# joejep/FOCNeRF

Hardware: AMD Instinct MI355X
Metric: train_samples_per_sec (higher is better)
Workload: dtype f16

## Files before the change

### focnerf_amd/_lib.py

```python
import ctypes
import os

import torch

_HERE = os.path.dirname(os.path.abspath(__file__))
LIB_PATH = os.environ.get("FOCNERF_LIB_PATH") or os.path.join(_HERE, "libfocnerf_hip.so")

c_u8p = ctypes.c_void_p
c_vp = ctypes.c_void_p
u32 = ctypes.c_uint32
u64 = ctypes.c_uint64
f32 = ctypes.c_float
i32 = ctypes.c_int

FOC_F32 = 0
FOC_F16 = 1



class FocOccTrainNode(ctypes.Structure):
    _fields_ = [
        ("struct_bytes", u32),
        ("n_rays", u32), ("max_steps", u32), ("cascade", u32), ("grid_size", u32), ("cap", u32), ("pad_align", u32),
        ("bound", f32), ("dt_gamma", f32), ("min_near", f32),
# ... 23 lines not shown
        ("mlp_workspace_bytes", u64),
    ]


SIGNATURES = {
    "foc_abi_version": (i32, []),
    "foc_last_error": (ctypes.c_char_p, []),
    "foc_arch": (ctypes.c_char_p, []),
    "foc_near_far_from_aabb": (i32, [c_vp, c_vp, c_vp, u32, f32, c_vp, c_vp, c_vp]),
    "foc_sph_from_ray": (i32, [c_vp, c_vp, f32, u32, c_vp, c_vp]),
    "foc_morton3D": (i32, [c_vp, u32, c_vp, c_vp]),
    "foc_morton3D_invert": (i32, [c_vp, u32, c_vp, c_vp]),
    "foc_packbits": (i32, [c_vp, u32, f32, c_vp, c_vp]),
    "foc_march_rays_train": (i32, [c_vp, c_vp, c_vp, f32, f32, u32, u32, u32, u32, u32, c_vp, c_vp,
                                   c_vp, c_vp, c_vp, c_vp, c_vp, c_vp, c_vp, c_vp]),
    "foc_march_rays_train_field": (i32, [c_vp, c_vp, c_vp, f32, f32, u32, u32, u32, u32, u32, c_vp, c_vp,
                                         c_vp, c_vp, c_vp, c_vp, c_vp, c_vp, c_vp, u32, c_vp, f32, c_vp]),
    "foc_set_option": (i32, [ctypes.c_char_p, i32]),
    "foc_get_option": (i32, [ctypes.c_char_p, c_vp]),
    "foc_guard_pick_device": (i32, [i32, i32, i32, i32]),
    "foc_grid_forward_index_path": (i32, [u32, u32, u32]),
    "foc_view_tile_order": (i32, [c_vp, u32, u32, u32, c_vp, c_vp, c_vp]),
    "foc_occ_train_forward": (i32, [ctypes.POINTER(FocOccTrainNode), c_vp]),
    "foc_occ_train_backward": (i32, [ctypes.POINTER(FocOccTrainNode), c_vp]),
    "foc_occ_train_forward_pad31": (i32, [ctypes.POINTER(FocOccTrainNode), f32, c_vp]),
    "foc_occ_train_backward_pad31": (i32, [ctypes.POINTER(FocOccTrainNode), f32, c_vp]),
    "foc_occ_tail_forward": (i32, [c_vp, c_vp, u32, c_vp, c_vp, u32, u32, f32, f32, c_vp, f32, c_vp, c_vp, c_vp, c_vp, c_vp, c_vp, c_vp]),
    "foc_occ_tail_backward": (i32, [c_vp, c_vp, c_vp, c_vp, u32, c_vp, c_vp, c_vp, c_vp, c_vp, u32, u32, f32, f32, c_vp, f32, c_vp, c_vp, c_vp]),
    "foc_march_rays_train_scratch_bytes": (u64, [u32, u32]),
    "foc_composite_rays_train_forward": (i32, [c_vp, c_vp, c_vp, c_vp, u32, u32, f32, c_vp, c_vp, c_vp, c_vp]),
    "foc_composite_rays_train_backward": (i32, [c_vp, c_vp, c_vp, c_vp, c_vp, c_vp, c_vp, c_vp, u32, u32, f32,
                                                c_vp, c_vp, c_vp]),
    "foc_march_rays": (i32, [u32, u32, c_vp, c_vp, c_vp, c_vp, f32, f32, u32, u32, u32, c_vp, c_vp, c_vp,
                             c_vp, c_vp, c_vp, c_vp, c_vp]),
    "foc_composite_rays": (i32, [u32, u32, f32, c_vp, c_vp, c_vp, c_vp, c_vp, c_vp, c_vp, c_vp, c_vp]),
    "foc_compact_alive": (i32, [c_vp, u32, c_vp, c_vp, c_vp, c_vp]),
    "foc_march_rays_two_phase": (i32, [u32, u32, c_vp, c_vp, c_vp, c_vp, f32, f32, u32, u32, u32, c_vp, c_vp, c_vp, c_vp, c_vp, c_vp, c_vp, c_vp, i32, c_vp]),
    "foc_composite_compact": (i32, [u32, u32, f32, c_vp, c_vp, c_vp, c_vp, c_vp, c_vp, c_vp, c_vp, c_vp, c_vp, c_vp, c_vp, u32, u32, i32, c_vp]),
    "foc_march_rays_two_phase_fills": (i32, [u32, i32]),
    "foc_march_rays_two_phase_sample_major": (i32, [u32, u32, i32]),
    "foc_occ_render_step_scratch_bytes": (u64, [u32]),
    "foc_occ_render_step": (i32, [u32, u32, c_vp, c_vp, c_vp, c_vp, c_vp, c_vp, f32, f32, u32, u32, u32, c_vp, c_vp, c_vp, c_vp, c_vp, c_vp, c_vp, c_vp,
                                  c_vp, c_vp, c_vp, u32, f32, u32, c_vp, u32, c_vp, u32, u32, c_vp, f32, c_vp, c_vp, c_vp, c_vp, u32, c_vp, u32, u32, c_vp]),
    "foc_occ_render_step_pad31": (i32, [u32, u32, c_vp, c_vp, c_vp, c_vp, c_vp, c_vp, f32, f32, u32, u32, u32, c_vp, c_vp, c_vp, c_vp, c_vp, c_vp, c_vp, c_vp,
                                        c_vp, c_vp, c_vp, u32, f32, u32, c_vp, u32, c_vp, u32, u32, c_vp, f32, c_vp, c_vp, c_vp, c_vp, u32, c_vp, u32, u32, f32,
                                        c_vp]),
    "foc_grid_encode_forward": (i32, [c_vp, c_vp, c_vp, c_vp, u32, u32, u32, u32, f32, u32, c_vp, u32, i32, u32,
                                      i32, c_vp, c_vp]),
    "foc_grid_encode_forward_bl": (i32, [c_vp, c_vp, c_vp, c_vp, u32, u32, u32, u32, f32, u32, c_vp, u32, i32, u32,
                                         i32, c_vp, c_vp]),
    "foc_grid_encode_backward": (i32, [c_vp, c_vp, c_vp, c_vp, c_vp, u32, u32, u32, u32, f32, u32, c_vp, c_vp,
                                       u32, i32, u32, i32, i32, c_vp, c_vp]),
    "foc_grid_encode_backward_workspace_bytes": (u64, [u32, u32, u32, u32, i32]),
    "foc_grid_planes_to_rows": (i32, [c_vp, c_vp, u32, u32, u32, c_vp]),
    "foc_grid_rows_to_planes": (i32, [c_vp, c_vp, u32, u32, u32, c_vp]),
    "foc_grid_encode_backward_binned": (i32, [c_vp, c_vp, c_vp, c_vp, c_vp, u32, u32, u32, u32, f32, u32, c_vp, c_vp,
                                              u32, i32, u32, i32, i32, c_vp, c_vp, u64, c_vp]),
    "foc_grid_encode_forward_counted": (i32, [c_vp, c_vp, c_vp, c_vp, u32, u32, u32, u32, f32, u32, u32, i32, u32, i32, c_vp, c_vp, u64, c_vp]),
    "foc_grid_encode_backward_count": (i32, [c_vp, c_vp, u32, u32, u32, u32, f32, u32, u32, i32, u32, i32, c_vp, c_vp, u64, c_vp]),
    "foc_grid_encode_backward_binned_counted": (i32, [c_vp, c_vp, c_vp, c_vp, c_vp, u32, u32, u32, u32, f32, u32, c_vp, c_vp,
                                                      u32, i32, u32, i32, i32, c_vp, c_vp, u64, c_vp]),
    "foc_grad_total_variation": (i32, [c_vp, c_vp, c_vp, c_vp, f32, u32, u32, u32, u32, f32, u32, u32, i32, i32, c_vp]),
    "foc_freq_encode_forward": (i32, [c_vp, u32, u32, u32, u32, c_vp, c_vp]),
    "foc_freq_encode_backward": (i32, [c_vp, c_vp, u32, u32, u32, u32, c_vp, c_vp]),
    "foc_ffmlp_forward": (i32, [c_vp, c_vp, u32, u32, u32, u32, u32, u32, u32, c_vp, c_vp, c_vp]),
    "foc_ffmlp_inference": (i32, [c_vp, c_vp, u32, u32, u32, u32, u32, u32, u32, c_vp, c_vp, c_vp]),
    "foc_ffmlp_backward": (i32, [c_vp, c_vp, c_vp, c_vp, u32, u32, u32, u32, u32, u32, u32, i32,
                                 c_vp, c_vp, c_vp, c_vp, u64, c_vp]),
    "foc_ffmlp_backward_workspace_bytes": (u64, [u32, u32, u32]),
    "foc_ffmlp_forward_planar": (i32, [c_vp, c_vp, u32, u32, u32, u32, u32, u32, u32, c_vp, c_vp]),
    "foc_ffmlp_backward_planar": (i32, [c_vp, c_vp, c_vp, u32, u32, u32, u32, u32, u32, u32, i32, c_vp, c_vp, c_vp, u64, c_vp]),
    "foc_allocate_splitk": (i32, [u64]),
    "foc_free_splitk": (i32, []),
    "foc_combine_select": (i32, [c_vp, c_vp, c_vp, c_vp, u64, c_vp]),
    "foc_combine_pack_keys": (i32, [c_vp, u32, c_vp, u64, c_vp]),
    "foc_combine_unpack": (i32, [c_vp, u32, c_vp, c_vp, c_vp, u64, c_vp]),
    "foc_combine_select_composite": (i32, [c_vp, u32, c_vp, c_vp, u32, u32, c_vp, u32, c_vp, c_vp, c_vp, c_vp]),
    "foc_combine_select4": (i32, [c_vp, c_vp, u64, c_vp]),
    "foc_mo_select": (i32, [c_vp, c_vp, c_vp, c_vp, u64, u32, u32, c_vp]),
    "foc_fixed_field_pack": (i32, [c_vp, c_vp, c_vp, c_vp, c_vp, c_vp, f32, u32, u32, f32, f32, c_vp, c_vp, c_vp, c_vp, u32, c_vp]),
    "foc_composite_fixed_steps": (i32, [c_vp, c_vp, c_vp, c_vp, u32, u32, f32, c_vp, c_vp, c_vp]),
    "foc_fixed_sample": (i32, [c_vp, c_vp, c_vp, c_vp, c_vp, c_vp, u32, u32, f32, c_vp, c_vp, c_vp, u32, c_vp]),
    "foc_fixed_tail_forward": (i32, [c_vp, c_vp, c_vp, c_vp, c_vp, c_vp, f32, u32, u32, f32, f32, c_vp, c_vp, c_vp, c_vp, c_vp, c_vp, u32, c_vp, c_vp]),
    "foc_fixed_tail_backward": (i32, [c_vp, c_vp, c_vp, c_vp, c_vp, c_vp, c_vp, c_vp, c_vp, c_vp, c_vp, f32, u32, u32, f32, f32, c_vp, c_vp, u32, c_vp, c_vp]),
    "foc_fixed_head_forward": (i32, [c_vp, c_vp, c_vp, c_vp, c_vp, u32, u32, f32, c_vp, c_vp, c_vp, c_vp, c_vp, c_vp, c_vp, u32, c_vp]),
    "foc_fixed_head_backward": (i32, [c_vp, c_vp, c_vp, c_vp, c_vp, c_vp, c_vp, c_vp, c_vp, c_vp, u32, u32, f32, c_vp, u32, c_vp]),
    "foc_color_head_forward": (i32, [c_vp, c_vp, u32, c_vp, u32, u32, u32, u32, c_vp, u32, c_vp, c_vp]),
    "foc_field_forward_train": (i32, [c_vp, c_vp, u32, c_vp, u32, c_vp, u32, u32, u32, u32, c_vp, c_vp, u32, c_vp, c_vp]),
    "foc_color_head_backward": (i32, [c_vp, c_vp, c_vp, u32, c_vp, c_vp, u32, u32, u32, u32, c_vp, c_vp, c_vp, u64, u32, c_vp, c_vp, c_vp]),
    "foc_color_head_forward_pad": (i32, [c_vp, c_vp, u32, c_vp, u32, u32, u32, u32, c_vp, u32, c_vp, f32, c_vp]),
    "foc_color_head_backward_pad": (i32, [c_vp, c_vp, c_vp, u32, c_vp, c_vp, u32, u32, u32, u32, c_vp, c_vp, c_vp, u64, u32, c_vp, c_vp, f32, c_vp]),
    "foc_field_forward_train_pad": (i32, [c_vp, c_vp, u32, c_vp, u32, c_vp, u32, u32, u32, u32, c_vp, c_vp, u32, c_vp, f32, c_vp]),
    "foc_color_head_forward_pad31": (i32, [c_vp, c_vp, u32, c_vp, u32, u32, u32, u32, c_vp, u32, c_vp, f32, c_vp]),
    "foc_color_head_backward_pad31": (i32, [c_vp, c_vp, c_vp, u32, c_vp, c_vp, u32, u32, u32, u32, c_vp, c_vp, c_vp, u64, u32, c_vp, c_vp, f32, c_vp]),
    "foc_field_forward_train_pad31": (i32, [c_vp, c_vp, u32, c_vp, u32, c_vp, u32, u32, u32, u32, c_vp, c_vp, u32, c_vp, f32, c_vp]),
    "foc_fixed_composite_forward": (i32, [c_vp, c_vp, c_vp, f32, u32, u32, f32, c_vp, c_vp]),
    "foc_fixed_composite_backward": (i32, [c_vp, c_vp, c_vp, c_vp, f32, u32, u32, f32, c_vp, c_vp, c_vp]),
    "foc_sample_head_forward": (i32, [c_vp, c_vp, u64, c_vp, c_vp, c_vp, u32, c_vp]),
    "foc_sample_head_backward": (i32, [c_vp, c_vp, c_vp, u64, c_vp, u32, c_vp]),
    "foc_sh_encode": (i32, [c_vp, u64, c_vp, c_vp]),
    "foc_rgb_head_forward": (i32, [c_vp, u64, c_vp, c_vp]),
    "foc_rgb_head_backward": (i32, [c_vp, c_vp, u64, c_vp, c_vp]),
    "foc_fixed_render_inference": (i32, [c_vp, c_vp, c_vp, c_vp, c_vp, c_vp, f32, u32, u32, f32, f32, c_vp, c_vp, c_vp, c_vp, u32, c_vp, c_vp]),
    "foc_nerf_field_inference": (i32, [c_vp, i32, c_vp, u32, u32, u32, c_vp, u32, c_vp, u32, u32, u32, u32, c_vp, c_vp, c_vp, c_vp]),
    "foc_nerf_field_inference_pad": (i32, [c_vp, i32, c_vp, u32, u32, u32, c_vp, u32, c_vp, u32, u32, u32, u32, c_vp, c_vp, c_vp, f32, c_vp]),
    "foc_nerf_field_inference_pad31": (i32, [c_vp, i32, c_vp, u32, u32, u32, c_vp, u32, c_vp, u32, u32, u32, u32, c_vp, c_vp, c_vp, f32, c_vp]),
    "foc_mark_untrained_grid": (i32, [c_vp, u32, f32, f32, f32, f32, f32, u32, u32, c_vp, c_vp, c_vp]),
    "foc_grid_cells_xyz": (i32, [u32, u32, f32, c_vp, c_vp, c_vp]),
    "foc_grid_update_sample_workspace_bytes": (u64, [u32, u32]),
    "foc_grid_update_sample": (i32, [c_vp, u32, u32, f32, u32, c_vp, c_vp, c_vp, c_vp, c_vp, c_vp, u64, c_vp]),
    "foc_grid_update_apply_workspace_bytes": (u64, [u32, u32]),
    "foc_grid_update_apply": (i32, [c_vp, u32, u32, c_vp, c_vp, u32, f32, f32, f32, c_vp, c_vp, c_vp, u64, c_vp]),
    "foc_background_forward": (i32, [c_vp, c_vp, c_vp, f32, u32, c_vp, c_vp, f32, u32, c_vp, c_vp, c_vp]),
    "foc_background_backward_workspace_bytes": (u64, [u32]),
    "foc_background_backward": (i32, [c_vp, c_vp, c_vp, c_vp, f32, u32, c_vp, c_vp, f32, u32, c_vp, c_vp, c_vp, c_vp, u64, c_vp]),
}


def _load():
    if not os.path.exists(LIB_PATH):
        raise ImportError(
            f"focnerf_amd: {LIB_PATH} is missing. Build it with `python -c 'import __graft_entry__ as g; g.build()'` "
            f"or `make -C focnerf_amd/csrc`. There is no CPU or PyTorch fallback for these ops.")
    try:
        lib = ctypes.CDLL(LIB_PATH)
    except OSError as e:
        raise ImportError(f"focnerf_amd: failed to load {LIB_PATH}: {e}") from e
    for name, (res, args) in SIGNATURES.items():
        fn = getattr(lib, name)
        fn.restype = res
        fn.argtypes = args
    return lib


class _Stream(ctypes.c_void_p):
    device_index = None


_multi_device = None


def _on_tensor_device(fn):
    def call(*args):
        global _multi_device
        if _multi_device is None:
            _multi_device = torch.cuda.device_count() > 1
        if _multi_device and args:
            idx = getattr(args[-1], "device_index", None)
            if idx is not None and idx != torch.cuda.current_device():
                with torch.cuda.device(idx):
                    return fn(*args)
        return fn(*args)
    call.__name__ = getattr(fn, "__name__", "foc_call")
    return call


class _Lib:

    def __init__(self, cdll):
        self._cdll = cdll
        for name, (_, args) in SIGNATURES.items():
            fn = getattr(cdll, name)
            setattr(self, name, _on_tensor_device(fn) if args and args[-1] is c_vp and not name.endswith("_bytes") else fn)


lib = _Lib(_load())


def check(rc, what=""):
    if rc != 0:
        msg = lib.foc_last_error().decode("utf-8", "replace")
        raise RuntimeError(f"focnerf_amd {what}: {msg} (code {rc})")


def ptr(t):
    if t is None:
        return None
    return ctypes.c_void_p(t.data_ptr())
# ... 57 lines not shown
```

### focnerf_amd/csrc/combine.hip

```cpp
#include "common.h"
#include <string.h>

static thread_local char g_err[512] = "";

void foc_set_error(const char *fmt, ...) {
    va_list ap;
    va_start(ap, fmt);
    vsnprintf(g_err, sizeof(g_err), fmt, ap);
    va_end(ap);
}

__global__ void __launch_bounds__(256) k_combine_select(const float *__restrict__ dens, const float *__restrict__ rgb,
                                                        float *__restrict__ max_dens, float *__restrict__ best_rgb, uint64_t n) {
    for (uint64_t i = (uint64_t)blockIdx.x * 256 + threadIdx.x; i < n; i += (uint64_t)gridDim.x * 256) {
        const float d = dens[i], m = max_dens[i];
        if (d > m) { best_rgb[i * 3] = rgb[i * 3]; best_rgb[i * 3 + 1] = rgb[i * 3 + 1]; best_rgb[i * 3 + 2] = rgb[i * 3 + 2]; }
        max_dens[i] = (d != d || m != m) ? __builtin_nanf("") : (d > m ? d : m);
    }
}

__global__ void __launch_bounds__(256) k_combine_pack(const float *__restrict__ dens, uint32_t rank, uint64_t *__restrict__ keys, uint64_t n) {
    for (uint64_t i = (uint64_t)blockIdx.x * 256 + threadIdx.x; i < n; i += (uint64_t)gridDim.x * 256) {
        float d = dens[i];
        d = d > 0.0f ? d : 0.0f;
// ... 85 lines not shown
        if (valid) {
            const uint64_t s = (uint64_t)n * T + i;
            float4 best = fields.p[0][s];
            for (uint32_t k = 1; k < K; k++) {
                const float4 f = fields.p[k][s];
                const float m = best.x;
                if (f.x > m) { best.y = f.y; best.z = f.z; best.w = f.w; }
                best.x = (f.x != f.x || m != m) ? __builtin_nanf("") : (f.x > m ? f.x : m);
            }
            if (merged4) merged4[s] = best;
            sigma = best.x; c0 = best.y; c1 = best.z; c2 = best.w;
            const float l0 = (i < T / 2) ? (step * (float)i) : fmaf(-step, (float)(T - 1 - i), 1.0f);
            const float z = near + span * l0;
            float delta = sample_dist;
            if (i + 1 < T) {
                const uint32_t i1 = i + 1;
                const float l1 = (i1 < T / 2) ? (step * (float)i1) : fmaf(-step, (float)(T - 1 - i1), 1.0f);
                delta = (near + span * l1) - z;
            }
            alpha = 1 - __expf(-delta * sigma);
            oz = (z - near) / span;
            oz = oz < 0 ? 0 : (oz > 1 ? 1 : oz);
        }
        const float om = valid ? (1 - alpha + 1e-15f) : 1.0f;
        const float P = wave_incl_prod(om, (int)lane);
        float Pex = __shfl_up(P, 1, 64);
        if (lane == 0) Pex = 1.0f;
        const float w = alpha * (Tc * Pex);
        r = fmaf(w, c0, r); g = fmaf(w, c1, g); b = fmaf(w, c2, b);
        a = fmaf(w, sigma, a); d = fmaf(w, oz, d); ws += w;
        Tc *= __shfl(P, 63, 64);
    }
    r = wave_sum(r); g = wave_sum(g); b = wave_sum(b); a = wave_sum(a); d = wave_sum(d); ws = wave_sum(ws);
    if (lane == 0) {
        for (uint32_t q = 0; q < n_bg; q++) {
            const float rest = (1 - ws) * (q == 0 ? bg0 : bg1);
            const float o[4] = {r + rest, g + rest, b + rest, a + rest};
#pragma unroll
            for (int k = 0; k < 4; k++) image4[((uint64_t)q * N + n) * 4 + k] = fminf(1.0f, fmaxf(0.0f, o[k]));
        }
        depth[n] = d;
    }
}

__global__ void __launch_bounds__(256) k_combine_select4(const float4 *__restrict__ f4, float4 *__restrict__ acc4, uint64_t n) {
    for (uint64_t i = (uint64_t)blockIdx.x * 256 + threadIdx.x; i < n; i += (uint64_t)gridDim.x * 256) {
        const float4 f = f4[i];
        float4 best = acc4[i];
        const float m = best.x;
        if (f.x > m) { best.y = f.y; best.z = f.z; best.w = f.w; }
        best.x = (f.x != f.x || m != m) ? __builtin_nanf("") : (f.x > m ? f.x : m);
        acc4[i] = best;
    }
}

template <typename T>
__global__ void __launch_bounds__(256) k_mo_select(const T *__restrict__ sig_new, const T *__restrict__ feat_new, T *__restrict__ sig_best,
                                                   T *__restrict__ feat_best, uint64_t n, uint32_t width) {
    const uint64_t s0 = ((uint64_t)blockIdx.x * 4u + (threadIdx.x >> 6)) * 64u;
    if (s0 >= n) return;
    const uint32_t lane = threadIdx.x & 63u;
    bool take = false;
    if (s0 + lane < n) {
        const T a_raw = sig_new[s0 + lane];
        const float a = (float)a_raw, b = (float)sig_best[s0 + lane];
        take = (a != a) || (b == b && a >= b);
        if (take) sig_best[s0 + lane] = a_raw;
    }
    const uint64_t rows = __ballot(take);
    const uint32_t live = (uint32_t)(n - s0 < 64u ? n - s0 : 64u);
    const uint64_t base = s0 * width;
    for (uint32_t e = lane; e < live * width; e += 64u)
        if ((rows >> (e / width)) & 1ull) feat_best[base + e] = feat_new[base + e];
}

#include <stdlib.h>
#include <string.h>
#include <atomic>
#include <mutex>
struct FocOptionRow { const char *name; std::atomic<int> value; };
static FocOptionRow foc_option_table[FOC_OPT_COUNT] = {
    {"FOC_MLP_BWD_FUSED", 1}, {"FOC_FIELD_FWD_FUSED", 1}, {"FOC_GB_MERGE_MAX_RES", 480}, {"FOC_GB_FACTORED", 1}, {"FOC_GB_TAIL_SPLIT", 16}, {"FOC_GRID_FUSE_SMALL", 1},
    {"FOC_GRID_PAIRS", 1}, {"FOC_GRID_FAST", 1}, {"FOC_MARCH_SERIAL", -1}, {"FOC_MARCH_RAYS_ROW_MAX", 131072}, {"FOC_OCC_MARCH_FORM", -1},
    {"FOC_OCC_SAMPLE_MAJOR", 1}, {"FOC_OCC_FIELD_PIECE", 1 << 23},
};
static int foc_option_parse(int which, const char *text) {
    if (which == FOC_OPT_OCC_MARCH_FORM) {
        if (text[0] == 't') return 0;
        if (text[0] == 'r') return 1;
        if (text[0] == 'l') return 2;
        if (text[0] == 's') return 3;
    }
    return atoi(text);
}
static void foc_options_init() {
    static std::once_flag once;
    std::call_once(once, [] {
        for (int i = 0; i < FOC_OPT_COUNT; i++) {
            const char *e = getenv(foc_option_table[i].name);
            if (e && e[0]) foc_option_table[i].value.store(foc_option_parse(i, e), std::memory_order_relaxed);
        }
    });
}
int foc_opt(FocOpt which) { foc_options_init(); return foc_option_table[which].value.load(std::memory_order_relaxed); }

extern "C" {

int foc_set_option(const char *name, int value) {
    foc_options_init();
    for (int i = 0; i < FOC_OPT_COUNT; i++)
        if (name && strcmp(name, foc_option_table[i].name) == 0) { foc_option_table[i].value.store(value, std::memory_order_relaxed); return FOC_OK; }
    foc_set_error("set_option: unknown option '%s'", name ? name : "(null)");
    return FOC_E_INVALID;
}

int foc_get_option(const char *name, int *value) {
    foc_options_init();
    for (int i = 0; i < FOC_OPT_COUNT; i++)
        if (name && value && strcmp(name, foc_option_table[i].name) == 0) { *value = foc_option_table[i].value.load(std::memory_order_relaxed); return FOC_OK; }
    foc_set_error("get_option: unknown option '%s'", name ? name : "(null)");
    return FOC_E_INVALID;
}

int foc_guard_pick_device(int stream_is_null, int stream_device, int pointer_device, int current_device) {
    return foc_guard_pick(stream_is_null != 0, stream_device, pointer_device, current_device);
}


int foc_combine_select_composite(const float *const *fields4, uint32_t K, const float *nears, const float *fars, uint32_t N, uint32_t T,
                                 const float *bgs, uint32_t n_bg, float *image4, float *depth, float *merged4, void *stream) {
    FocDeviceGuard foc_guard_(stream, nears);
    FOC_REQUIRE(K >= 1 && K <= FOC_COMBINE_MAX_OBJECTS, FOC_E_INVALID, "combine_select_composite: 1 <= K <= %d objects per call (got %u)",
                FOC_COMBINE_MAX_OBJECTS, K);
    FOC_REQUIRE(n_bg >= 1 && n_bg <= 2 && bgs, FOC_E_INVALID, "combine_select_composite: one or two backgrounds");
    FOC_REQUIRE(T >= 2, FOC_E_INVALID, "combine_select_composite: T must be >= 2");
    if (N == 0) return FOC_OK;
    FOC_REQUIRE(fields4 && nears && fars && image4 && depth, FOC_E_INVALID, "combine_select_composite: null pointer");
    CombineFields f;
    for (uint32_t k = 0; k < FOC_COMBINE_MAX_OBJECTS; k++) {
        f.p[k] = reinterpret_cast<const float4 *>(k < K ? fields4[k] : fields4[0]);
        FOC_REQUIRE(f.p[k] && ((uintptr_t)f.p[k] & 15) == 0, FOC_E_INVALID, "combine_select_composite: field %u is null or not 16-byte aligned", k);
    }
    FOC_REQUIRE(((uintptr_t)merged4 & 15) == 0, FOC_E_INVALID, "combine_select_composite: merged4 must be 16-byte aligned");
    hipLaunchKernelGGL(k_combine_select_composite, dim3(foc_div_up(N, 4)), dim3(256), 0, (hipStream_t)stream, f, K, nears, fars, N, T, bgs[0],
                       n_bg > 1 ? bgs[1] : 0.0f, n_bg, image4, depth, reinterpret_cast<float4 *>(merged4));
    FOC_CHECK_LAUNCH("combine_select_composite");
    return FOC_OK;
}

int foc_combine_select4(const float *field4, float *acc4, uint64_t n, void *stream) {
    FocDeviceGuard foc_guard_(stream, field4);
    FOC_REQUIRE(n == 0 || (field4 && acc4), FOC_E_INVALID, "combine_select4: null pointer");
    FOC_REQUIRE((((uintptr_t)field4 | (uintptr_t)acc4) & 15) == 0, FOC_E_INVALID, "combine_select4: fields must be 16-byte aligned");
    if (n == 0) return FOC_OK;
    hipLaunchKernelGGL(k_combine_select4, dim3(foc_grid_1d(n, 256)), dim3(256), 0, (hipStream_t)stream, reinterpret_cast<const float4 *>(field4),
                       reinterpret_cast<float4 *>(acc4), n);
    FOC_CHECK_LAUNCH("combine_select4");
    return FOC_OK;
}

int foc_mo_select(const void *sigma_new, const void *feat_new, void *sigma_best, void *feat_best, uint64_t n, uint32_t feat_width,
                  uint32_t elem_bytes, void *stream) {
    FocDeviceGuard foc_guard_(stream, sigma_new);
    FOC_REQUIRE(elem_bytes == 2 || elem_bytes == 4, FOC_E_INVALID, "mo_select: elem_bytes must be 2 (half) or 4 (float), got %u", elem_bytes);
    FOC_REQUIRE(feat_width >= 1 && feat_width <= 64, FOC_E_INVALID, "mo_select: feat_width %u outside 1..64", feat_width);
    FOC_REQUIRE(n == 0 || (sigma_new && feat_new && sigma_best && feat_best), FOC_E_INVALID, "mo_select: null pointer");
    FOC_REQUIRE(n < (1ull << 38), FOC_E_INVALID, "mo_select: n too large");
// ... 56 lines not shown
```

### focnerf_amd/csrc/common.h

```cpp
#pragma once
#include <hip/hip_runtime.h>
#include <hip/hip_fp16.h>
#include <stdint.h>
#include <stdio.h>
#include <stdarg.h>
#include "../../include/focnerf.h"

#define FOC_WAVE 64

void foc_set_error(const char *fmt, ...);

enum FocOpt {
    FOC_OPT_MLP_BWD_FUSED,
    FOC_OPT_FIELD_FWD_FUSED,
    FOC_OPT_GB_MERGE_MAX_RES,
    FOC_OPT_GB_FACTORED,
    FOC_OPT_GB_TAIL_SPLIT,
    FOC_OPT_GRID_FUSE_SMALL,
    FOC_OPT_GRID_PAIRS,
    FOC_OPT_GRID_FAST,
    FOC_OPT_MARCH_SERIAL,
    FOC_OPT_MARCH_RAYS_ROW_MAX,
    FOC_OPT_OCC_MARCH_FORM,
    FOC_OPT_OCC_SAMPLE_MAJOR,
    FOC_OPT_OCC_FIELD_PIECE,
    FOC_OPT_COUNT
};
int foc_opt(FocOpt which);

#define FOC_REQUIRE(cond, code, ...)                    \
    do {                                                \
        if (!(cond)) {                                  \
            foc_set_error(__VA_ARGS__);                 \
            return (code);                              \
        }                                               \
    } while (0)

#define FOC_CHECK_LAUNCH(name)                                                     \
    do {                                                                           \
        hipError_t e_ = hipGetLastError();                                         \
        if (e_ != hipSuccess) {                                                    \
            foc_set_error("%s: launch failed: %s", name, hipGetErrorString(e_));   \
            return FOC_E_LAUNCH;                                                   \
        }                                                                          \
    } while (0)

static inline int foc_guard_pick(bool stream_is_null, int stream_device, int pointer_device, int current_device) {
    if (!stream_is_null && stream_device >= 0) return stream_device;
    if (pointer_device >= 0) return pointer_device;
    return current_device;
}
struct FocDeviceGuard {
    int prev = -1;
    explicit FocDeviceGuard(void *stream, const void *first_pointer = nullptr) {
        static int n_devices = -1;
        if (n_devices < 0 && hipGetDeviceCount(&n_devices) != hipSuccess) { (void)hipGetLastError(); n_devices = 0; }
        if (n_devices == 1) return;
        int cur = 0;
        if (hipGetDevice(&cur) != hipSuccess) return;
        int sdev = -1, pdev = -1;
        if (stream != nullptr) {
            if (hipStreamGetDevice(static_cast<hipStream_t>(stream), &sdev) != hipSuccess) { (void)hipGetLastError(); sdev = -1; }
        } else if (first_pointer != nullptr) {
            hipPointerAttribute_t attr;
            if (hipPointerGetAttributes(&attr, first_pointer) == hipSuccess && attr.type == hipMemoryTypeDevice) pdev = attr.device;
            else (void)hipGetLastError();
        }
        const int want = foc_guard_pick(stream == nullptr, sdev, pdev, cur);
        if (want != cur && hipSetDevice(want) == hipSuccess) prev = cur;
    }
    ~FocDeviceGuard() { if (prev >= 0) (void)hipSetDevice(prev); }
    FocDeviceGuard(const FocDeviceGuard &) = delete;
    FocDeviceGuard &operator=(const FocDeviceGuard &) = delete;
};

static inline uint32_t foc_div_up(uint64_t a, uint64_t b) { return (uint32_t)((a + b - 1) / b); }

static inline uint32_t foc_grid_1d(uint64_t n, uint32_t block, uint32_t max_blocks = 256 * 8) {
    uint64_t g = (n + block - 1) / block;
    if (g < 1) g = 1;
    if (g > max_blocks) g = max_blocks;
    return (uint32_t)g;
}

__device__ __forceinline__ _Float16 foc_f2h(float v) { asm volatile("" : "+v"(v)); return (_Float16)v; }

__global__ static void __launch_bounds__(256) k_foc_zero(uint32_t *__restrict__ p, uint64_t n_words) {
    for (uint64_t i = (uint64_t)blockIdx.x * 256 + threadIdx.x; i < n_words; i += (uint64_t)gridDim.x * 256) p[i] = 0u;
}
static inline hipError_t foc_zero_async(void *p, size_t bytes, hipStream_t st) {
    const uint64_t n = bytes / 4;
    if (n == 0) return hipSuccess;
    uint64_t blocks = (n + 255) / 256;
    if (blocks > 4096) blocks = 4096;
    hipLaunchKernelGGL(k_foc_zero, dim3((uint32_t)blocks), dim3(256), 0, st, reinterpret_cast<uint32_t *>(p), n);
    return hipGetLastError();
}

__device__ __forceinline__ void foc_lds_barrier() { asm volatile("s_waitcnt lgkmcnt(0)\n\ts_barrier" ::: "memory"); }

__device__ __forceinline__ float wave_sum(float v) {
#pragma unroll
    for (int o = 32; o > 0; o >>= 1) v += __shfl_xor(v, o, 64);
    return v;
}
__device__ __forceinline__ int wave_sum_i(int v) {
#pragma unroll
    for (int o = 32; o > 0; o >>= 1) v += __shfl_xor(v, o, 64);
// ... 27 lines not shown
```

### focnerf_amd/csrc/field_fwd.hip

```cpp
#include "mlp_common.h"

typedef uint32_t ff_u2 __attribute__((ext_vector_type(2)));

__device__ __forceinline__ uint32_t ff_pack(float a, float b) {
    typedef _Float16 h2 __attribute__((ext_vector_type(2)));
    const h2 p = {(_Float16)a, (_Float16)b};
    return __builtin_bit_cast(uint32_t, p);
}

#ifndef FF_MIN_WAVES
#define FF_MIN_WAVES 2
#endif
template <int NLS, int NLC, bool RELU>
__global__ void __launch_bounds__(MLP_BLOCK, FF_MIN_WAVES) k_field_fwd_train(const _Float16 *__restrict__ planes, const _Float16 *__restrict__ w_sigma,
                                                               const _Float16 *__restrict__ w_color, _Float16 *__restrict__ h_out,
                                                               _Float16 *__restrict__ c_out, uint32_t B, MlpHead hd) {
    constexpr int HIDDEN = 64, MT = 2, KC = 4, KS0 = 2;
    constexpr int FS = MT * KS0 + (NLS - 1) * MT * KC + KC;
    constexpr int FC = MT * KS0 + (NLC - 1) * MT * KC + KC;
    extern __shared__ __attribute__((aligned(16))) _Float16 lds[];
    _Float16 *ldsS = lds, *ldsC = lds + FS * 512;
    const float *obj_bias = reinterpret_cast<const float *>(ldsC + FC * 512);
    stage_weights_fwd<HIDDEN>(w_sigma, ldsS, 32, NLS);
    stage_weights_fwd<HIDDEN>(w_color, ldsC, 32, NLC, true, head_ld0(hd));
    if (head_bias(hd)) stage_head_bias(w_color, hd, const_cast<float *>(obj_bias), HIDDEN);
    __syncthreads();

    const uint32_t lane = threadIdx.x & 63, wave = threadIdx.x >> 6;
    const int c = lane & 31, h = lane >> 5;
    const uint32_t n_tiles = (B + 31) / 32;
    const uint32_t tstride = gridDim.x * MLP_WAVES;
    uint32_t tile = blockIdx.x * MLP_WAVES + wave;
    h8 x_nxt[KS0], sh_nxt;
    auto fetch = [&](uint32_t t) {
#ifdef FF_TIMING_NO_LOAD
        const uint64_t r = (uint64_t)c + 0 * t;
#else
        const uint64_t r = min((uint64_t)min(t, n_tiles - 1u) * 32 + c, (uint64_t)B - 1);
#endif
#pragma unroll
        for (int kc = 0; kc < KS0; kc++) x_nxt[kc] = ld_planar8(planes, B, r, kc, h);
        sh_nxt = ld_head8(planes, hd, r, 0, h);
    };
    fetch(tile);
    for (; tile < n_tiles; tile += tstride) {
#ifndef FF_TIMING_HOIST
        asm volatile("" ::: "memory");
#endif
        const uint64_t row_raw = (uint64_t)tile * 32 + c;
        h8 x_cur[KS0];
#pragma unroll
        for (int kc = 0; kc < KS0; kc++) x_cur[kc] = x_nxt[kc];
        const h8 sh = sh_nxt;
        fetch(tile + tstride);
        f16v acc[MT];
#pragma unroll
        for (int mt = 0; mt < MT; mt++)
#pragma unroll
            for (int e = 0; e < 16; e++) acc[mt][e] = 0.0f;
#pragma unroll
        for (int kc = 0; kc < KS0; kc++)
#pragma unroll
            for (int mt = 0; mt < MT; mt++) acc[mt] = mfma16(ld_frag(ldsS, mt * KS0 + kc, lane), x_cur[kc], acc[mt]);
        f16v o;
        for (uint32_t l = 1; l <= (uint32_t)NLS; l++) {
            h8 bf[KC];
#pragma unroll
            for (int kc = 0; kc < KC; kc++) bf[kc] = acc_to_frag<RELU>(acc[kc >> 1], kc & 1);
            if (l < (uint32_t)NLS) {
                const uint32_t fbase = MT * KS0 + (l - 1) * MT * KC;
#pragma unroll
                for (int mt = 0; mt < MT; mt++)
#pragma unroll
                    for (int e = 0; e < 16; e++) acc[mt][e] = 0.0f;
#pragma unroll
                for (int kc = 0; kc < KC; kc++)
#pragma unroll
                    for (int mt = 0; mt < MT; mt++) acc[mt] = mfma16(ld_frag(ldsS, fbase + mt * KC + kc, lane), bf[kc], acc[mt]);
            } else {
#pragma unroll
                for (int e = 0; e < 16; e++) o[e] = 0.0f;
#pragma unroll
                for (int kc = 0; kc < KC; kc++) o = mfma16(ld_frag(ldsS, FS - KC + kc, lane), bf[kc], o);
            }
        }
        uint32_t P0 = ff_pack(o[0], o[1]), P1 = ff_pack(o[2], o[3]), P2 = ff_pack(o[4], o[5]), P3 = ff_pack(o[6], o[7]);
#ifdef FF_TIMING_NO_STORE
        if (row_raw == 0xFFFFFFFFFFull) {
#else
        if (row_raw < B) {
#endif
            *reinterpret_cast<ff_u2 *>(h_out + row_raw * 16 + 4 * h) = ff_u2{P0, P1};
            *reinterpret_cast<ff_u2 *>(h_out + row_raw * 16 + 8 + 4 * h) = ff_u2{P2, P3};
        }
        const uint32_t nxt = h == 0 ? P2 : 0u;
        const ff_u2 s02 = __builtin_amdgcn_permlane32_swap(P0, P2, false, false);
        const ff_u2 s13 = __builtin_amdgcn_permlane32_swap(P1, P3, false, false);
        const h8 hk = head_shift(u32x4{s02.x, s13.x, s02.y, s13.y}, nxt);
#pragma unroll
        for (int mt = 0; mt < MT; mt++) {
            if (head_bias(hd)) acc[mt] = ld_obj_bias(obj_bias, mt, h);
            else {
#pragma unroll
                for (int e = 0; e < 16; e++) acc[mt][e] = 0.0f;
            }
        }
#pragma unroll
        for (int kc = 0; kc < KS0; kc++)
#pragma unroll
            for (int mt = 0; mt < MT; mt++) acc[mt] = mfma16(ld_frag(ldsC, mt * KS0 + kc, lane), kc == 0 ? sh : hk, acc[mt]);
        for (uint32_t l = 1; l <= (uint32_t)NLC; l++) {
            h8 bf[KC];
#pragma unroll
            for (int kc = 0; kc < KC; kc++) bf[kc] = acc_to_frag<RELU>(acc[kc >> 1], kc & 1);
            if (l < (uint32_t)NLC) {
                const uint32_t fbase = MT * KS0 + (l - 1) * MT * KC;
#pragma unroll
                for (int mt = 0; mt < MT; mt++)
#pragma unroll
                    for (int e = 0; e < 16; e++) acc[mt][e] = 0.0f;
#pragma unroll
                for (int kc = 0; kc < KC; kc++)
#pragma unroll
                    for (int mt = 0; mt < MT; mt++) acc[mt] = mfma16(ld_frag(ldsC, fbase + mt * KC + kc, lane), bf[kc], acc[mt]);
            } else {
#pragma unroll
                for (int e = 0; e < 16; e++) o[e] = 0.0f;
#pragma unroll
                for (int kc = 0; kc < KC; kc++) o = mfma16(ld_frag(ldsC, FC - KC + kc, lane), bf[kc], o);
                if (hd.out_width == 4u) {
#ifdef FF_TIMING_NO_STORE
                    if (h == 0 && row_raw == 0xFFFFFFFFFFull) *reinterpret_cast<ff_u2 *>(c_out + row_raw * 4) = ff_u2{ff_pack(o[0], o[1]), ff_pack(o[2], o[3])};
#else
                    if (h == 0 && row_raw < B) *reinterpret_cast<ff_u2 *>(c_out + row_raw * 4) = ff_u2{ff_pack(o[0], o[1]), ff_pack(o[2], o[3])};
#endif
                } else store_tile<false>(c_out, 16, row_raw, B, 0, 16, o, h);
            }
        }
    }
}

static uint32_t ff_num_cus() {
    int dev = 0, n = 0;
    if (hipGetDevice(&dev) != hipSuccess || hipDeviceGetAttribute(&n, hipDeviceAttributeMultiprocessorCount, dev) != hipSuccess || n <= 0) n = 256;
    return (uint32_t)n;
}

template <int NLS, int NLC, bool RELU>
static int ff_launch(const void *planes, const void *w_sigma, const void *w_color, void *h, void *c, uint32_t B, const MlpHead &hd, hipStream_t st) {
    auto kern = k_field_fwd_train<NLS, NLC, RELU>;
    const size_t lds = (size_t)((4 + (NLS - 1) * 8 + 4) + (4 + (NLC - 1) * 8 + 4)) * 1024 + 256;
    if (lds > 64 * 1024) (void)hipFuncSetAttribute(reinterpret_cast<const void *>(kern), hipFuncAttributeMaxDynamicSharedMemorySize, (int)lds);
    static int resident = 0;
    if (!resident) {
        int n = 0;
        if (hipOccupancyMaxActiveBlocksPerMultiprocessor(&n, kern, MLP_BLOCK, lds) != hipSuccess || n < 1) n = 2;
        resident = n > 8 ? 8 : n;
    }
    uint32_t grid = foc_div_up(foc_div_up(B, 32), MLP_WAVES);
    const uint32_t cap = ff_num_cus() * (uint32_t)resident;
    if (grid > cap) grid = cap;
    hipLaunchKernelGGL(kern, dim3(grid), dim3(MLP_BLOCK), lds, st, (const _Float16 *)planes, (const _Float16 *)w_sigma, (const _Float16 *)w_color,
                       (_Float16 *)h, (_Float16 *)c, B, hd);
    FOC_CHECK_LAUNCH("field_forward_train");
    return FOC_OK;
}

template <int NLS, int NLC>
static int ff_launch_act(const void *planes, const void *w_sigma, const void *w_color, void *h, void *c, uint32_t B, int relu, const MlpHead &hd, hipStream_t st) {
    return relu ? ff_launch<NLS, NLC, true>(planes, w_sigma, w_color, h, c, B, hd, st) : ff_launch<NLS, NLC, false>(planes, w_sigma, w_color, h, c, B, hd, st);
}

static int field_forward_train(const void *planes, const void *sigma_weights, uint32_t sigma_layers, const void *ray_sh, uint32_t samples_per_ray,
                               const void *color_weights, uint32_t color_layers, uint32_t hidden_dim, uint32_t activation, uint32_t B, void *h, void *c,
                               uint32_t out_width, const void *obj_feat, float input_pad, bool pad31, void *stream) {
    FocDeviceGuard foc_guard_(stream, planes);
    if (B == 0) return FOC_OK;
    FOC_REQUIRE(planes && sigma_weights && ray_sh && color_weights && h && c, FOC_E_INVALID, "field_forward_train: null pointer");
    FOC_REQUIRE(hidden_dim == 64 && samples_per_ray >= 1, FOC_E_INVALID, "field_forward_train: hidden_dim must be 64 (got %u), samples_per_ray >= 1", hidden_dim);
    FOC_REQUIRE(activation == FOC_ACT_RELU || activation == FOC_ACT_NONE, FOC_E_INVALID, "field_forward_train: hidden activation must be relu(0) or none(6)");
    FOC_REQUIRE(out_width == 16 || out_width == 4, FOC_E_INVALID, "field_forward_train: out_width must be 16 or 4 (got %u)", out_width);
    const int prc = head_pad_check("field_forward_train", pad31, obj_feat, input_pad);
    if (prc) return prc;
    const MlpHead hd{(const _Float16 *)ray_sh, nullptr, samples_per_ray, out_width, (const _Float16 *)obj_feat, input_pad};
    const int relu = activation == FOC_ACT_RELU;
    hipStream_t st = (hipStream_t)stream;
    switch (sigma_layers * 10 + color_layers) {
        case 12: return ff_launch_act<1, 2>(planes, sigma_weights, color_weights, h, c, B, relu, hd, st);
        case 13: return ff_launch_act<1, 3>(planes, sigma_weights, color_weights, h, c, B, relu, hd, st);
        case 22: return ff_launch_act<2, 2>(planes, sigma_weights, color_weights, h, c, B, relu, hd, st);
        case 23: return ff_launch_act<2, 3>(planes, sigma_weights, color_weights, h, c, B, relu, hd, st);
        case 33: return ff_launch_act<3, 3>(planes, sigma_weights, color_weights, h, c, B, relu, hd, st);
        default: foc_set_error("field_forward_train: layer counts (%u, %u) are not built (1/2, 1/3, 2/2, 2/3, 3/3)", sigma_layers, color_layers); return FOC_E_INVALID;
    }
}

extern "C" {

int foc_field_forward_train(const void *planes, const void *sigma_weights, uint32_t sigma_layers, const void *ray_sh, uint32_t samples_per_ray,
                            const void *color_weights, uint32_t color_layers, uint32_t hidden_dim, uint32_t activation, uint32_t B, void *h, void *c,
                            uint32_t out_width, const void *obj_feat, void *stream) {
    return field_forward_train(planes, sigma_weights, sigma_layers, ray_sh, samples_per_ray, color_weights, color_layers, hidden_dim, activation, B, h, c,
                               out_width, obj_feat, 0.0f, false, stream);
}

int foc_field_forward_train_pad(const void *planes, const void *sigma_weights, uint32_t sigma_layers, const void *ray_sh, uint32_t samples_per_ray,
                                const void *color_weights, uint32_t color_layers, uint32_t hidden_dim, uint32_t activation, uint32_t B, void *h, void *c,
                                uint32_t out_width, const void *obj_feat, float input_pad, void *stream) {
    return field_forward_train(planes, sigma_weights, sigma_layers, ray_sh, samples_per_ray, color_weights, color_layers, hidden_dim, activation, B, h, c,
                               out_width, obj_feat, input_pad, false, stream);
}

int foc_field_forward_train_pad31(const void *planes, const void *sigma_weights, uint32_t sigma_layers, const void *ray_sh, uint32_t samples_per_ray,
                                  const void *color_weights, uint32_t color_layers, uint32_t hidden_dim, uint32_t activation, uint32_t B, void *h, void *c,
                                  uint32_t out_width, const void *obj_feat, float input_pad, void *stream) {
    return field_forward_train(planes, sigma_weights, sigma_layers, ray_sh, samples_per_ray, color_weights, color_layers, hidden_dim, activation, B, h, c,
                               out_width, obj_feat, input_pad, true, stream);
}

}
```

### focnerf_amd/csrc/fixedstep.hip

```cpp
#include "common.h"
#include <float.h>

typedef _Float16 h8 __attribute__((ext_vector_type(8)));

struct FsGeom { float near, far, span, sample_dist, step; };

#define FS_RAY_BLOCK 64u
__host__ __device__ __forceinline__ uint64_t fs_block_row(uint32_t n, uint32_t i, uint32_t T) {
    return (uint64_t)(n / FS_RAY_BLOCK) * FS_RAY_BLOCK * T + (uint64_t)i * FS_RAY_BLOCK + n % FS_RAY_BLOCK;
}

__device__ __forceinline__ FsGeom fs_geom(const float *__restrict__ nears, const float *__restrict__ fars, uint32_t n, uint32_t T) {
    FsGeom g;
    g.near = nears[n]; g.far = fars[n];
    g.span = g.far - g.near;
    g.sample_dist = g.span / (float)T;
    g.step = 1.0f / (float)(T - 1);
    return g;
}
__device__ __forceinline__ float fs_z(const FsGeom &g, uint32_t i, uint32_t T, const float *__restrict__ noise, uint64_t s) {
    const float lin = (i < T / 2) ? (g.step * (float)i) : fmaf(-g.step, (float)(T - 1 - i), 1.0f);
    float z = g.near + g.span * lin;
    if (noise) z = z + (noise[s] - 0.5f) * g.sample_dist;
    return z;
}

template <bool NOISE>
__device__ __forceinline__ float fs_zu(const FsGeom &g, uint32_t i, uint32_t T, float u) {
    const float lin = (i < T / 2) ? (g.step * (float)i) : fmaf(-g.step, (float)(T - 1 - i), 1.0f);
    float z = g.near + g.span * lin;
    if (NOISE) z = z + (u - 0.5f) * g.sample_dist;
    return z;
}

__device__ __forceinline__ void fs_sh16(float x, float y, float z, float (&o)[16]) {
    const float xy = x * y, xz = x * z, yz = y * z, x2 = x * x, y2 = y * y, z2 = z * z;
    o[0] = 0.28209479177387814f;
    o[1] = -0.48860251190291987f * y;
    o[2] = 0.48860251190291987f * z;
    o[3] = -0.48860251190291987f * x;
    o[4] = 1.0925484305920792f * xy;
    o[5] = -1.0925484305920792f * yz;
    o[6] = 0.94617469575755997f * z2 - 0.31539156525251999f;
    o[7] = -1.0925484305920792f * xz;
    o[8] = 0.54627421529603959f * x2 - 0.54627421529603959f * y2;
    o[9] = 0.59004358992664352f * y * (-3.0f * x2 + y2);
    o[10] = 2.8906114426405538f * xy * z;
    o[11] = 0.45704579946446572f * y * (1.0f - 5.0f * z2);
    o[12] = 0.3731763325901154f * z * (5.0f * z2 - 3.0f);
    o[13] = 0.45704579946446572f * x * (1.0f - 5.0f * z2);
    o[14] = 1.4453057213202769f * z * (x2 - y2);
    o[15] = 0.59004358992664352f * x * (-x2 + 3.0f * y2);
}

__global__ void __launch_bounds__(256) k_fs_sample(const float *__restrict__ rays_o, const float *__restrict__ rays_d, const float *__restrict__ nears,
                                                   const float *__restrict__ fars, const float *__restrict__ aabb, const float *__restrict__ noise,
                                                   uint32_t N, uint32_t T, float bound, float *__restrict__ xyzs, float *__restrict__ enc_in,
                                                   _Float16 *__restrict__ ray_sh, uint32_t ray_block) {
    const uint64_t total = ray_block ? (uint64_t)((N + FS_RAY_BLOCK - 1) / FS_RAY_BLOCK) * FS_RAY_BLOCK * T : (uint64_t)N * T;
    const float a0 = aabb[0], a1 = aabb[1], a2 = aabb[2], a3 = aabb[3], a4 = aabb[4], a5 = aabb[5];
    const float two_b = 2 * bound;
    for (uint64_t s = (uint64_t)blockIdx.x * 256 + threadIdx.x; s < total; s += (uint64_t)gridDim.x * 256) {
        uint32_t n, i;
        bool own = true;
        if (ray_block) {
            const uint32_t blk = (uint32_t)(s / ((uint64_t)FS_RAY_BLOCK * T)), in = (uint32_t)(s - (uint64_t)blk * FS_RAY_BLOCK * T);
            i = in / FS_RAY_BLOCK;
            n = blk * FS_RAY_BLOCK + in % FS_RAY_BLOCK;
            own = n < N;
            n = own ? n : N - 1;
        } else {
            n = (uint32_t)(s / T); i = (uint32_t)(s - (uint64_t)n * T);
        }
        const FsGeom g = fs_geom(nears, fars, n, T);
        const float z = fs_z(g, i, T, noise, (uint64_t)n * T + i);
        float x = rays_o[n * 3] + rays_d[n * 3] * z, y = rays_o[n * 3 + 1] + rays_d[n * 3 + 1] * z, w = rays_o[n * 3 + 2] + rays_d[n * 3 + 2] * z;
        x = fminf(fmaxf(x, a0), a3); y = fminf(fmaxf(y, a1), a4); w = fminf(fmaxf(w, a2), a5);
        if (xyzs) { xyzs[s * 3] = x; xyzs[s * 3 + 1] = y; xyzs[s * 3 + 2] = w; }
        if (enc_in) { enc_in[s * 3] = (x + bound) / two_b; enc_in[s * 3 + 1] = (y + bound) / two_b; enc_in[s * 3 + 2] = (w + bound) / two_b; }
        if (ray_sh && i == 0 && own) {
            float sh[16];
            fs_sh16(rays_d[n * 3], rays_d[n * 3 + 1], rays_d[n * 3 + 2], sh);
            h8 lo, hi;
#pragma unroll
            for (int k = 0; k < 8; k++) { lo[k] = foc_f2h(sh[k]); hi[k] = foc_f2h(sh[8 + k]); }
            h8 *dst = reinterpret_cast<h8 *>(ray_sh + (uint64_t)n * 16);
            dst[0] = lo; dst[1] = hi;
        }
    }
}

__global__ void __launch_bounds__(256) k_fs_head_fwd(const _Float16 *__restrict__ h, const float *__restrict__ rays_d, const float *__restrict__ nears,
                                                     const float *__restrict__ fars, const float *__restrict__ noise, uint32_t N, uint32_t T,
                                                     float density_scale, float *__restrict__ sigma_out, float *__restrict__ trans_out,
                                                     float *__restrict__ weights_out, float *__restrict__ weights_sum, float *__restrict__ depth,
                                                     _Float16 *__restrict__ cin, const _Float16 *__restrict__ obj, uint32_t cin_ld) {
    const uint32_t lane = threadIdx.x & 63;
    const uint32_t n = blockIdx.x * 4 + (threadIdx.x >> 6);
    if (n >= N) return;
    const FsGeom g = fs_geom(nears, fars, n, T);
    h8 shlo, shhi;
    h8 ob1 = {0, 0, 0, 0, 0, 0, 0, 0}, ob2 = {0, 0, 0, 0, 0, 0, 0, 0};
    _Float16 ob0 = (_Float16)0;
    if (cin) {
        float sh[16];
        fs_sh16(rays_d[n * 3], rays_d[n * 3 + 1], rays_d[n * 3 + 2], sh);
#pragma unroll
        for (int k = 0; k < 8; k++) { shlo[k] = foc_f2h(sh[k]); shhi[k] = foc_f2h(sh[8 + k]); }
        if (obj) {
            ob0 = obj[0];
#pragma unroll
            for (int k = 0; k < 8; k++) ob1[k] = obj[1 + k];
#pragma unroll
            for (int k = 0; k < 7; k++) ob2[k] = obj[9 + k];
        }
    }
    float Tc = 1.0f, ws = 0, dp = 0;
    for (uint32_t base = 0; base < T; base += 64) {
        const uint32_t i = base + lane;
        const bool valid = i < T;
        const uint64_t s = (uint64_t)n * T + (valid ? i : T - 1);
        h8 r0, r1;
        if (cin) { r0 = *reinterpret_cast<const h8 *>(h + s * 16); r1 = *reinterpret_cast<const h8 *>(h + s * 16 + 8); }
        else r0[0] = h[s * 16];
        const float sigma = expf((float)r0[0]);
        const float z = fs_z(g, valid ? i : T - 1, T, noise, s);
        float delta = g.sample_dist;
        if (i + 1 < T) delta = fs_z(g, i + 1, T, noise, s + 1) - z;
        const float alpha = valid ? 1 - expf((-delta * density_scale) * sigma) : 0.0f;
        const float om = valid ? (1 - alpha + 1e-15f) : 1.0f;
        const float P = wave_incl_prod(om, (int)lane);
        float Pex = __shfl_up(P, 1, 64);
        if (lane == 0) Pex = 1.0f;
        const float Tb = Tc * Pex;
        const float w = alpha * Tb;
        if (valid) {
            sigma_out[s] = sigma; trans_out[s] = Tb; weights_out[s] = w;
            float oz = (z - g.near) / g.span;
            oz = oz < 0.0f ? 0.0f : (oz > 1.0f ? 1.0f : oz);
            ws += w; dp += w * oz;
            if (cin) {
                h8 c2, c3;
#pragma unroll
                for (int k = 0; k < 7; k++) { c2[k] = r0[k + 1]; c3[k] = r1[k + 1]; }
                c2[7] = r1[0]; c3[7] = ob0;
                h8 *dst = reinterpret_cast<h8 *>(cin + s * cin_ld);
                dst[0] = shlo; dst[1] = shhi; dst[2] = c2; dst[3] = c3;
                if (cin_ld == 48) { dst[4] = ob1; dst[5] = ob2; }
            }
        }
        Tc *= __shfl(P, 63, 64);
    }
    ws = wave_sum(ws); dp = wave_sum(dp);
    if (lane == 0) { weights_sum[n] = ws; depth[n] = dp; }
}

__device__ __forceinline__ float wave_suffix_incl_sum(float v, int lane) {
#pragma unroll
    for (int o = 1; o < 64; o <<= 1) {
        const float u = __shfl_down(v, o, 64);
        if (lane + o < 64) v += u;
    }
    return v;
}

__global__ void __launch_bounds__(256) k_fs_head_bwd(const _Float16 *__restrict__ h, const float *__restrict__ sigma_in, const float *__restrict__ trans_in,
                                                     const float *__restrict__ nears, const float *__restrict__ fars, const float *__restrict__ noise,
                                                     const float *__restrict__ grad_w, const float *__restrict__ grad_ws, const float *__restrict__ grad_depth,
                                                     const _Float16 *__restrict__ grad_cin, uint32_t N, uint32_t T, float density_scale,
                                                     _Float16 *__restrict__ grad_h, uint32_t cin_ld) {
    const uint32_t lane = threadIdx.x & 63;
    const uint32_t n = blockIdx.x * 4 + (threadIdx.x >> 6);
// ... 22 lines not shown
        const float S_i = S_carry + (incl - gw_i);
        const float dalpha = gi * Tb - S_i / om;
        const float dsigma = dalpha * (delta * density_scale) * ex;
        const _Float16 h0 = h[s * 16];
        const float dh0 = dsigma * expf(fminf(fmaxf((float)h0, -15.0f), 15.0f));
        if (valid) {
            h8 o0, o1;
            if (grad_cin) {
                const h8 c2 = *reinterpret_cast<const h8 *>(grad_cin + s * cin_ld + 16), c3 = *reinterpret_cast<const h8 *>(grad_cin + s * cin_ld + 24);
#pragma unroll
                for (int k = 0; k < 7; k++) { o0[k + 1] = c2[k]; o1[k + 1] = c3[k]; }
                o1[0] = c2[7];
            } else {
#pragma unroll
                for (int k = 0; k < 8; k++) { o0[k] = (_Float16)0; o1[k] = (_Float16)0; }
            }
            o0[0] = foc_f2h(dh0);
            h8 *dst = reinterpret_cast<h8 *>(grad_h + s * 16);
            dst[0] = o0; dst[1] = o1;
        }
        S_carry += __shfl(incl, 0, 64);
    }
}

__device__ __forceinline__ float fs_sigmoid_h(float x) {
    return (float)(_Float16)(1.0f / (1.0f + expf(-x)));
}

__global__ void __launch_bounds__(256) k_fs_composite_fwd(const _Float16 *__restrict__ c, const float *__restrict__ weights, const float *__restrict__ bg_ray,
                                                          float bg_scalar, uint32_t N, uint32_t T, float thresh, float *__restrict__ image) {
    const uint32_t lane = threadIdx.x & 63;
    const uint32_t n = blockIdx.x * 4 + (threadIdx.x >> 6);
    if (n >= N) return;
    float r = 0, g = 0, b = 0, ws = 0;
    for (uint32_t i = lane; i < T; i += 64) {
        const uint64_t s = (uint64_t)n * T + i;
        const float w = weights[s];
        ws += w;
        if (w > thresh) {
            const uint2 raw = *reinterpret_cast<const uint2 *>(c + s * 16);
            const _Float16 *cc = reinterpret_cast<const _Float16 *>(&raw);
            r += w * fs_sigmoid_h((float)cc[0]); g += w * fs_sigmoid_h((float)cc[1]); b += w * fs_sigmoid_h((float)cc[2]);
        }
    }
    r = wave_sum(r); g = wave_sum(g); b = wave_sum(b); ws = wave_sum(ws);
    if (lane == 0) {
        const float b0 = bg_ray ? bg_ray[n * 3] : bg_scalar, b1 = bg_ray ? bg_ray[n * 3 + 1] : bg_scalar, b2 = bg_ray ? bg_ray[n * 3 + 2] : bg_scalar;
        image[n * 3] = r + (1 - ws) * b0; image[n * 3 + 1] = g + (1 - ws) * b1; image[n * 3 + 2] = b + (1 - ws) * b2;
    }
}

__global__ void __launch_bounds__(256) k_fs_composite_bwd(const float *__restrict__ grad_image, const _Float16 *__restrict__ c, const float *__restrict__ weights,
                                                          const float *__restrict__ bg_ray, float bg_scalar, uint32_t N, uint32_t T, float thresh,
                                                          _Float16 *__restrict__ grad_c, float *__restrict__ grad_w) {
    const uint64_t total = (uint64_t)N * T;
    for (uint64_t s = (uint64_t)blockIdx.x * 256 + threadIdx.x; s < total; s += (uint64_t)gridDim.x * 256) {
        const uint32_t n = (uint32_t)(s / T);
        const float g0 = grad_image[n * 3], g1 = grad_image[n * 3 + 1], g2 = grad_image[n * 3 + 2];
        const float b0 = bg_ray ? bg_ray[n * 3] : bg_scalar, b1 = bg_ray ? bg_ray[n * 3 + 1] : bg_scalar, b2 = bg_ray ? bg_ray[n * 3 + 2] : bg_scalar;
        const float w = weights[s];
        float gw = -(g0 * b0 + g1 * b1 + g2 * b2);
        h8 o0, o1;
#pragma unroll
        for (int k = 0; k < 8; k++) { o0[k] = (_Float16)0; o1[k] = (_Float16)0; }
        if (w > thresh) {
            const uint2 raw = *reinterpret_cast<const uint2 *>(c + s * 16);
            const _Float16 *cc = reinterpret_cast<const _Float16 *>(&raw);
            const float y0 = fs_sigmoid_h((float)cc[0]), y1 = fs_sigmoid_h((float)cc[1]), y2 = fs_sigmoid_h((float)cc[2]);
            gw += g0 * y0 + g1 * y1 + g2 * y2;
            o0[0] = foc_f2h(g0 * w * y0 * (1 - y0)); o0[1] = foc_f2h(g1 * w * y1 * (1 - y1)); o0[2] = foc_f2h(g2 * w * y2 * (1 - y2));
        }
        grad_w[s] = gw;
        h8 *dst = reinterpret_cast<h8 *>(grad_c + s * 16);
        dst[0] = o0; dst[1] = o1;
    }
}

template <bool NOISE>
__global__ void __launch_bounds__(256) k_fs_tail_fwd(const _Float16 *__restrict__ h, const _Float16 *__restrict__ c, const float *__restrict__ nears,
                                                     const float *__restrict__ fars, const float *__restrict__ noise, const float *__restrict__ bg_ray,
                                                     float bg_scalar, uint32_t N, uint32_t T, float density_scale, float thresh,
                                                     float *__restrict__ sigma_out, float *__restrict__ trans_out, float *__restrict__ weights_out,
                                                     float *__restrict__ weights_sum, float *__restrict__ depth, float *__restrict__ image, uint32_t c_ld,
                                                     float *__restrict__ ray_sumsq) {
    const uint32_t lane = threadIdx.x & 63;
    const uint32_t n = blockIdx.x * 4 + (threadIdx.x >> 6);
    if (n >= N) return;
    const FsGeom g = fs_geom(nears, fars, n, T);
    float Tc = 1.0f, ws = 0, dp = 0, r = 0, gg = 0, b = 0, sq = 0;
    for (uint32_t base = 0; base < T; base += 64) {
        const uint32_t i = base + lane;
        const bool valid = i < T;
        const uint32_t ic = valid ? i : T - 1;
        const uint64_t s = (uint64_t)n * T + ic;
        const _Float16 h0 = h[s * 16];
        const uint2 raw = *reinterpret_cast<const uint2 *>(c + s * c_ld);
        float u0 = 0.0f, u1 = 0.0f;
        if (NOISE) { u0 = noise[s]; u1 = noise[(uint64_t)n * T + min(ic + 1u, T - 1u)]; }
        const float sigma = expf((float)h0);
        const float z = fs_zu<NOISE>(g, ic, T, u0);
        float delta = g.sample_dist;
        if (i + 1 < T) delta = fs_zu<NOISE>(g, i + 1, T, u1) - z;
        const float alpha = valid ? 1 - expf((-delta * density_scale) * sigma) : 0.0f;
        const float om = valid ? (1 - alpha + 1e-15f) : 1.0f;
        const float P = wave_incl_prod(om, (int)lane);
        float Pex = __shfl_up(P, 1, 64);
        if (lane == 0) Pex = 1.0f;
        const float Tb = Tc * Pex;
        const float w = alpha * Tb;
        if (valid) {
            sigma_out[s] = sigma; trans_out[s] = Tb; weights_out[s] = w;
            float oz = (z - g.near) / g.span;
            oz = oz < 0.0f ? 0.0f : (oz > 1.0f ? 1.0f : oz);
            ws += w; dp += w * oz; sq = fmaf(sigma, sigma, sq);
            if (w > thresh) {
                const _Float16 *cc = reinterpret_cast<const _Float16 *>(&raw);
                r += w * fs_sigmoid_h((float)cc[0]); gg += w * fs_sigmoid_h((float)cc[1]); b += w * fs_sigmoid_h((float)cc[2]);
            }
        }
        Tc *= __shfl(P, 63, 64);
    }
    ws = wave_sum(ws); dp = wave_sum(dp); r = wave_sum(r); gg = wave_sum(gg); b = wave_sum(b);
    if (ray_sumsq) {
        sq = wave_sum(sq);
        if (lane == 0) ray_sumsq[n] = sq;
    }
    if (lane == 0) {
        const float b0 = bg_ray ? bg_ray[n * 3] : bg_scalar, b1 = bg_ray ? bg_ray[n * 3 + 1] : bg_scalar, b2 = bg_ray ? bg_ray[n * 3 + 2] : bg_scalar;
        image[n * 3] = r + (1 - ws) * b0; image[n * 3 + 1] = gg + (1 - ws) * b1; image[n * 3 + 2] = b + (1 - ws) * b2;
        weights_sum[n] = ws; depth[n] = dp;
    }
}

__device__ __forceinline__ float fs_opaque(float v) { asm volatile("" : "+v"(v)); return v; }

template <bool NOISE>
__global__ void __launch_bounds__(256) k_fs_tail_bwd(const float *__restrict__ grad_image, const float *__restrict__ grad_ws, const float *__restrict__ grad_depth,
                                                     const _Float16 *__restrict__ c, const float *__restrict__ sigma_in, const float *__restrict__ trans_in,
                                                     const float *__restrict__ weights, const float *__restrict__ nears, const float *__restrict__ fars,
                                                     const float *__restrict__ noise, const float *__restrict__ bg_ray, float bg_scalar, uint32_t N, uint32_t T,
                                                     float density_scale, float thresh, _Float16 *__restrict__ grad_c, _Float16 *__restrict__ grad_h0, uint32_t c_ld,
                                                     const float *__restrict__ grad_sumsq) {
    const uint32_t lane = threadIdx.x & 63;
    const uint32_t n = blockIdx.x * 4 + (threadIdx.x >> 6);
    if (n >= N) return;
    const FsGeom g = fs_geom(nears, fars, n, T);
    const float gws = grad_ws ? grad_ws[n] : 0.0f, gdp = grad_depth ? grad_depth[n] : 0.0f;
    const float gsq2 = grad_sumsq ? 2.0f * grad_sumsq[n] : 0.0f;
    const float g0 = grad_image[n * 3], g1 = grad_image[n * 3 + 1], g2 = grad_image[n * 3 + 2];
    const float b0 = bg_ray ? bg_ray[n * 3] : bg_scalar, b1 = bg_ray ? bg_ray[n * 3 + 1] : bg_scalar, b2 = bg_ray ? bg_ray[n * 3 + 2] : bg_scalar;
    const float e_lo = expf(fs_opaque(-15.0f)), e_hi = expf(fs_opaque(15.0f));
    float S_carry = 0.0f;
    const uint32_t n_chunks = (T + 63) / 64;
    for (uint32_t cidx = n_chunks; cidx-- > 0;) {
        const uint32_t i = cidx * 64 + lane;
        const bool valid = i < T;
        const uint32_t ic = valid ? i : T - 1;
        const uint64_t s = (uint64_t)n * T + ic;
        const float sigma = sigma_in[s], Tb = trans_in[s], w = weights[s];
        const uint2 raw = *reinterpret_cast<const uint2 *>(c + s * c_ld);
        float u0 = 0.0f, u1 = 0.0f;
        if (NOISE) { u0 = noise[s]; u1 = noise[(uint64_t)n * T + min(ic + 1u, T - 1u)]; }
        float gw = -(g0 * b0 + g1 * b1 + g2 * b2);
        h8 o0, o1;
#pragma unroll
        for (int k = 0; k < 8; k++) { o0[k] = (_Float16)0; o1[k] = (_Float16)0; }
        if (w > thresh) {
            const _Float16 *cc = reinterpret_cast<const _Float16 *>(&raw);
            const float y0 = fs_sigmoid_h((float)cc[0]), y1 = fs_sigmoid_h((float)cc[1]), y2 = fs_sigmoid_h((float)cc[2]);
            gw += g0 * y0 + g1 * y1 + g2 * y2;
            o0[0] = foc_f2h(g0 * w * y0 * (1 - y0)); o0[1] = foc_f2h(g1 * w * y1 * (1 - y1)); o0[2] = foc_f2h(g2 * w * y2 * (1 - y2));
        }
        if (valid) {
            if (c_ld == 4u) *reinterpret_cast<uint2 *>(grad_c + s * 4) = *reinterpret_cast<const uint2 *>(&o0);
            else { h8 *dst = reinterpret_cast<h8 *>(grad_c + s * 16); dst[0] = o0; dst[1] = o1; }
        }
        const float z = fs_zu<NOISE>(g, ic, T, u0);
        float delta = g.sample_dist;
// ... 90 lines not shown
                                                              float *__restrict__ image, float *__restrict__ depth, float *__restrict__ weights_sum,
                                                              float *__restrict__ rgb_masked, float4 *__restrict__ field4, float *__restrict__ sigma_rm) {
    __shared__ float tile_s[64][FS_BLK_RAYS + 1];
    __shared__ float tile_c[64][FS_BLK_RAYS * 3 + 1];
    const uint32_t tid = threadIdx.x, lane = tid & 63;
    const uint32_t wv = __builtin_amdgcn_readfirstlane(tid >> 6);
    const uint32_t n0 = blockIdx.x * FS_BLK_RAYS;
    const uint64_t row0 = fs_block_row(n0, 0, T);
    const bool is_s = tid < 256;
    const uint32_t li = is_s ? tid : tid - 256;
    const uint32_t l_step = is_s ? li >> 2 : li / 12, l_part = is_s ? (li & 3) : li % 12;
    const float *src = is_s ? sigma_in + row0 + l_part * 4 : rgb_in + row0 * 3 + l_part * 4;
    const uint32_t src_ld = is_s ? FS_RAY_BLOCK : FS_RAY_BLOCK * 3;
    float *dst = is_s ? &tile_s[l_step][l_part * 4] : &tile_c[l_step][l_part * 4];
    float4 nx = make_float4(0, 0, 0, 0);
    if (l_step < T) nx = *reinterpret_cast<const float4 *>(src + (uint64_t)l_step * src_ld);
    const uint32_t n = n0 + wv;
    const bool own = n < N;
    const FsGeom g = fs_geom(nears, fars, own ? n : N - 1, T);
    FsRayAcc a = {1.0f, 0, 0, 0, 0, 0};
    for (uint32_t base = 0; base < T; base += 64) {
        dst[0] = nx.x; dst[1] = nx.y; dst[2] = nx.z; dst[3] = nx.w;
        __syncthreads();
        if (base + 64 + l_step < T) nx = *reinterpret_cast<const float4 *>(src + (uint64_t)(base + 64 + l_step) * src_ld);
        if (own)
            fs_infer_tile<PACK>(a, g, n, base + lane, lane, T, tile_s[lane][wv], tile_c[lane][wv * 3], tile_c[lane][wv * 3 + 1], tile_c[lane][wv * 3 + 2],
                                noise, density_scale, thresh, rgb_masked, field4, sigma_rm);
        __syncthreads();
    }
    if (own) fs_infer_finish<PACK>(a, n, lane, bg_ray, bg_scalar, image, depth, weights_sum);
}

struct VtState { uint32_t count, first_enc, bad, pad; };

__device__ __forceinline__ bool vt_turn(const float *__restrict__ d, uint32_t i) {
    const float ax = d[(i + 1) * 3] - d[i * 3], ay = d[(i + 1) * 3 + 1] - d[i * 3 + 1], az = d[(i + 1) * 3 + 2] - d[i * 3 + 2];
    const float bx = d[(i + 2) * 3] - d[(i + 1) * 3], by = d[(i + 2) * 3 + 1] - d[(i + 1) * 3 + 1], bz = d[(i + 2) * 3 + 2] - d[(i + 1) * 3 + 2];
    return (bx * ax + by * ay) + bz * az < 0.0f;
}

__global__ void __launch_bounds__(256) k_vt_find(const float *__restrict__ d, uint32_t N, VtState *__restrict__ st) {
    for (uint32_t i = blockIdx.x * 256 + threadIdx.x; i + 2 < N; i += gridDim.x * 256)
        if (vt_turn(d, i)) { atomicAdd(&st->count, 1u); atomicMax(&st->first_enc, N - i); }
}

__global__ void __launch_bounds__(256) k_vt_check(const float *__restrict__ d, uint32_t N, VtState *__restrict__ st) {
    const uint32_t fe = st->first_enc;
    if (fe == 0u) return;
    const uint32_t W = N - fe + 2u;
    for (uint32_t i = blockIdx.x * 256 + threadIdx.x; i + 2 < N; i += gridDim.x * 256) {
        const bool expect = (i + 2u) % W == 0u || (i + 1u) % W == 0u;
        if (vt_turn(d, i) != expect) st->bad = 1u;
    }
}

__global__ void __launch_bounds__(256) k_vt_perm(uint32_t N, uint32_t th, uint32_t tw, const VtState *__restrict__ st, int64_t *__restrict__ perm) {
    const uint32_t fe = st->first_enc, W = fe ? N - fe + 2u : 0u;
    const uint32_t H = W ? N / W : 0u;
    const bool grid = W >= 16u && N % W == 0u && H >= 8u && st->count == 2u * (H - 1u) && st->bad == 0u;
    for (uint32_t p = blockIdx.x * 256 + threadIdx.x; p < N; p += gridDim.x * 256) {
        uint32_t src = p;
        if (grid) {
            const uint64_t wt = (uint64_t)W * th;
            const uint32_t ty = (uint32_t)(p / wt), rem = (uint32_t)(p - ty * wt);
            const uint32_t rows_here = min(th, H - ty * th);
            const uint32_t tx = min(rem / (rows_here * tw), (W - 1u) / tw), r2 = rem - tx * rows_here * tw;
            const uint32_t cols_here = min(tw, W - tx * tw);
            src = (ty * th + r2 / cols_here) * W + tx * tw + r2 % cols_here;
        }
        perm[p] = (int64_t)src;
    }
}

extern "C" {

int foc_fixed_sample(const float *rays_o, const float *rays_d, const float *nears, const float *fars, const float *aabb, const float *noise,
                     uint32_t N, uint32_t T, float bound, float *xyzs, float *enc_in, void *ray_sh, uint32_t ray_block, void *stream) {
    FocDeviceGuard foc_guard_(stream, rays_o);
    if (N == 0) return FOC_OK;
    FOC_REQUIRE(rays_o && rays_d && nears && fars && aabb && (xyzs || enc_in), FOC_E_INVALID, "fixed_sample: null pointer");
    FOC_REQUIRE(T >= 2, FOC_E_INVALID, "fixed_sample: T must be >= 2");
    FOC_REQUIRE(ray_block == 0 || ray_block == FS_RAY_BLOCK, FOC_E_INVALID, "fixed_sample: ray_block must be 0 (ray-major) or %u (got %u)", FS_RAY_BLOCK, ray_block);
    const uint64_t rows = ray_block ? (uint64_t)foc_div_up(N, FS_RAY_BLOCK) * FS_RAY_BLOCK * T : (uint64_t)N * T;
    hipLaunchKernelGGL(k_fs_sample, dim3(foc_grid_1d(rows, 256, 256 * 16)), dim3(256), 0, (hipStream_t)stream, rays_o, rays_d, nears, fars, aabb,
                       noise, N, T, bound, xyzs, enc_in, (_Float16 *)ray_sh, ray_block);
    FOC_CHECK_LAUNCH("fixed_sample");
    return FOC_OK;
}

int foc_fixed_head_forward(const void *h, const float *rays_d, const float *nears, const float *fars, const float *noise, uint32_t N, uint32_t T,
                           float density_scale, float *sigma, float *trans, float *weights, float *weights_sum, float *depth, void *cin,
                           const void *obj_feat, uint32_t cin_width, void *stream) {
    FocDeviceGuard foc_guard_(stream, h);
    if (N == 0) return FOC_OK;
    FOC_REQUIRE(h && rays_d && nears && fars && sigma && trans && weights && weights_sum && depth, FOC_E_INVALID, "fixed_head_forward: null pointer");
    FOC_REQUIRE(T >= 2, FOC_E_INVALID, "fixed_head_forward: T must be >= 2");
    FOC_REQUIRE(cin_width == 32 || cin_width == 48, FOC_E_INVALID, "fixed_head_forward: cin_width must be 32 or 48 (got %u)", cin_width);
    FOC_REQUIRE(!obj_feat || cin_width == 48, FOC_E_INVALID, "fixed_head_forward: an object feature needs the 48-wide colour input");
    hipLaunchKernelGGL(k_fs_head_fwd, dim3(foc_div_up(N, 4)), dim3(256), 0, (hipStream_t)stream, (const _Float16 *)h, rays_d, nears, fars, noise, N, T,
                       density_scale, sigma, trans, weights, weights_sum, depth, (_Float16 *)cin, (const _Float16 *)obj_feat, cin_width);
    FOC_CHECK_LAUNCH("fixed_head_forward");
    return FOC_OK;
}

int foc_fixed_head_backward(const void *h, const float *sigma, const float *trans, const float *nears, const float *fars, const float *noise,
                            const float *grad_w, const float *grad_ws, const float *grad_depth, const void *grad_cin, uint32_t N, uint32_t T,
                            float density_scale, void *grad_h, uint32_t cin_width, void *stream) {
    FocDeviceGuard foc_guard_(stream, h);
    if (N == 0) return FOC_OK;
    FOC_REQUIRE(h && sigma && trans && nears && fars && grad_h, FOC_E_INVALID, "fixed_head_backward: null pointer");
    FOC_REQUIRE(T >= 2, FOC_E_INVALID, "fixed_head_backward: T must be >= 2");
    FOC_REQUIRE(cin_width == 32 || cin_width == 48, FOC_E_INVALID, "fixed_head_backward: cin_width must be 32 or 48 (got %u)", cin_width);
    hipLaunchKernelGGL(k_fs_head_bwd, dim3(foc_div_up(N, 4)), dim3(256), 0, (hipStream_t)stream, (const _Float16 *)h, sigma, trans, nears, fars, noise,
                       grad_w, grad_ws, grad_depth, (const _Float16 *)grad_cin, N, T, density_scale, (_Float16 *)grad_h, cin_width);
    FOC_CHECK_LAUNCH("fixed_head_backward");
    return FOC_OK;
}

int foc_fixed_composite_forward(const void *c, const float *weights, const float *bg_ray, float bg_scalar, uint32_t N, uint32_t T, float thresh,
                                float *image, void *stream) {
    FocDeviceGuard foc_guard_(stream, c);
    if (N == 0) return FOC_OK;
    FOC_REQUIRE(c && weights && image, FOC_E_INVALID, "fixed_composite_forward: null pointer");
    hipLaunchKernelGGL(k_fs_composite_fwd, dim3(foc_div_up(N, 4)), dim3(256), 0, (hipStream_t)stream, (const _Float16 *)c, weights, bg_ray, bg_scalar, N, T,
                       thresh, image);
    FOC_CHECK_LAUNCH("fixed_composite_forward");
    return FOC_OK;
}

int foc_fixed_composite_backward(const float *grad_image, const void *c, const float *weights, const float *bg_ray, float bg_scalar, uint32_t N,
                                 uint32_t T, float thresh, void *grad_c, float *grad_w, void *stream) {
    FocDeviceGuard foc_guard_(stream, grad_image);
    if (N == 0) return FOC_OK;
    FOC_REQUIRE(grad_image && c && weights && grad_c && grad_w, FOC_E_INVALID, "fixed_composite_backward: null pointer");
    hipLaunchKernelGGL(k_fs_composite_bwd, dim3(foc_grid_1d((uint64_t)N * T, 256, 256 * 16)), dim3(256), 0, (hipStream_t)stream, grad_image,
                       (const _Float16 *)c, weights, bg_ray, bg_scalar, N, T, thresh, (_Float16 *)grad_c, grad_w);
    FOC_CHECK_LAUNCH("fixed_composite_backward");
    return FOC_OK;
}

int foc_fixed_tail_forward(const void *h, const void *c, const float *nears, const float *fars, const float *noise, const float *bg_ray, float bg_scalar,
                           uint32_t N, uint32_t T, float density_scale, float thresh, float *sigma, float *trans, float *weights, float *weights_sum,
                           float *depth, float *image, uint32_t c_width, float *ray_sumsq, void *stream) {
    FocDeviceGuard foc_guard_(stream, h);
    if (N == 0) return FOC_OK;
    FOC_REQUIRE(c_width == 16 || c_width == 4, FOC_E_INVALID, "fixed_tail_forward: c_width must be 16 or 4 (got %u)", c_width);
    FOC_REQUIRE(h && c && nears && fars && sigma && trans && weights && weights_sum && depth && image, FOC_E_INVALID, "fixed_tail_forward: null pointer");
    FOC_REQUIRE(T >= 2, FOC_E_INVALID, "fixed_tail_forward: T must be >= 2");
    auto kern = noise ? k_fs_tail_fwd<true> : k_fs_tail_fwd<false>;
    hipLaunchKernelGGL(kern, dim3(foc_div_up(N, 4)), dim3(256), 0, (hipStream_t)stream, (const _Float16 *)h, (const _Float16 *)c, nears, fars, noise,
                       bg_ray, bg_scalar, N, T, density_scale, thresh, sigma, trans, weights, weights_sum, depth, image, c_width, ray_sumsq);
    FOC_CHECK_LAUNCH("fixed_tail_forward");
    return FOC_OK;
}

int foc_fixed_tail_backward(const float *grad_image, const float *grad_ws, const float *grad_depth, const void *c, const float *sigma, const float *trans,
                            const float *weights, const float *nears, const float *fars, const float *noise, const float *bg_ray, float bg_scalar,
                            uint32_t N, uint32_t T, float density_scale, float thresh, void *grad_c, void *grad_h0, uint32_t c_width, const float *grad_sumsq,
                            void *stream) {
    FocDeviceGuard foc_guard_(stream, grad_image);
    if (N == 0) return FOC_OK;
    FOC_REQUIRE(c_width == 16 || c_width == 4, FOC_E_INVALID, "fixed_tail_backward: c_width must be 16 or 4 (got %u)", c_width);
    FOC_REQUIRE(grad_image && c && sigma && trans && weights && nears && fars && grad_c && grad_h0, FOC_E_INVALID, "fixed_tail_backward: null pointer");
    FOC_REQUIRE(T >= 2, FOC_E_INVALID, "fixed_tail_backward: T must be >= 2");
    auto kern = noise ? k_fs_tail_bwd<true> : k_fs_tail_bwd<false>;
    hipLaunchKernelGGL(kern, dim3(foc_div_up(N, 4)), dim3(256), 0, (hipStream_t)stream, grad_image, grad_ws, grad_depth, (const _Float16 *)c, sigma,
                       trans, weights, nears, fars, noise, bg_ray, bg_scalar, N, T, density_scale, thresh, (_Float16 *)grad_c, (_Float16 *)grad_h0, c_width,
                       grad_sumsq);
    FOC_CHECK_LAUNCH("fixed_tail_backward");
    return FOC_OK;
}

int foc_fixed_render_inference(const float *sigma, const float *rgb, const float *nears, const float *fars, const float *noise, const float *bg_ray,
                               float bg_scalar, uint32_t N, uint32_t T, float density_scale, float thresh, float *image, float *depth, float *weights_sum,
                               float *rgb_masked, uint32_t ray_block, float *sigma_raymajor, void *stream) {
    FocDeviceGuard foc_guard_(stream, sigma);
    if (N == 0) return FOC_OK;
    FOC_REQUIRE(sigma && rgb && nears && fars && image && depth && weights_sum, FOC_E_INVALID, "fixed_render_inference: null pointer");
    FOC_REQUIRE(T >= 2, FOC_E_INVALID, "fixed_render_inference: T must be >= 2");
    FOC_REQUIRE(ray_block == 0 || ray_block == FS_RAY_BLOCK, FOC_E_INVALID, "fixed_render_inference: ray_block must be 0 or %u (got %u)", FS_RAY_BLOCK, ray_block);
    FOC_REQUIRE(ray_block || !sigma_raymajor, FOC_E_INVALID, "fixed_render_inference: sigma_raymajor is the un-blocked copy of a blocked sigma (ray_block == 0: sigma already is ray-major)");
    if (ray_block) {
        FOC_REQUIRE((((uintptr_t)sigma | (uintptr_t)rgb) & 15) == 0, FOC_E_INVALID, "fixed_render_inference: blocked sigma / rgb must be 16-byte aligned");
        hipLaunchKernelGGL(k_fs_render_infer_blk<false>, dim3(foc_div_up(N, FS_BLK_RAYS)), dim3(1024), 0, (hipStream_t)stream, sigma, rgb, nears, fars, noise, bg_ray, bg_scalar,
                           N, T, density_scale, thresh, image, depth, weights_sum, rgb_masked, (float4 *)nullptr, sigma_raymajor);
        FOC_CHECK_LAUNCH("fixed_render_inference");
        return FOC_OK;
    }
    hipLaunchKernelGGL(k_fs_render_infer<false>, dim3(foc_div_up(N, 4)), dim3(256), 0, (hipStream_t)stream, sigma, rgb, nears, fars, noise, bg_ray, bg_scalar, N, T,
                       density_scale, thresh, image, depth, weights_sum, rgb_masked, (float4 *)nullptr);
    FOC_CHECK_LAUNCH("fixed_render_inference");
    return FOC_OK;
}

int foc_fixed_field_pack(const float *sigma, const float *rgb, const float *nears, const float *fars, const float *noise, const float *bg_ray,
                         float bg_scalar, uint32_t N, uint32_t T, float density_scale, float thresh, float *image, float *depth, float *weights_sum,
                         float *field4, uint32_t ray_block, void *stream) {
    FocDeviceGuard foc_guard_(stream, sigma);
    if (N == 0) return FOC_OK;
    FOC_REQUIRE(sigma && rgb && nears && fars && field4, FOC_E_INVALID, "fixed_field_pack: null pointer");
    FOC_REQUIRE((image && depth && weights_sum) || (!image && !depth && !weights_sum), FOC_E_INVALID,
                "fixed_field_pack: image, depth and weights_sum go together (all or none)");
    FOC_REQUIRE(((uintptr_t)field4 & 15) == 0, FOC_E_INVALID, "fixed_field_pack: field4 must be 16-byte aligned");
    FOC_REQUIRE(T >= 2, FOC_E_INVALID, "fixed_field_pack: T must be >= 2");
    FOC_REQUIRE(ray_block == 0 || ray_block == FS_RAY_BLOCK, FOC_E_INVALID, "fixed_field_pack: ray_block must be 0 or %u (got %u)", FS_RAY_BLOCK, ray_block);
    if (ray_block) {
        FOC_REQUIRE((((uintptr_t)sigma | (uintptr_t)rgb) & 15) == 0, FOC_E_INVALID, "fixed_field_pack: blocked sigma / rgb must be 16-byte aligned");
        hipLaunchKernelGGL(k_fs_render_infer_blk<true>, dim3(foc_div_up(N, FS_BLK_RAYS)), dim3(1024), 0, (hipStream_t)stream, sigma, rgb, nears, fars, noise, bg_ray, bg_scalar,
                           N, T, density_scale, thresh, image, depth, weights_sum, (float *)nullptr, (float4 *)field4, (float *)nullptr);
        FOC_CHECK_LAUNCH("fixed_field_pack");
        return FOC_OK;
    }
    hipLaunchKernelGGL(k_fs_render_infer<true>, dim3(foc_div_up(N, 4)), dim3(256), 0, (hipStream_t)stream, sigma, rgb, nears, fars, noise, bg_ray, bg_scalar, N, T,
                       density_scale, thresh, image, depth, weights_sum, (float *)nullptr, (float4 *)field4);
    FOC_CHECK_LAUNCH("fixed_field_pack");
    return FOC_OK;
}

int foc_view_tile_order(const float *rays_d, uint32_t N, uint32_t tile_h, uint32_t tile_w, int64_t *perm, void *state16, void *stream) {
    FocDeviceGuard foc_guard_(stream, rays_d);
    if (N == 0) return FOC_OK;
    FOC_REQUIRE(rays_d && perm && state16, FOC_E_INVALID, "view_tile_order: null pointer");
    FOC_REQUIRE(tile_h >= 1 && tile_w >= 1 && tile_h * tile_w <= 4096, FOC_E_INVALID, "view_tile_order: tile %u x %u", tile_h, tile_w);
    FOC_REQUIRE(N < (1u << 31), FOC_E_INVALID, "view_tile_order: N too large");
    hipStream_t st = (hipStream_t)stream;
    VtState *state = reinterpret_cast<VtState *>(state16);
    if (foc_zero_async(state, sizeof(VtState), st) != hipSuccess) { foc_set_error("view_tile_order: zero fill failed"); return FOC_E_LAUNCH; }
    if (N >= 3) {
        hipLaunchKernelGGL(k_vt_find, dim3(foc_grid_1d(N, 256)), dim3(256), 0, st, rays_d, N, state);
        hipLaunchKernelGGL(k_vt_check, dim3(foc_grid_1d(N, 256)), dim3(256), 0, st, rays_d, N, state);
    }
    hipLaunchKernelGGL(k_vt_perm, dim3(foc_grid_1d(N, 256)), dim3(256), 0, st, N, tile_h, tile_w, state, perm);
    FOC_CHECK_LAUNCH("view_tile_order");
    return FOC_OK;
}

// ... 2 lines not shown
```

### focnerf_amd/csrc/gridencoder.hip

```cpp
#include "common.h"
#include <math.h>
#include <stdlib.h>

#include "ge_common.h"

template <uint32_t D>
__device__ __forceinline__ uint32_t ge_index(uint32_t gridtype, bool align_corners, uint32_t hashmap_size, uint32_t resolution,
                                             const uint32_t (&pos_grid)[D]) {
    constexpr uint32_t primes[7] = {1u, 2654435761u, 805459861u, 3674653429u, 2097192037u, 1434869437u, 2165219737u};
    uint32_t stride = 1, index = 0;
#pragma unroll
    for (uint32_t d = 0; d < D; d++) {
        if (stride <= hashmap_size) {
            index += pos_grid[d] * stride;
            stride *= align_corners ? resolution : (resolution + 1);
        }
    }
    if (gridtype == 0 && stride > hashmap_size) {
        uint32_t result = 0;
#pragma unroll
        for (uint32_t i = 0; i < D; i++) result ^= pos_grid[i] * primes[i];
        index = result;
    }
    if (index >= hashmap_size) index = ((hashmap_size & (hashmap_size - 1u)) == 0u) ? (index & (hashmap_size - 1u)) : (index % hashmap_size);
// ... 466 lines not shown
    gb_cell_weights<D>(pos, ws);
    gb_cell_rows<D>(pos_grid, hashmap_size, resolution, gridtype, align_corners, rows);
}

#define GB_MERGE_MAX_RES 480u
template <int CTRL>
__device__ __forceinline__ uint32_t gb_dpp(uint32_t v) { return (uint32_t)__builtin_amdgcn_update_dpp(0, (int)v, CTRL, 0xf, 0xf, true); }
struct GbRun { uint32_t f0, f1, f2, f3; float k0, k1, k2, k3; bool tail; };
__device__ __forceinline__ GbRun gb_run_flags(bool inside, const uint32_t (&pos_grid)[3]) {
    const uint32_t r = threadIdx.x & 15u;
    const uint32_t key = inside ? (pos_grid[0] | (pos_grid[1] << 10) | (pos_grid[2] << 20)) : 0xFFFFFFFFu;
    const uint32_t prev = gb_dpp<0x111>(key);
    const uint32_t head = (r == 0u || key != prev || !inside) ? 1u : 0u;
    GbRun run;
    run.f0 = head;
    run.f1 = run.f0 | gb_dpp<0x111>(run.f0);
    run.f2 = run.f1 | gb_dpp<0x112>(run.f1);
    run.f3 = run.f2 | gb_dpp<0x114>(run.f2);
    const uint32_t next_head = gb_dpp<0x101>(head);
    run.tail = inside && (r == 15u || next_head != 0u);
    run.k0 = run.f0 ? 0.0f : 1.0f; run.k1 = run.f1 ? 0.0f : 1.0f; run.k2 = run.f2 ? 0.0f : 1.0f; run.k3 = run.f3 ? 0.0f : 1.0f;
    return run;
}
__device__ __forceinline__ float gb_run_sum(float v, const GbRun &run) {
    float u;
#ifdef FOC_GB_MERGE_SELECT
    u = __uint_as_float(gb_dpp<0x111>(__float_as_uint(v))); v = run.f0 ? v : v + u;
    u = __uint_as_float(gb_dpp<0x112>(__float_as_uint(v))); v = run.f1 ? v : v + u;
    u = __uint_as_float(gb_dpp<0x114>(__float_as_uint(v))); v = run.f2 ? v : v + u;
    u = __uint_as_float(gb_dpp<0x118>(__float_as_uint(v))); v = run.f3 ? v : v + u;
#else
    u = __uint_as_float(gb_dpp<0x111>(__float_as_uint(v))); v = fmaf(u, run.k0, v);
    u = __uint_as_float(gb_dpp<0x112>(__float_as_uint(v))); v = fmaf(u, run.k1, v);
    u = __uint_as_float(gb_dpp<0x114>(__float_as_uint(v))); v = fmaf(u, run.k2, v);
    u = __uint_as_float(gb_dpp<0x118>(__float_as_uint(v))); v = fmaf(u, run.k3, v);
#endif
    return v;
}
#ifndef FOC_GB_MERGE_SELECT
#define GB_FMAC16(CTRL)                                                                                                                  \
    asm volatile("s_nop 1\n\t"                                                                                                           \
                 "v_fmac_f32_dpp %0, %0, %16 " CTRL " row_mask:0xf bank_mask:0xf bound_ctrl:1\n\t"                                       \
                 "v_fmac_f32_dpp %1, %1, %16 " CTRL " row_mask:0xf bank_mask:0xf bound_ctrl:1\n\t"                                       \
                 "v_fmac_f32_dpp %2, %2, %16 " CTRL " row_mask:0xf bank_mask:0xf bound_ctrl:1\n\t"                                       \
                 "v_fmac_f32_dpp %3, %3, %16 " CTRL " row_mask:0xf bank_mask:0xf bound_ctrl:1\n\t"                                       \
                 "v_fmac_f32_dpp %4, %4, %16 " CTRL " row_mask:0xf bank_mask:0xf bound_ctrl:1\n\t"                                       \
                 "v_fmac_f32_dpp %5, %5, %16 " CTRL " row_mask:0xf bank_mask:0xf bound_ctrl:1\n\t"                                       \
                 "v_fmac_f32_dpp %6, %6, %16 " CTRL " row_mask:0xf bank_mask:0xf bound_ctrl:1\n\t"                                       \
                 "v_fmac_f32_dpp %7, %7, %16 " CTRL " row_mask:0xf bank_mask:0xf bound_ctrl:1\n\t"                                       \
                 "v_fmac_f32_dpp %8, %8, %16 " CTRL " row_mask:0xf bank_mask:0xf bound_ctrl:1\n\t"                                       \
                 "v_fmac_f32_dpp %9, %9, %16 " CTRL " row_mask:0xf bank_mask:0xf bound_ctrl:1\n\t"                                       \
                 "v_fmac_f32_dpp %10, %10, %16 " CTRL " row_mask:0xf bank_mask:0xf bound_ctrl:1\n\t"                                     \
                 "v_fmac_f32_dpp %11, %11, %16 " CTRL " row_mask:0xf bank_mask:0xf bound_ctrl:1\n\t"                                     \
                 "v_fmac_f32_dpp %12, %12, %16 " CTRL " row_mask:0xf bank_mask:0xf bound_ctrl:1\n\t"                                     \
                 "v_fmac_f32_dpp %13, %13, %16 " CTRL " row_mask:0xf bank_mask:0xf bound_ctrl:1\n\t"                                     \
                 "v_fmac_f32_dpp %14, %14, %16 " CTRL " row_mask:0xf bank_mask:0xf bound_ctrl:1\n\t"                                     \
                 "v_fmac_f32_dpp %15, %15, %16 " CTRL " row_mask:0xf bank_mask:0xf bound_ctrl:1"                                          \
                 : "+v"(v[0]), "+v"(v[1]), "+v"(v[2]), "+v"(v[3]), "+v"(v[4]), "+v"(v[5]), "+v"(v[6]), "+v"(v[7]), "+v"(v[8]), "+v"(v[9]),   \
                   "+v"(v[10]), "+v"(v[11]), "+v"(v[12]), "+v"(v[13]), "+v"(v[14]), "+v"(v[15])                                           \
                 : "v"(k))
#endif
__device__ __forceinline__ void gb_run_sum16(float (&v)[16], const GbRun &run) {
#ifdef FOC_GB_MERGE_SELECT
#pragma unroll
    for (int i = 0; i < 16; i++) v[i] = gb_run_sum(v[i], run);
#else
    float k;
    if (__builtin_amdgcn_ballot_w64(run.f0 == 0u) != 0ull) {
        k = run.k0; GB_FMAC16("row_shr:1");
        if (__builtin_amdgcn_ballot_w64(run.f1 == 0u) != 0ull) {
            k = run.k1; GB_FMAC16("row_shr:2");
            if (__builtin_amdgcn_ballot_w64(run.f2 == 0u) != 0ull) {
                k = run.k2; GB_FMAC16("row_shr:4");
                if (__builtin_amdgcn_ballot_w64(run.f3 == 0u) != 0ull) { k = run.k3; GB_FMAC16("row_shr:8"); }
            }
        }
    }
#endif
}

#define GB_PM_TILE 1024u
#define GB_PMS_WG 1024u

__global__ void __launch_bounds__(256) k_gbin_scans(GbHeader *__restrict__ hdr, uint32_t *__restrict__ wg_hist, uint32_t n_wg, uint32_t L) {
    __shared__ uint32_t s_wave[2][4];
    const uint32_t lane = threadIdx.x & 63, wave = threadIdx.x >> 6;
    const uint32_t n = L * GB_MAX_SEGS;
    if (blockIdx.x == n) {
        const uint32_t per = (n + 255) / 256;
        const uint32_t lo = threadIdx.x * per, hi = min(n, lo + per);
        uint32_t recs = 0, chks = 0;
        for (uint32_t i = lo; i < hi; i++) { const uint32_t c = hdr->counts[i]; recs += c; chks += (c + GB_CHUNK - 1) / GB_CHUNK; }
        const uint32_t ir = (uint32_t)wave_incl_sum_i((int)recs, (int)lane), ic = (uint32_t)wave_incl_sum_i((int)chks, (int)lane);
        if (lane == 63) { s_wave[0][wave] = ir; s_wave[1][wave] = ic; }
        __syncthreads();
        uint32_t r = ir - recs, k = ic - chks;
        for (uint32_t w = 0; w < wave; w++) { r += s_wave[0][w]; k += s_wave[1][w]; }
        for (uint32_t i = lo; i < hi; i++) {
            const uint32_t c = hdr->counts[i];
            hdr->base[i] = r; hdr->chunk_prefix[i] = k;
            r += c; k += (c + GB_CHUNK - 1) / GB_CHUNK;
        }
        if (threadIdx.x == 255) { hdr->base[n] = r; hdr->chunk_prefix[n] = k; }
        return;
    }
    const uint32_t slot = blockIdx.x;
    uint32_t *col = wg_hist + (uint64_t)slot * n_wg;
    const uint32_t per = (n_wg + 255) / 256;
    const uint32_t lo = min(n_wg, threadIdx.x * per), hi = min(n_wg, lo + per);
    uint32_t local = 0;
    for (uint32_t i = lo; i < hi; i++) local += col[i];
    const uint32_t incl = (uint32_t)wave_incl_sum_i((int)local, (int)lane);
    if (lane == 63) s_wave[0][wave] = incl;
    __syncthreads();
    uint32_t run = incl - local;
    for (uint32_t k = 0; k < wave; k++) run += s_wave[0][k];
    for (uint32_t i = lo; i < hi; i++) { const uint32_t c = col[i]; col[i] = run; run += c; }
}

template <uint32_t THREADS>
__device__ __forceinline__ void gb_count_tile(uint32_t *hist, uint32_t tile, uint32_t n_wg, const float *__restrict__ inputs, const int32_t *__restrict__ offsets,
                                              GbHeader *__restrict__ hdr, uint32_t *__restrict__ wg_hist, uint32_t B, uint32_t L, const GeLevels &lv,
                                              uint32_t gridtype, bool align_corners, uint32_t interp, uint32_t l_begin, uint32_t l_end) {
    static_assert(GB_PM_TILE % THREADS == 0 && THREADS % 64 == 0, "whole waves, whole tile");
    const uint32_t slot_lo = l_begin * GB_MAX_SEGS, slot_hi = l_end * GB_MAX_SEGS;
    for (uint32_t i = slot_lo + threadIdx.x; i < slot_hi; i += THREADS) hist[i] = 0;
    __syncthreads();
    for (uint32_t it = 0; it < GB_PM_TILE / THREADS; it++) {
        const uint32_t b = tile * GB_PM_TILE + it * THREADS + threadIdx.x;
        float x[3] = {0.f, 0.f, 0.f};
        const bool inside = b < B && !ge_load_point<3>(inputs, b, x);
        for (uint32_t level = l_begin; level < l_end; level++) {
            const uint32_t resolution = lv.resolution[level];
            uint32_t pg[3]; float pf[3];
            gb_cell<3>(x, lv.scale[level], align_corners, interp, pg, pf);
            bool emit = inside;
            if (resolution <= lv.merge_max_res) emit = gb_run_flags(inside, pg).tail;
            if (emit) {
                const uint32_t hashmap_size = (uint32_t)offsets[level + 1] - (uint32_t)offsets[level];
                uint32_t rows[8];
                bool hashed;
                ge_rows3(pg, hashmap_size, resolution, gridtype, align_corners, rows, &hashed);
                if (hashed) {
#pragma unroll
                    for (int j = 0; j < 4; j++) atomicAdd(&hist[level * GB_MAX_SEGS + (rows[2 * j] >> GB_SEG_SHIFT)], 1u);
                } else {
#pragma unroll
                    for (int j = 0; j < 4; j++) {
                        const uint32_t s0 = rows[2 * j] >> GB_SEG_SHIFT, s1 = rows[2 * j + 1] >> GB_SEG_SHIFT;
                        atomicAdd(&hist[level * GB_MAX_SEGS + s0], 1u);
                        if (s0 != s1) atomicAdd(&hist[level * GB_MAX_SEGS + s1], 1u);
                    }
                }
            }
        }
    }
    __syncthreads();
    for (uint32_t i = slot_lo + threadIdx.x; i < slot_hi; i += THREADS) {
        const uint32_t hcount = hist[i];
        if (hcount) (void)__hip_atomic_fetch_add(&hdr->counts[i], hcount, __ATOMIC_RELAXED, __HIP_MEMORY_SCOPE_AGENT);
        wg_hist[(uint64_t)i * n_wg + tile] = hcount;
    }
}

__global__ void __launch_bounds__(GB_PMS_WG) k_gbin_count_pt(const float *__restrict__ inputs, const int32_t *__restrict__ offsets, GbHeader *__restrict__ hdr,
                                                             uint32_t *__restrict__ wg_hist, uint32_t B, uint32_t L, GeLevels lv, uint32_t gridtype,
                                                             bool align_corners, uint32_t interp) {
    __shared__ uint32_t hist[GE_MAX_LEVELS * GB_MAX_SEGS];
    gb_count_tile<GB_PMS_WG>(hist, blockIdx.x, gridDim.x, inputs, offsets, hdr, wg_hist, B, L, lv, gridtype, align_corners, interp, 0u, L);
}

template <typename T>
__global__ void __launch_bounds__(256) k_grid_fwd_counted(const float *__restrict__ inputs, const T *__restrict__ grid, const int32_t *__restrict__ offsets,
                                                          T *__restrict__ outputs, uint32_t B, uint32_t L, GeLevels lv, uint32_t gridtype, bool align_corners,
                                                          uint32_t interp, uint32_t chunks, uint32_t pairs, GbHeader *__restrict__ hdr,
                                                          uint32_t *__restrict__ wg_hist, uint32_t n_tiles, uint32_t period, uint32_t w0, uint32_t lc, uint32_t csplit) {
    __shared__ uint32_t hist[GE_MAX_LEVELS * GB_MAX_SEGS];
    const uint32_t n_count = n_tiles * csplit;
    uint32_t f = blockIdx.x;
    if (blockIdx.x >= w0) {
        const uint32_t g = blockIdx.x - w0, q = g / period, r = g - q * period;
        if (r == period - 1u && q < n_count) {
            const uint32_t part = q % csplit;
            gb_count_tile<256>(hist, q / csplit, n_tiles, inputs, offsets, hdr, wg_hist, B, L, lv, gridtype, align_corners, interp, (part * L) / csplit, ((part + 1u) * L) / csplit);
            return;
        }
        f = blockIdx.x - min(q, n_count);
    }
    uint32_t chunk, l0, l1;
    ge_walk(f, chunks, lc, chunk, l0, l1);
// ... 580 lines not shown
    ge_make_levels(L, S, H, lv);
    hipStream_t st = (hipStream_t)stream;
    if (dtype == FOC_F32) return ge_forward_d<float>(D, C, inputs, embeddings, offsets, outputs, B, L, lv, dy_dx, gridtype, align_corners != 0, interp, bl, st);
    return ge_forward_d<__half>(D, C, inputs, embeddings, offsets, outputs, B, L, lv, dy_dx, gridtype, align_corners != 0, interp, bl, st);
}

template <typename T, uint32_t D, uint32_t C>
static int ge_backward_launch(const void *grad, const float *inputs, const int32_t *offsets, void *grad_emb, uint32_t B, uint32_t L,
                              const GeLevels &lv, const void *dy_dx, void *grad_inputs, uint32_t gridtype, bool ac, uint32_t interp,
                              bool bl, hipStream_t st) {
    const uint32_t chunks = foc_div_up(B, 256);
    if (bl) hipLaunchKernelGGL((k_grid_bwd<T, D, C, true>), dim3(ge_xcd_grid(chunks, L)), dim3(256), 0, st, (const T *)grad, inputs, offsets,
                               (T *)grad_emb, B, L, lv, gridtype, ac, interp, chunks);
    else hipLaunchKernelGGL((k_grid_bwd<T, D, C, false>), dim3(ge_xcd_grid(chunks, L)), dim3(256), 0, st, (const T *)grad, inputs, offsets,
                            (T *)grad_emb, B, L, lv, gridtype, ac, interp, chunks);
    FOC_CHECK_LAUNCH("grid_encode_backward");
    if (dy_dx && grad_inputs) {
        const uint32_t g = foc_grid_1d((uint64_t)B * D, 256);
        if (bl) hipLaunchKernelGGL((k_grid_input_bwd<T, D, C, true>), dim3(g), dim3(256), 0, st, (const T *)grad, (const T *)dy_dx, (T *)grad_inputs, B, L);
        else hipLaunchKernelGGL((k_grid_input_bwd<T, D, C, false>), dim3(g), dim3(256), 0, st, (const T *)grad, (const T *)dy_dx, (T *)grad_inputs, B, L);
        FOC_CHECK_LAUNCH("grid_encode_backward(inputs)");
    }
    return FOC_OK;
}

template <typename T, uint32_t D>
static int ge_backward_c(uint32_t C, const void *grad, const float *inputs, const int32_t *offsets, void *grad_emb, uint32_t B, uint32_t L,
                         const GeLevels &lv, const void *dy_dx, void *grad_inputs, uint32_t gridtype, bool ac, uint32_t interp, bool bl,
                         hipStream_t st) {
    switch (C) {
        case 1: return ge_backward_launch<T, D, 1>(grad, inputs, offsets, grad_emb, B, L, lv, dy_dx, grad_inputs, gridtype, ac, interp, bl, st);
        case 2: return ge_backward_launch<T, D, 2>(grad, inputs, offsets, grad_emb, B, L, lv, dy_dx, grad_inputs, gridtype, ac, interp, bl, st);
        case 4: return ge_backward_launch<T, D, 4>(grad, inputs, offsets, grad_emb, B, L, lv, dy_dx, grad_inputs, gridtype, ac, interp, bl, st);
        case 8: return ge_backward_launch<T, D, 8>(grad, inputs, offsets, grad_emb, B, L, lv, dy_dx, grad_inputs, gridtype, ac, interp, bl, st);
        default: foc_set_error("GridEncoding: C must be 1, 2, 4, or 8."); return FOC_E_INVALID;
    }
}

template <typename T, uint32_t D, uint32_t C>
static int ge_tv_launch(const void *inputs, const void *emb, void *grad, const int32_t *offsets, float weight, uint32_t B, uint32_t L,
                        const GeLevels &lv, uint32_t gridtype, bool ac, hipStream_t st) {
    const uint32_t chunks = foc_div_up(B, 256);
    hipLaunchKernelGGL((k_grad_tv<T, D, C>), dim3(ge_xcd_grid(chunks, L)), dim3(256), 0, st, (const T *)inputs, (const T *)emb, (T *)grad, offsets,
                       weight, B, L, lv, gridtype, ac, chunks);
    FOC_CHECK_LAUNCH("grad_total_variation");
    return FOC_OK;
}

template <typename T, uint32_t D>
static int ge_tv_c(uint32_t C, const void *inputs, const void *emb, void *grad, const int32_t *offsets, float weight, uint32_t B, uint32_t L,
                   const GeLevels &lv, uint32_t gridtype, bool ac, hipStream_t st) {
    switch (C) {
        case 1: return ge_tv_launch<T, D, 1>(inputs, emb, grad, offsets, weight, B, L, lv, gridtype, ac, st);
        case 2: return ge_tv_launch<T, D, 2>(inputs, emb, grad, offsets, weight, B, L, lv, gridtype, ac, st);
        case 4: return ge_tv_launch<T, D, 4>(inputs, emb, grad, offsets, weight, B, L, lv, gridtype, ac, st);
        case 8: return ge_tv_launch<T, D, 8>(inputs, emb, grad, offsets, weight, B, L, lv, gridtype, ac, st);
        default: foc_set_error("GridEncoding: C must be 1, 2, 4, or 8."); return FOC_E_INVALID;
    }
}


static uint64_t gb_max_recs(uint32_t B, uint32_t L) { return (uint64_t)B * 5u * L; }
static uint64_t gb_rec_array_bytes(uint64_t m, int dtype) { return ((m + 3) & ~(uint64_t)3) * 4 + m * (dtype == FOC_F16 ? 8 : 16); }
static uint64_t gb_workspace_bytes(uint32_t B, uint32_t L, int dtype) {
    const uint64_t hdr = (sizeof(GbHeader) + 255) & ~(uint64_t)255;
    const uint64_t m = gb_max_recs(B, L);
    const uint64_t wg = (uint64_t)foc_div_up(B, GB_PM_TILE) * L * GB_MAX_SEGS * 4;
    return hdr + gb_rec_array_bytes(m, dtype) + 256 + wg + 256;
}
static uint64_t gb_recs_bytes(uint32_t B, uint32_t L, int dtype) {
    const uint64_t m = gb_max_recs(B, L);
    return (gb_rec_array_bytes(m, dtype) + 255) & ~(uint64_t)255;
}

static int gb_count(const float *inputs, const int32_t *offsets, uint32_t B, uint32_t L, const GeLevels &lv, uint32_t gridtype, bool ac, uint32_t interp,
                    int dtype, void *workspace, hipStream_t st) {
    GbHeader *hdr = reinterpret_cast<GbHeader *>(workspace);
    void *recs = reinterpret_cast<char *>(workspace) + ((sizeof(GbHeader) + 255) & ~(uint64_t)255);
    if (foc_zero_async(hdr->counts, sizeof(hdr->counts), st) != hipSuccess) { foc_set_error("grid_encode_backward: memset failed"); return FOC_E_LAUNCH; }
    const uint32_t n_wg = foc_div_up(B, GB_PM_TILE);
    uint32_t *wg_hist = reinterpret_cast<uint32_t *>(reinterpret_cast<char *>(recs) + gb_recs_bytes(B, L, dtype));
    hipLaunchKernelGGL(k_gbin_count_pt, dim3(n_wg), dim3(GB_PMS_WG), 0, st, inputs, offsets, hdr, wg_hist, B, L, lv, gridtype, ac, interp);
    FOC_CHECK_LAUNCH("grid_encode_backward(count)");
    hipLaunchKernelGGL(k_gbin_scans, dim3(L * GB_MAX_SEGS + 1), dim3(256), 0, st, hdr, wg_hist, n_wg, L);
    FOC_CHECK_LAUNCH("grid_encode_backward(scans)");
    return FOC_OK;
}

template <typename T>
static int gb_forward_counted(const float *inputs, const void *emb, const int32_t *offsets, void *outputs, uint32_t B, uint32_t L, const GeLevels &lv,
                              uint32_t gridtype, bool ac, uint32_t interp, void *workspace, hipStream_t st) {
    GbHeader *hdr = reinterpret_cast<GbHeader *>(workspace);
    void *recs = reinterpret_cast<char *>(workspace) + ((sizeof(GbHeader) + 255) & ~(uint64_t)255);
    if (foc_zero_async(hdr->counts, sizeof(hdr->counts), st) != hipSuccess) { foc_set_error("grid_encode_forward_counted: memset failed"); return FOC_E_LAUNCH; }
    const uint32_t n_tiles = foc_div_up(B, GB_PM_TILE), chunks = foc_div_up(B, 256);
    const uint32_t lc = ge_small_levels(L, lv);
    const uint32_t groups = lc >= 2u ? L - lc + 1u : L;
    const uint32_t fwd_blocks = chunks * groups;
    const uint32_t lo = groups >= 4 ? groups / 2 : 0, hi = groups >= 4 ? groups - 1 : groups;
    const uint32_t csplit = L >= 4u ? 4u : 1u, n_count = n_tiles * csplit;
    const uint32_t w0 = lo * chunks, fit = ((hi - lo) * chunks) / n_count + 1u, period = (fit & 1u) ? fit : fit - 1u;
    uint32_t *wg_hist = reinterpret_cast<uint32_t *>(reinterpret_cast<char *>(recs) + gb_recs_bytes(B, L, sizeof(T) == 2 ? FOC_F16 : FOC_F32));
    hipLaunchKernelGGL((k_grid_fwd_counted<T>), dim3(fwd_blocks + n_count), dim3(256), 0, st, inputs, (const T *)emb, offsets, (T *)outputs, B, L, lv, gridtype, ac,
                       interp, chunks, sizeof(T) == 2 ? ge_pairs_mode(emb, nullptr, sizeof(T), 3, 2, gridtype, ac, interp) : 0u, hdr, wg_hist, n_tiles, period, w0, lc, csplit);
    FOC_CHECK_LAUNCH("grid_encode_forward_counted");
    hipLaunchKernelGGL(k_gbin_scans, dim3(L * GB_MAX_SEGS + 1), dim3(256), 0, st, hdr, wg_hist, n_tiles, L);
    FOC_CHECK_LAUNCH("grid_encode_forward_counted(scans)");
    return FOC_OK;
}

static uint32_t gb_fact_mask(uint32_t L, const GeLevels &lv, const int32_t *offsets_host, uint32_t gridtype, bool ac, int dtype) {
    const int on = foc_opt(FOC_OPT_GB_FACTORED);
    if (!on || dtype != FOC_F16 || gridtype != 0u) return 0u;
    uint32_t m = 0;
    for (uint32_t l = 0; l < L && l < 32u; l++) {
        const uint32_t size = (uint32_t)(offsets_host[l + 1] - offsets_host[l]);
        const uint32_t r1 = ac ? lv.resolution[l] : lv.resolution[l] + 1u;
        uint32_t stride = 1u;
        for (int d = 0; d < 3; d++) if (stride <= size) stride *= r1;
        const bool hashed = stride > size;
        if (hashed && (size & (size - 1u)) == 0u && size >= GB_SEG && lv.resolution[l] > lv.merge_max_res) m |= 1u << l;
    }
    return m;
}

static uint32_t gb_scatter_resident(size_t elem) {
    static uint32_t cus[16];
    int dev = 0;
    if (hipGetDevice(&dev) != hipSuccess || dev < 0 || dev >= 16) dev = 0;
    if (!cus[dev]) {
        int n = 0;
        if (hipDeviceGetAttribute(&n, hipDeviceAttributeMultiprocessorCount, dev) != hipSuccess || n <= 0) n = 256;
        cus[dev] = (uint32_t)n;
    }
    return cus[dev] * (elem == 2 ? 2u : 1u);
}

template <typename T>
static int gb_run(const void *grad, const float *inputs, const int32_t *offsets, void *grad_emb, uint32_t B, uint32_t L, const GeLevels &lv,
                  uint32_t gridtype, bool ac, uint32_t interp, bool bl, void *workspace, bool counted, uint32_t fact_mask, const GbSizes &sz, hipStream_t st) {
    GbHeader *hdr = reinterpret_cast<GbHeader *>(workspace);
    void *recs = reinterpret_cast<char *>(workspace) + ((sizeof(GbHeader) + 255) & ~(uint64_t)255);
    const uint64_t max_recs = gb_max_recs(B, L);
    const uint32_t n_tiles = foc_div_up(B, GB_PM_TILE);
    uint32_t *wg_hist = reinterpret_cast<uint32_t *>(reinterpret_cast<char *>(recs) + gb_recs_bytes(B, L, sizeof(T) == 2 ? FOC_F16 : FOC_F32));
    if (!counted) {
        const int rc = gb_count(inputs, offsets, B, L, lv, gridtype, ac, interp, sizeof(T) == 2 ? FOC_F16 : FOC_F32, workspace, st);
        if (rc) return rc;
    }
    const uint32_t resident = gb_scatter_resident(sizeof(T));
    const uint32_t n_tail = n_tiles % resident, n_whole = n_tiles - n_tail;
    uint32_t split = 1u;
    const uint32_t split_max = (uint32_t)max(1, foc_opt(FOC_OPT_GB_TAIL_SPLIT));
    while (n_tail && split * 2u <= L && n_tail * split * 2u <= resident && split * 2u <= split_max) split *= 2u;
    hipLaunchKernelGGL((k_gbin_scatter_pms<T>), dim3(n_whole + n_tail * split), dim3(GB_PMS_WG), 0, st, (const T *)grad, inputs, offsets, hdr, wg_hist, recs, max_recs, B, L, lv,
                       gridtype, ac, interp, bl, fact_mask, sz, n_tiles, n_whole, split);
    FOC_CHECK_LAUNCH("grid_encode_backward(scatter)");
    const uint32_t ub = (uint32_t)(((uint64_t)B * 5u * L + GB_CHUNK - 1) / GB_CHUNK) + L * GB_MAX_SEGS;
    hipLaunchKernelGGL((k_gbin_reduce<T>), dim3(ub), dim3(GB_RTHREADS), 0, st, hdr, recs, max_recs, offsets, (T *)grad_emb, L, fact_mask);
    FOC_CHECK_LAUNCH("grid_encode_backward(reduce)");
    return FOC_OK;
}

extern "C" {

int foc_grid_encode_forward(const float *inputs, const void *embeddings, const int32_t *offsets, void *outputs, uint32_t B, uint32_t D,
                            uint32_t C, uint32_t L, float S, uint32_t H, void *dy_dx, uint32_t gridtype, int align_corners,
                            uint32_t interp, int dtype, const int32_t *offsets_host, void *stream) {
    FocDeviceGuard foc_guard_(stream, inputs);
    (void)offsets_host;
    return ge_forward(inputs, embeddings, offsets, outputs, B, D, C, L, S, H, dy_dx, gridtype, align_corners, interp, dtype, false, stream);
}

int foc_grid_encode_forward_bl(const float *inputs, const void *embeddings, const int32_t *offsets, void *outputs, uint32_t B, uint32_t D,
                               uint32_t C, uint32_t L, float S, uint32_t H, void *dy_dx, uint32_t gridtype, int align_corners,
                               uint32_t interp, int dtype, const int32_t *offsets_host, void *stream) {
    FocDeviceGuard foc_guard_(stream, inputs);
    (void)offsets_host;
    return ge_forward(inputs, embeddings, offsets, outputs, B, D, C, L, S, H, dy_dx, gridtype, align_corners, interp, dtype, true, stream);
}

int foc_grid_forward_index_path(uint32_t level_rows, uint32_t resolution, uint32_t level_offset_rows) {
    if (((level_offset_rows | level_rows) & 1u) != 0u) return 0;
    uint32_t st1, st2;
    const bool hashed = ge_level_hashed(level_rows, resolution, st1, st2);
    if (!ge_hash3_admits(level_rows, hashed)) return 0;
    return level_rows <= (1u << 22) ? 2 : 1;
}

// ... 194 lines not shown
```

### focnerf_amd/field.py

```python
import os
from dataclasses import dataclass
from typing import Optional

import torch
from torch.autograd import Function
from torch.amp import custom_bwd, custom_fwd

from .backend import _gridencoder, _ffmlp
from .ffmlp import FFMLP, PackedMLP, single_pass_backward
from .gridencoder import GridEncoder, GridSpec


def fused_mlp(model, name):
    get = getattr(model, "fused_mlp", None)
    return get(name) if get is not None else getattr(model, name, None)


@dataclass(frozen=True)
class MlpShape:
    input_dim: int
    hidden_dim: int
    num_layers: int
    activation: int
    output_activation: int
    padded_output_dim: int

    @staticmethod
    def of(mlp):
        if not isinstance(mlp, (FFMLP, PackedMLP)):
            return None
        return MlpShape(mlp.input_dim, mlp.hidden_dim, mlp.num_layers, mlp.activation, mlp.output_activation, mlp.padded_output_dim)

    def blob_numel(self):
        return self.hidden_dim * (self.input_dim + self.hidden_dim * (self.num_layers - 1) + self.padded_output_dim)


@dataclass(frozen=True)
class FieldPlan:
    grid: Optional[GridSpec]
    levels: int
    sigma: Optional[MlpShape]
    colour: Optional[MlpShape]
    uses_object_feature: bool
    field: bool
    train_forward: bool
    tail: bool
    infer: bool
    occ: bool
    native_loop: bool
    head: bool
    colour_input_pad: float = 0.0
    background: bool = False


def pad_twin(name, pad, obj):
    from ._lib import lib
    if pad == 0:
        return getattr(lib, name), ()
    return getattr(lib, name + ("_pad" if obj else "_pad31")), (float(pad),)


def _on(switch):
    return os.environ.get(switch, "1") != "0"


def field_plan(model):
    from ._lib import get_option
    from .shencoder import SHEncoder
    enc, enc_dir = getattr(model, "encoder", None), getattr(model, "encoder_dir", None)
    sigma, colour = MlpShape.of(fused_mlp(model, "sigma_net")), MlpShape.of(fused_mlp(model, "color_net"))
    obj = bool(getattr(model, "uses_object_feature", False))
    pad = float(getattr(model, "colour_input_pad", 0.0))
    grid = enc.spec() if isinstance(enc, GridEncoder) else None

    hash_grid = grid is not None and enc.input_dim == 3 and enc.level_dim == 2 and sigma is not None and sigma.input_dim == enc.output_dim
    plain_grid = grid is not None and grid.gridtype == 0 and not grid.align_corners and grid.interpolation == 0
    sigma_one_pass = sigma is not None and single_pass_backward(sigma.input_dim, sigma.hidden_dim, sigma.num_layers, sigma.activation)
    sigma_16 = sigma is not None and sigma.padded_output_dim == 16
    sigma_32_64 = sigma is not None and sigma.input_dim == 32 and sigma.hidden_dim == 64
    colour_in = 48 if obj else 32
    colour_64 = colour is not None and colour.input_dim == colour_in and colour.hidden_dim == 64 and colour.padded_output_dim == 16
    colour_rows = (isinstance(enc_dir, SHEncoder) and enc_dir.degree == 4 and getattr(model, "geo_feat_dim", 0) == 15
                   and (not obj or getattr(model, "yolo_encoding_dim", 0) == 16))
    colour_relu_or_none = colour is not None and colour.activation in (0, 6)
    both = sigma is not None and colour is not None
    same_activation = both and sigma.activation == colour.activation
    layer_pair = both and (sigma.num_layers, colour.num_layers) in ((1, 2), (1, 3), (2, 2), (2, 3), (3, 3))
    whole_field = sigma_32_64 and colour_64 and colour_rows and layer_pair and same_activation

    field = hash_grid and sigma_one_pass and sigma_16 and _on("FOC_FUSED_FIELD")
    tail = colour_64 and colour.num_layers in (2, 3) and colour_relu_or_none and colour_rows and _on("FOC_FUSED_TAIL")
    infer = field and whole_field and (not obj or sigma.activation == 0) and _on("FOC_FUSED_INFER")
    enc_bg, bg_mlp = getattr(model, "encoder_bg", None), fused_mlp(model, "bg_net")
    bg_grid = enc_bg.spec() if isinstance(enc_bg, GridEncoder) else None
    background = (bg_grid is not None and enc_bg.input_dim == 2 and enc_bg.level_dim == 2 and enc_bg.offsets.numel() == 5
                  and bg_grid.gridtype == 0 and not bg_grid.align_corners and bg_grid.interpolation == 0
                  and isinstance(bg_mlp, PackedMLP) and bg_mlp.in_features == 24 and MlpShape.of(bg_mlp) == MlpShape(32, 64, 1, 0, 6, 16)
                  and bg_mlp.output_dim == 3 and isinstance(enc_dir, SHEncoder) and enc_dir.degree == 4 and _on("FOC_FUSED_BG"))
    return FieldPlan(
        grid=grid, levels=enc.offsets.numel() - 1 if grid is not None else 0, sigma=sigma, colour=colour, uses_object_feature=obj,
        field=field, tail=tail, infer=infer,
        train_forward=(field and tail and whole_field and sigma.output_activation == 6 and get_option("FOC_FIELD_FWD_FUSED") != 0),
        occ=field and tail and not obj and (getattr(model, "bg_radius", 0) <= 0 or background) and same_activation and _on("FOC_FUSED_OCC"),
        native_loop=(infer and not obj and getattr(model, "density_scale", 1) == 1 and plain_grid and _on("FOC_RENDER_NATIVE")),
        head=both and colour.input_dim == colour_in and colour_rows and pad == 0 and _on("FOC_FUSED_HEAD"), colour_input_pad=pad,
        background=background)


def _raw_stream_of(device):
    from ._lib import raw_stream
    return raw_stream(device.index if device.index is not None else torch.cuda.current_device())


_half_scope = None


class half_cache_scope:

    def __enter__(self):
        global _half_scope
        self._outer = _half_scope
        if _half_scope is None:
            _half_scope = {}
        return self

    def __exit__(self, *exc):
        global _half_scope
        _half_scope = self._outer
        return False


def _half_of(param):
    if param.dtype == torch.half:
        return param.contiguous()
    if _half_scope is None:
        return param.detach().to(torch.half).contiguous()
    hit = _half_scope.get(id(param))
    if hit is not None and hit[0] is param and hit[1].device == param.device:
        if hit[2] is not None and _raw_stream_of(param.device) != hit[3]:
            torch.cuda.current_stream(param.device).wait_event(hit[2])
        return hit[1]
    h = param.detach().to(torch.half).contiguous()
    ev = st = None
    if h.is_cuda:
        st = _raw_stream_of(h.device)
        ev = torch.cuda.Event()
        ev.record(torch.cuda.current_stream(h.device))
    _half_scope[id(param)] = (param, h, ev, st)
    return h


def scope_cached(key, owner, make):
    if _half_scope is None:
        return make()
    hit = _half_scope.get(key)
    if hit is not None and hit[0] is owner:
        if hit[2] is not None and _raw_stream_of(hit[1].device) != hit[3]:
            torch.cuda.current_stream(hit[1].device).wait_event(hit[2])
        return hit[1]
    v = make()
    ev = st = None
    if v.is_cuda:
        st = _raw_stream_of(v.device)
        ev = torch.cuda.Event()
        ev.record(torch.cuda.current_stream(v.device))
    _half_scope[key] = (owner, v, ev, st)
    return v


def _check_colour_branch(colour, B):
    cweights, shape, ray_sh, T, c_width, obj_feat = colour[:6]
    T = int(T)
    if not (ray_sh.dtype == torch.half and ray_sh.dim() == 2 and ray_sh.shape[1] == 16 and ray_sh.is_contiguous() and T > 0
            and B == ray_sh.shape[0] * T):
        raise RuntimeError(f"hashgrid_mlp colour branch: ray_sh must be a contiguous half [B / T, 16] tensor with B = {B}, T = {T}; got "
                           f"{tuple(ray_sh.shape)} {ray_sh.dtype}{'' if ray_sh.is_contiguous() else ' (strided)'}")
    if c_width not in (4, 16):
        raise RuntimeError(f"hashgrid_mlp colour branch: c_width must be 4 or 16, got {c_width}")
    if shape.input_dim not in (32, 48) or (obj_feat is not None) != (shape.input_dim == 48) or (obj_feat is not None and obj_feat.numel() != 16):
        raise RuntimeError(f"hashgrid_mlp colour branch: a {shape.input_dim}-wide colour input takes "
                           f"{'a 16-element object feature' if shape.input_dim == 48 else 'no object feature'}, got "
                           f"{'none' if obj_feat is None else f'{obj_feat.numel()} elements'}")
    if cweights.numel() != 64 * (shape.input_dim + 64 * (shape.num_layers - 1) + 16):
        raise RuntimeError(f"hashgrid_mlp colour branch: the colour weights hold {cweights.numel()} elements, a {shape.input_dim}-wide "
                           f"{shape.num_layers}-layer network has {64 * (shape.input_dim + 64 * (shape.num_layers - 1) + 16)}")


class _hashgrid_mlp(Function):
    @staticmethod
    @custom_fwd(device_type="cuda")
    def forward(ctx, x, embeddings, weights, offsets, grid, sigma, training, colour=None):
        x = x.contiguous().float()
        B = x.shape[0]
        if colour is not None:
            _check_colour_branch(colour, B)
        S, H, (gridtype, align_corners, interp) = grid.log2_scale, grid.base_resolution, grid.tail()
        L = offsets.shape[0] - 1
        emb = _half_of(embeddings)
        w = _half_of(weights)
        enc = torch.empty(L, B, 2, device=x.device, dtype=torch.half)
        ticket = _gridencoder.grid_encode_forward_counted(x, emb, offsets, enc, B, 3, 2, L, S, H, gridtype, align_corners, interp,
                                                          standalone=_gridencoder.precount_standalone()) if training else None
        if ticket is None:
            _gridencoder.grid_encode_forward(x, emb, offsets, enc, B, 3, 2, L, S, H, None, gridtype, align_corners, interp)
        h = torch.empty(B, 16, device=x.device, dtype=torch.half)
        c = None
        if colour is not None:
            from ._lib import ptr, stream_of, check
            cweights, cshape, ray_sh, T, c_width, obj_feat = colour[:6]
            pad = float(colour[6]) if len(colour) > 6 else 0.0
            wc = _half_of(cweights)
            obj16 = obj_feat.detach().reshape(-1).half().contiguous() if obj_feat is not None else None
            c = torch.empty(B, c_width, device=x.device, dtype=torch.half)
            args = (ptr(enc), ptr(w), sigma.num_layers, ptr(ray_sh), int(T), ptr(wc), int(cshape.num_layers), 64, int(sigma.activation), B, ptr(h),
                    ptr(c), int(c_width), ptr(obj16))
            fn, extra = pad_twin("foc_field_forward_train", pad, obj16 is not None)
            check(fn(*args, *extra, stream_of(enc)), "field_forward_train")
        else:
            _ffmlp.ffmlp_forward_planar(enc, w, B, sigma.input_dim, 16, sigma.hidden_dim, sigma.num_layers, sigma.activation, sigma.output_activation, h)
        if training:
            ctx.save_for_backward(x, emb, w, offsets, enc)
            ctx.cfg = (grid, sigma, B, L)
            ctx.ticket = ticket
        if c is None:
            return h
        ctx.mark_non_differentiable(c)
        ctx.set_materialize_grads(False)
        return h, c

    @staticmethod
    @custom_bwd(device_type="cuda")
    def backward(ctx, grad_h, _grad_c=None):
        x, emb, w, offsets, enc = ctx.saved_tensors
        grid, sigma, B, L = ctx.cfg
        if grad_h is None:
            return (None,) * 8
        grad_h = grad_h.contiguous().half()
        g_enc = torch.empty_like(enc)
        g_w = torch.empty_like(w)
        _ffmlp.ffmlp_backward_planar(grad_h, enc, w, B, sigma.input_dim, 16, sigma.hidden_dim, sigma.num_layers, sigma.activation,
                                     sigma.output_activation, True, g_enc, g_w)
        g_emb = torch.zeros_like(emb)
        _gridencoder.grid_encode_backward(g_enc, x, emb, offsets, g_emb, B, 3, 2, L, grid.log2_scale, grid.base_resolution, None, None, *grid.tail(),
                                          grad_bl=False, precount=ctx.ticket)
        return None, g_emb, g_w, None, None, None, None, None


@torch.no_grad()
def field_infer(model, xn, dirs, dir_div=1, dir_block=0, obj_feat=None):
    from ._lib import ptr, stream_of, check
    enc, sn, cn = model.encoder, fused_mlp(model, "sigma_net"), fused_mlp(model, "color_net")
    grid = enc.spec()
    xn = xn.contiguous().float()
    dirs = dirs.contiguous().float()
    M = xn.shape[0]
    L = enc.offsets.shape[0] - 1
    emb, ws, wc = _half_of(enc.embeddings), _half_of(sn.weights), _half_of(cn.weights)
    planes = torch.empty(L, M, 2, device=xn.device, dtype=torch.half)
    _gridencoder.grid_encode_forward(xn, emb, enc.offsets, planes, M, 3, 2, L, grid.log2_scale, grid.base_resolution, None, *grid.tail())
    sigma = torch.empty(M, dtype=torch.float32, device=xn.device)
    rgb = torch.empty(M, 3, dtype=torch.float32, device=xn.device)
    obj16 = None
    if getattr(model, "uses_object_feature", False):
        if obj_feat is None:
            raise RuntimeError("field_infer: an object-conditioned network needs its encoded object feature")
        obj16 = obj_feat.detach().reshape(-1).half().contiguous()
        assert obj16.numel() == 16
    args = (ptr(planes), 1, ptr(dirs), int(dir_div), int(dir_block), dirs.shape[0], ptr(ws), sn.num_layers, ptr(wc), cn.num_layers, 64, sn.activation, M,
            ptr(sigma), ptr(rgb), ptr(obj16))
    fn, extra = pad_twin("foc_nerf_field_inference", float(getattr(model, "colour_input_pad", 0.0)), obj16 is not None)
    check(fn(*args, *extra, stream_of(xn)), "nerf_field_inference")
    return sigma, rgb


def hashgrid_mlp(encoder, mlp, x, bound=1, colour=None):
    prefix = list(x.shape[:-1])
    xn = (x if bound is None else (x + bound) / (2 * bound)).view(-1, 3)
    h = _hashgrid_mlp.apply(xn, encoder.embeddings, mlp.weights, encoder.offsets, encoder.spec(), MlpShape.of(mlp), mlp.training and torch.is_grad_enabled(),
                            colour)
    if colour is not None:
        h, c = h
        return h.view(prefix + [16]), c
    return h.view(prefix + [16])
```

### focnerf_amd/fixedstep.py

```python
import torch
from torch.autograd import Function

from . import raymarching
from ._lib import lib, ptr, stream_of, check
from .gridencoder import grid_encode


RAY_BLOCK = 64


def ray_block_default():
    import os
    return RAY_BLOCK if os.environ.get("FOC_RAY_BLOCK", str(RAY_BLOCK)) != "0" else 0


def blocked_rows(N, T, ray_block):
    return N * T if not ray_block else -(-N // ray_block) * ray_block * T


def fixed_sample(rays_o, rays_d, nears, fars, aabb, noise, T, bound, want_xyzs=False, want_ray_sh=False, ray_block=0):
    N = rays_o.shape[0]
    dev = rays_o.device
    rows = blocked_rows(N, T, ray_block)
    enc_in = torch.empty(rows, 3, dtype=torch.float32, device=dev)
# ... 20 lines not shown
    def forward(ctx, h, rays_d, nears, fars, noise, N, T, density_scale, obj_feat=None):
        h = h.contiguous()
        assert h.dtype == torch.float16 and h.shape == (N * T, 16)
        dev = h.device
        M = N * T
        sigma = torch.empty(M, dtype=torch.float32, device=dev)
        trans = torch.empty(M, dtype=torch.float32, device=dev)
        weights = torch.empty(M, dtype=torch.float32, device=dev)
        ws = torch.empty(N, dtype=torch.float32, device=dev)
        depth = torch.empty(N, dtype=torch.float32, device=dev)
        width = 32 if obj_feat is None else 48
        if obj_feat is not None:
            obj_feat = obj_feat.detach().reshape(-1).half().contiguous()
            assert obj_feat.numel() == 16
        cin = torch.empty(M, width, dtype=torch.float16, device=dev)
        check(lib.foc_fixed_head_forward(ptr(h), ptr(rays_d), ptr(nears), ptr(fars), ptr(noise), N, T, float(density_scale), ptr(sigma), ptr(trans),
                                         ptr(weights), ptr(ws), ptr(depth), ptr(cin), ptr(obj_feat), width, stream_of(h)), "fixed_head_forward")
        ctx.save_for_backward(h, sigma, trans, nears, fars, noise if noise is not None else torch.empty(0, device=dev))
        ctx.has_noise = noise is not None
        ctx.dims = (N, T, float(density_scale))
        ctx.width = width
        ctx.mark_non_differentiable(sigma)
        ctx.set_materialize_grads(False)
        return weights, ws, depth, sigma, cin

    @staticmethod
    def backward(ctx, g_weights, g_ws, g_depth, g_sigma, g_cin):
        h, sigma, trans, nears, fars, noise = ctx.saved_tensors
        N, T, ds = ctx.dims
        noise = noise if ctx.has_noise else None
        g_weights = g_weights.contiguous().float() if g_weights is not None else None
        g_ws = g_ws.contiguous().float() if g_ws is not None else None
        g_depth = g_depth.contiguous().float() if g_depth is not None else None
        g_cin = g_cin.contiguous().half() if g_cin is not None else None
        grad_h = torch.empty_like(h)
        check(lib.foc_fixed_head_backward(ptr(h), ptr(sigma), ptr(trans), ptr(nears), ptr(fars), ptr(noise), ptr(g_weights), ptr(g_ws), ptr(g_depth),
                                          ptr(g_cin), N, T, ds, ptr(grad_h), ctx.width, stream_of(h)), "fixed_head_backward")
        g_obj = None
        if ctx.width == 48 and ctx.needs_input_grad[8] and g_cin is not None:
            g_obj = g_cin[:, 31:47].float().sum(0)
        return grad_h, None, None, None, None, None, None, None, g_obj


class _fixed_composite(Function):

    @staticmethod
    def forward(ctx, c, weights, bg_ray, bg_scalar, N, T, thresh, weights_sum=None):
        c = c.contiguous()
        weights = weights.contiguous()
        assert c.dtype == torch.float16 and c.shape == (N * T, 16) and weights.dtype == torch.float32
        image = torch.empty(N, 3, dtype=torch.float32, device=c.device)
        check(lib.foc_fixed_composite_forward(ptr(c), ptr(weights), ptr(bg_ray), float(bg_scalar), N, T, float(thresh), ptr(image), stream_of(c)),
              "fixed_composite_forward")
        ctx.bg_grad = bg_ray is not None and ctx.needs_input_grad[2]
        if ctx.bg_grad and weights_sum is None:
            raise RuntimeError("_fixed_composite: a background that needs a gradient needs weights_sum")
        empty = torch.empty(0, device=c.device)
        ctx.save_for_backward(c, weights, bg_ray if bg_ray is not None else empty, weights_sum.detach() if ctx.bg_grad else empty)
        ctx.has_bg = bg_ray is not None
        ctx.dims = (N, T, float(thresh), float(bg_scalar))
        return image

    @staticmethod
    def backward(ctx, g_image):
        c, weights, bg_ray, weights_sum = ctx.saved_tensors
        N, T, thresh, bg_scalar = ctx.dims
        bg_ray = bg_ray if ctx.has_bg else None
        g_image = g_image.contiguous().float()
        grad_c = torch.empty_like(c)
        grad_w = torch.empty_like(weights)
        check(lib.foc_fixed_composite_backward(ptr(g_image), ptr(c), ptr(weights), ptr(bg_ray), bg_scalar, N, T, thresh, ptr(grad_c), ptr(grad_w),
                                               stream_of(c)), "fixed_composite_backward")
        g_bg = g_image * (1 - weights_sum).unsqueeze(-1) if ctx.bg_grad else None
        return grad_c, grad_w, g_bg, None, None, None, None, None


_C_WIDTH = 4


class _render_tail(Function):

    @staticmethod
    def forward(ctx, h, cweights, ray_sh, nears, fars, noise, bg_ray, bg_scalar, N, T, density_scale, thresh, num_layers, activation, obj_feat=None,
                want_sumsq=False, c_pre=None, w16_pre=None, input_pad=0.0):
        from .field import _half_of, pad_twin
        h = h.contiguous()
        assert h.dtype == torch.float16 and h.shape == (N * T, 16)
        assert ray_sh.dtype == torch.float16 and ray_sh.shape == (N, 16) and ray_sh.is_contiguous()
        dev, M = h.device, N * T
        st = stream_of(h)
        w16 = w16_pre if w16_pre is not None else _half_of(cweights)
        obj16 = None
        if obj_feat is not None:
            obj16 = obj_feat.detach().reshape(-1).half().contiguous()
            assert obj16.numel() == 16 and w16.numel() == 64 * (48 + 64 * (int(num_layers) - 1) + 16)
        if c_pre is not None:
            assert c_pre.dtype == torch.float16 and c_pre.shape == (M, _C_WIDTH) and c_pre.is_contiguous()
            c = c_pre
        else:
            c = torch.empty(M, _C_WIDTH, dtype=torch.float16, device=dev)
            args = (ptr(h), ptr(ray_sh), T, ptr(w16), M, 64, int(num_layers), int(activation), ptr(c), _C_WIDTH, ptr(obj16))
            fn, extra = pad_twin("foc_color_head_forward", input_pad, obj16 is not None)
            check(fn(*args, *extra, st), "color_head_forward")
        sigma = torch.empty(M, dtype=torch.float32, device=dev)
        trans = torch.empty(M, dtype=torch.float32, device=dev)
        weights = torch.empty(M, dtype=torch.float32, device=dev)
        ws = torch.empty(N, dtype=torch.float32, device=dev)
        depth = torch.empty(N, dtype=torch.float32, device=dev)
        image = torch.empty(N, 3, dtype=torch.float32, device=dev)
        sumsq = torch.empty(N, dtype=torch.float32, device=dev) if want_sumsq else None
        check(lib.foc_fixed_tail_forward(ptr(h), ptr(c), ptr(nears), ptr(fars), ptr(noise), ptr(bg_ray), float(bg_scalar), N, T, float(density_scale),
                                         float(thresh), ptr(sigma), ptr(trans), ptr(weights), ptr(ws), ptr(depth), ptr(image), _C_WIDTH, ptr(sumsq), st),
              "fixed_tail_forward")
        empty = torch.empty(0, device=dev)
        ctx.bg_grad = bg_ray is not None and ctx.needs_input_grad[6]
        ctx.save_for_backward(h, w16, sigma, trans, weights, c, ray_sh, nears, fars, noise if noise is not None else empty,
                              bg_ray if bg_ray is not None else empty, obj16 if obj16 is not None else empty, ws if ctx.bg_grad else empty)
        ctx.flags = (noise is not None, bg_ray is not None, obj16 is not None, obj_feat.dtype if obj_feat is not None else None,
                     tuple(obj_feat.shape) if obj_feat is not None else None)
        ctx.dims = (N, T, float(density_scale), float(thresh), float(bg_scalar), int(num_layers), int(activation), float(input_pad))
        ctx.mark_non_differentiable(sigma, weights, c)
        ctx.set_materialize_grads(False)
        if want_sumsq:
            return image, ws, depth, sigma, weights, c, sumsq
        return image, ws, depth, sigma, weights, c

    @staticmethod
    def backward(ctx, g_image, g_ws, g_depth, _g_sigma, _g_weights, _g_c, g_sumsq=None):
        from .backend import _scratch
        from .field import pad_twin
        h, w16, sigma, trans, weights, c, ray_sh, nears, fars, noise, bg_ray, obj16, ws = ctx.saved_tensors
        has_noise, has_bg, has_obj, obj_dtype, obj_shape = ctx.flags
        obj16 = obj16 if has_obj else None
        N, T, ds, thresh, bg_scalar, num_layers, activation, input_pad = ctx.dims
        noise = noise if has_noise else None
        bg_ray = bg_ray if has_bg else None
        dev, M = h.device, N * T
        st = stream_of(h)
        g_image = g_image.contiguous().float() if g_image is not None else torch.zeros(N, 3, dtype=torch.float32, device=dev)
        g_ws = g_ws.contiguous().float() if g_ws is not None else None
        g_depth = g_depth.contiguous().float() if g_depth is not None else None
        g_sumsq = g_sumsq.contiguous().float() if g_sumsq is not None else None
        grad_c = torch.empty_like(c)
        grad_h0 = torch.empty(M, dtype=torch.float16, device=dev)
        check(lib.foc_fixed_tail_backward(ptr(g_image), ptr(g_ws), ptr(g_depth), ptr(c), ptr(sigma), ptr(trans), ptr(weights), ptr(nears), ptr(fars),
                                          ptr(noise), ptr(bg_ray), bg_scalar, N, T, ds, thresh, ptr(grad_c), ptr(grad_h0), _C_WIDTH, ptr(g_sumsq), st),
              "fixed_tail_backward")
        grad_h = torch.empty_like(h)
        g_w = torch.empty_like(w16)
        wsb = _scratch.get("ffmlp_ws", lib.foc_ffmlp_backward_workspace_bytes(48 if has_obj else 32, 64, num_layers), dev)
        g_obj32 = torch.empty(16, dtype=torch.float32, device=dev) if has_obj and ctx.needs_input_grad[14] else None
        args = (ptr(grad_c), ptr(h), ptr(ray_sh), T, ptr(grad_h0), ptr(w16), M, 64, num_layers, activation, ptr(grad_h), ptr(g_w), ptr(wsb),
                wsb.numel(), _C_WIDTH, ptr(obj16), ptr(g_obj32))
        fn, extra = pad_twin("foc_color_head_backward", input_pad, has_obj)
        check(fn(*args, *extra, st), "color_head_backward")
        g_obj = g_obj32.to(obj_dtype).view(obj_shape) if g_obj32 is not None else None
        g_bg = g_image * (1 - ws).unsqueeze(-1) if ctx.bg_grad else None
        return (grad_h, g_w, None, None, None, None, g_bg) + (None,) * 7 + (g_obj, None, None, None, None)


class _masked_norm(Function):

    @staticmethod
    def forward(ctx, sumsq, outside):
        crit = torch.sqrt((sumsq * outside).sum())
        ctx.save_for_backward(crit, outside)
        return crit

    @staticmethod
    def backward(ctx, g):
        crit, outside = ctx.saved_tensors
        coef = torch.where(crit > 0, g / (2 * crit), torch.zeros_like(crit))
        return outside * coef, None


def _background(bg_color, N, dev):
    if bg_color is None:
        return None, 1.0
    if torch.is_tensor(bg_color):
        if bg_color.numel() > 1:
            return bg_color.to(dev, torch.float32).expand(N, 3).contiguous(), 0.0
        return None, float(bg_color)
    return None, float(bg_color)


def render_fixed_steps(model, rays_o, rays_d, yolo_details=None, num_steps=512, bg_color=None, perturb=False, weight_thresh=1e-10,
                       return_fields=None, _out=None, **kwargs):
    import time
    if return_fields is None:
        return_fields = not model.training
    t_start = time.time()
    prefix = rays_o.shape[:-1]
    rays_o = rays_o.contiguous().view(-1, 3).float()
    rays_d = rays_d.contiguous().view(-1, 3).float()
    N, T = rays_o.shape[0], int(num_steps)
    dev = rays_o.device
    aabb = model.aabb_train if model.training else model.aabb_infer
    nears, fars = raymarching.near_far_from_aabb(rays_o, rays_d, aabb, model.min_near)
    noise = torch.rand(N * T, dtype=torch.float32, device=dev) if perturb else None
    from .field import field_plan, field_infer
    plan = field_plan(model)
    if getattr(model, "bg_radius", 0) > 0:
        bg_color = model._background_colour(rays_o, rays_d, bg_color)
    want_tail = plan.tail and model.training and torch.is_grad_enabled()
    fused_infer = not torch.is_grad_enabled() and plan.infer
    rb = ray_block_default() if fused_infer else 0
    enc_in, _, ray_sh = fixed_sample(rays_o, rays_d, nears, fars, aabb, noise, T, model.bound, want_ray_sh=True) if want_tail else \
        fixed_sample(rays_o, rays_d, nears, fars, aabb, noise, T, model.bound, ray_block=rb) + (None,)

    if fused_infer:
        obj_feat = model.encode_object_feature(yolo_details, dev) if plan.uses_object_feature else None
        sigma, rgb = field_infer(model, enc_in, rays_d, dir_div=T, dir_block=rb, obj_feat=obj_feat)
        bg_ray, bg_scalar = _background(bg_color, N, dev)
        direct = (_out is not None and _out[0].dtype == torch.float32 and _out[1].dtype == torch.float32 and _out[0].is_contiguous()
                  and _out[1].is_contiguous() and _out[0].numel() == N and _out[1].numel() == 3 * N and _out[0].device == dev)
        depth, image = (_out[0].view(N), _out[1].view(N, 3)) if direct else (torch.empty(N, dtype=torch.float32, device=dev),
                                                                              torch.empty(N, 3, dtype=torch.float32, device=dev))
        weights_sum = torch.empty(N, dtype=torch.float32, device=dev)
        rgb_masked = densities = None
        if return_fields:
            if direct and len(_out) == 4 and all(t.dtype == torch.float32 and t.is_contiguous() and t.device == dev for t in _out[2:]) \
                    and _out[2].numel() == N * T and _out[3].numel() == 3 * N * T and rb:
                densities, rgb_masked = _out[2].view(N * T), _out[3].view(N * T, 3)
            else:
                rgb_masked = torch.empty(N * T, 3, dtype=torch.float32, device=dev)
                densities = torch.empty(N * T, dtype=torch.float32, device=dev) if rb else None
        check(lib.foc_fixed_render_inference(ptr(sigma), ptr(rgb), ptr(nears), ptr(fars), ptr(noise), ptr(bg_ray), float(bg_scalar), N, T,
                                             float(model.density_scale), float(weight_thresh), ptr(image), ptr(depth), ptr(weights_sum), ptr(rgb_masked),
                                             rb, ptr(densities), stream_of(sigma)), "fixed_render_inference")
        t_mid = time.time()
        results = {'depth': depth.view(*prefix), 'image': image.view(*prefix, 3), 'weights_sum': weights_sum, 'criterion_outside_mask': None,
                   'timing': [t_mid - t_start, time.time() - t_mid]}
        if return_fields:
            results['densities'] = (densities if rb else sigma).view(N, T, 1)
            results['rgbs'] = rgb_masked.view(N, T, 3)
        return results

    enc = model.encoder
    from .field import hashgrid_mlp, fused_mlp
    c_pre = obj_feat = None
    cweights = fused_mlp(model, "color_net").weights if want_tail else None
    with torch.autocast("cuda", dtype=torch.float16):
        if plan.uses_object_feature:
            obj_feat = model.encode_object_feature(yolo_details, dev)
        if plan.field:
            colour = wc16 = None
            if want_tail and plan.train_forward:
                from .field import _half_of
                wc16 = _half_of(cweights)
                colour = (wc16, plan.colour, ray_sh, T, _C_WIDTH, obj_feat, plan.colour_input_pad)
            h = hashgrid_mlp(enc, fused_mlp(model, "sigma_net"), enc_in, None, colour)
            if colour is not None:
                h, c_pre = h
        else:
            feats = grid_encode(enc_in, enc.embeddings, enc.offsets, enc.per_level_scale, enc.base_resolution, False, enc.gridtype_id,
                                enc.align_corners, enc.interp_id)
            h = fused_mlp(model, "sigma_net")(feats)
        if h.shape[1] != 16:
            raise RuntimeError("render_fixed_steps expects a 16-wide sigma head (1 + geo_feat_dim = 16)")
        fused_tail = want_tail
        want_crit = model.training and yolo_details is not None and yolo_details[0] is not None
        criterion_outside_mask = None
        if fused_tail:
            cn = fused_mlp(model, "color_net")
            bg_ray, bg_scalar = _background(bg_color, N, dev)
            outs = _render_tail.apply(h, cweights, ray_sh, nears, fars, noise, bg_ray, bg_scalar, N, T, model.density_scale, weight_thresh,
                                      cn.num_layers, cn.activation, obj_feat, want_crit and yolo_details[0].numel() == N, c_pre,
                                      wc16 if c_pre is not None else None, plan.colour_input_pad)
            image, weights_sum, depth, sigma, weights, c = outs[:6]
            if len(outs) == 7:
                criterion_outside_mask = _masked_norm.apply(outs[6], (~yolo_details[0].reshape(N)).to(torch.float32))
        else:
            weights, weights_sum, depth, sigma, cin = _density_head.apply(h, rays_d, nears, fars, noise, N, T, model.density_scale, obj_feat)
            if plan.colour_input_pad != 0:
                cin = torch.cat([cin[:, :-1], cin.new_full((cin.shape[0], 1), plan.colour_input_pad)], dim=1)
        if want_crit and criterion_outside_mask is None:
            from .activation import trunc_exp
            criterion_outside_mask = torch.norm(trunc_exp(h[:, 0]).view(N, T)[~yolo_details[0].squeeze(0)] - 0)
        if not fused_tail:
            c = fused_mlp(model, "color_net").forward_padded(cin)
    t_mid = time.time()

    if not fused_tail:
        bg_ray, bg_scalar = _background(bg_color, N, dev)
        image = _fixed_composite.apply(c, weights, bg_ray, bg_scalar, N, T, weight_thresh, weights_sum)

    results = {'depth': depth.view(*prefix), 'image': image.view(*prefix, 3), 'weights_sum': weights_sum,
               'criterion_outside_mask': criterion_outside_mask, 'timing': [t_mid - t_start, time.time() - t_mid]}
    if return_fields:
        from .head import rgb_head
        c16 = c.detach()
        if c16.shape[1] != 16:
            c16 = torch.nn.functional.pad(c16, (0, 16 - c16.shape[1]))
        rgb = rgb_head(c16) * (weights > weight_thresh).unsqueeze(-1)
        results['densities'] = sigma.view(N, T, 1)
        results['rgbs'] = rgb.view(N, T, 3)
    return results


@torch.no_grad()
def render_field4(model, rays_o, rays_d, num_steps=512, weight_thresh=1e-10, yolo_details=None, out=None):
    from .field import field_plan, field_infer
    rays_o = rays_o.contiguous().view(-1, 3).float()
    rays_d = rays_d.contiguous().view(-1, 3).float()
    N, T = rays_o.shape[0], int(num_steps)
    dev = rays_o.device
    if out is None:
        out = torch.empty(N, T, 4, dtype=torch.float32, device=dev)
    assert out.shape == (N, T, 4) and out.dtype == torch.float32 and out.is_contiguous()
    plan = field_plan(model)
    if plan.infer and model.bg_radius <= 0:
        aabb = model.aabb_train if model.training else model.aabb_infer
        nears, fars = raymarching.near_far_from_aabb(rays_o, rays_d, aabb, model.min_near)
        rb = ray_block_default()
        enc_in, _ = fixed_sample(rays_o, rays_d, nears, fars, aabb, None, T, model.bound, ray_block=rb)
        obj_feat = model.encode_object_feature(yolo_details, dev) if plan.uses_object_feature else None
        sigma, rgb = field_infer(model, enc_in, rays_d, dir_div=T, dir_block=rb, obj_feat=obj_feat)
        check(lib.foc_fixed_field_pack(ptr(sigma), ptr(rgb), ptr(nears), ptr(fars), None, None, 1.0, N, T, float(model.density_scale),
                                       float(weight_thresh), None, None, None, ptr(out), rb, stream_of(sigma)), "fixed_field_pack")
        return out
    from .combine import pack_field4
    with torch.autocast("cuda", dtype=torch.float16):
        res = model.run(rays_o[None], rays_d[None], yolo_details, num_steps=T, upsample_steps=0, perturb=False, weight_thresh=weight_thresh,
                        return_fields=True)
    out.copy_(pack_field4(res['densities'], res['rgbs']))
    return out
```

### include/focnerf.h

```cpp
#ifndef FOCNERF_H
#define FOCNERF_H

#include <stdint.h>

#ifdef __cplusplus
extern "C" {
#endif

#define FOC_OK            0
#define FOC_E_INVALID     1
#define FOC_E_DTYPE       2
#define FOC_E_LAUNCH      3

#define FOC_F32 0
#define FOC_F16 1

#define FOC_ABI_VERSION 2
int         foc_abi_version(void);
const char *foc_last_error(void);
int foc_set_option(const char *name, int value);
int foc_get_option(const char *name, int *value);
int foc_guard_pick_device(int stream_is_null, int stream_device, int pointer_device, int current_device);
const char *foc_arch(void);

// ... 131 lines not shown
                             const int32_t *offsets, float weight,
                             uint32_t B, uint32_t D, uint32_t C, uint32_t L, float S, uint32_t H,
                             uint32_t gridtype, int align_corners, int dtype, void *stream);


int foc_freq_encode_forward(const float *inputs, uint32_t B, uint32_t D, uint32_t deg, uint32_t C,
                            float *outputs, void *stream);
int foc_freq_encode_backward(const float *grad, const float *outputs, uint32_t B, uint32_t D,
                             uint32_t deg, uint32_t C, float *grad_inputs, void *stream);


int foc_ffmlp_forward(const void *inputs, const void *weights, uint32_t B, uint32_t input_dim,
                      uint32_t output_dim, uint32_t hidden_dim, uint32_t num_layers,
                      uint32_t activation, uint32_t output_activation,
                      void *forward_buffer, void *outputs, void *stream);

int foc_ffmlp_inference(const void *inputs, const void *weights, uint32_t B, uint32_t input_dim,
                        uint32_t output_dim, uint32_t hidden_dim, uint32_t num_layers,
                        uint32_t activation, uint32_t output_activation,
                        void *inference_buffer, void *outputs, void *stream);

int foc_ffmlp_backward(const void *grad, const void *inputs, const void *weights,
                       const void *forward_buffer, uint32_t B, uint32_t input_dim,
                       uint32_t output_dim, uint32_t hidden_dim, uint32_t num_layers,
                       uint32_t activation, uint32_t output_activation, int calc_grad_inputs,
                       void *backward_buffer, void *grad_inputs, void *grad_weights,
                       void *workspace, uint64_t workspace_bytes, void *stream);
uint64_t foc_ffmlp_backward_workspace_bytes(uint32_t input_dim, uint32_t hidden_dim, uint32_t num_layers);

int foc_ffmlp_forward_planar(const void *inputs_planar, const void *weights, uint32_t B, uint32_t input_dim,
                             uint32_t output_dim, uint32_t hidden_dim, uint32_t num_layers,
                             uint32_t activation, uint32_t output_activation, void *outputs, void *stream);
int foc_ffmlp_backward_planar(const void *grad, const void *inputs_planar, const void *weights, uint32_t B,
                              uint32_t input_dim, uint32_t output_dim, uint32_t hidden_dim, uint32_t num_layers,
                              uint32_t activation, uint32_t output_activation, int calc_grad_inputs,
                              void *grad_inputs_planar, void *grad_weights, void *workspace, uint64_t workspace_bytes, void *stream);

int foc_nerf_field_inference(const void *enc, int enc_planar, const float *dirs, uint32_t dir_div,
                             uint32_t dir_block, uint32_t n_dirs, const void *sigma_weights, uint32_t sigma_layers, const void *color_weights,
                             uint32_t color_layers, uint32_t hidden_dim, uint32_t activation, uint32_t B,
                             float *sigma, float *rgb, const void *obj_feat, void *stream);
int foc_nerf_field_inference_pad(const void *enc, int enc_planar, const float *dirs, uint32_t dir_div,
                                 uint32_t dir_block, uint32_t n_dirs, const void *sigma_weights, uint32_t sigma_layers, const void *color_weights,
                                 uint32_t color_layers, uint32_t hidden_dim, uint32_t activation, uint32_t B,
                                 float *sigma, float *rgb, const void *obj_feat, float input_pad, void *stream);
int foc_nerf_field_inference_pad31(const void *enc, int enc_planar, const float *dirs, uint32_t dir_div,
                                   uint32_t dir_block, uint32_t n_dirs, const void *sigma_weights, uint32_t sigma_layers, const void *color_weights,
                                   uint32_t color_layers, uint32_t hidden_dim, uint32_t activation, uint32_t B,
                                   float *sigma, float *rgb, const void *obj_feat, float input_pad, void *stream);

int foc_color_head_forward(const void *h, const void *ray_sh, uint32_t samples_per_ray, const void *weights,
                           uint32_t B, uint32_t hidden_dim, uint32_t num_layers, uint32_t activation,
                           void *outputs, uint32_t out_width, const void *obj_feat, void *stream);
int foc_color_head_backward(const void *grad, const void *h, const void *ray_sh, uint32_t samples_per_ray,
                            const void *grad_h0, const void *weights, uint32_t B, uint32_t hidden_dim,
                            uint32_t num_layers, uint32_t activation, void *grad_h, void *grad_weights,
                            void *workspace, uint64_t workspace_bytes, uint32_t out_width, const void *obj_feat, float *grad_obj, void *stream);
int foc_color_head_forward_pad(const void *h, const void *ray_sh, uint32_t samples_per_ray, const void *weights,
                               uint32_t B, uint32_t hidden_dim, uint32_t num_layers, uint32_t activation,
                               void *outputs, uint32_t out_width, const void *obj_feat, float input_pad, void *stream);
int foc_color_head_backward_pad(const void *grad, const void *h, const void *ray_sh, uint32_t samples_per_ray,
                                const void *grad_h0, const void *weights, uint32_t B, uint32_t hidden_dim,
                                uint32_t num_layers, uint32_t activation, void *grad_h, void *grad_weights,
                                void *workspace, uint64_t workspace_bytes, uint32_t out_width, const void *obj_feat, float *grad_obj,
                                float input_pad, void *stream);
int foc_color_head_forward_pad31(const void *h, const void *ray_sh, uint32_t samples_per_ray, const void *weights,
                                 uint32_t B, uint32_t hidden_dim, uint32_t num_layers, uint32_t activation,
                                 void *outputs, uint32_t out_width, const void *obj_feat, float input_pad, void *stream);
int foc_color_head_backward_pad31(const void *grad, const void *h, const void *ray_sh, uint32_t samples_per_ray,
                                  const void *grad_h0, const void *weights, uint32_t B, uint32_t hidden_dim,
                                  uint32_t num_layers, uint32_t activation, void *grad_h, void *grad_weights,
                                  void *workspace, uint64_t workspace_bytes, uint32_t out_width, const void *obj_feat, float *grad_obj,
                                  float input_pad, void *stream);

int foc_field_forward_train(const void *planes, const void *sigma_weights, uint32_t sigma_layers, const void *ray_sh, uint32_t samples_per_ray,
                            const void *color_weights, uint32_t color_layers, uint32_t hidden_dim, uint32_t activation, uint32_t B,
                            void *h, void *c, uint32_t out_width, const void *obj_feat, void *stream);
int foc_field_forward_train_pad(const void *planes, const void *sigma_weights, uint32_t sigma_layers, const void *ray_sh, uint32_t samples_per_ray,
                                const void *color_weights, uint32_t color_layers, uint32_t hidden_dim, uint32_t activation, uint32_t B,
                                void *h, void *c, uint32_t out_width, const void *obj_feat, float input_pad, void *stream);
int foc_field_forward_train_pad31(const void *planes, const void *sigma_weights, uint32_t sigma_layers, const void *ray_sh, uint32_t samples_per_ray,
                                  const void *color_weights, uint32_t color_layers, uint32_t hidden_dim, uint32_t activation, uint32_t B,
                                  void *h, void *c, uint32_t out_width, const void *obj_feat, float input_pad, void *stream);

int foc_allocate_splitk(uint64_t size);
int foc_free_splitk(void);


int foc_combine_select(const float *dens, const float *rgb, float *max_dens, float *best_rgb,
                       uint64_t n, void *stream);

int foc_combine_pack_keys(const float *dens, uint32_t rank, uint64_t *keys, uint64_t n, void *stream);
int foc_combine_unpack(const uint64_t *keys, uint32_t rank, const float *rgb,
                       float *max_dens, float *masked_rgb, uint64_t n, void *stream);

int foc_composite_fixed_steps(const float *sigmas, const float *rgbs, const float *nears,
                              const float *fars, uint32_t N, uint32_t T, float bg,
                              float *image4, float *depth, void *stream);

int foc_combine_select_composite(const float *const *fields4, uint32_t K, const float *nears, const float *fars,
                                 uint32_t N, uint32_t T, const float *bgs, uint32_t n_bg, float *image4, float *depth,
                                 float *merged4, void *stream);

int foc_combine_select4(const float *field4, float *acc4, uint64_t n, void *stream);

int foc_mo_select(const void *sigma_new, const void *feat_new, void *sigma_best, void *feat_best, uint64_t n,
                  uint32_t feat_width, uint32_t elem_bytes, void *stream);


int foc_fixed_sample(const float *rays_o, const float *rays_d, const float *nears, const float *fars,
                     const float *aabb, const float *noise, uint32_t N, uint32_t T, float bound,
                     float *xyzs, float *enc_in, void *ray_sh, uint32_t ray_block, void *stream);

int foc_fixed_head_forward(const void *h, const float *rays_d, const float *nears, const float *fars,
                           const float *noise, uint32_t N, uint32_t T, float density_scale,
                           float *sigma, float *trans, float *weights, float *weights_sum, float *depth,
                           void *cin, const void *obj_feat, uint32_t cin_width, void *stream);
int foc_fixed_head_backward(const void *h, const float *sigma, const float *trans, const float *nears,
                            const float *fars, const float *noise, const float *grad_w, const float *grad_ws,
                            const float *grad_depth, const void *grad_cin, uint32_t N, uint32_t T,
                            float density_scale, void *grad_h, uint32_t cin_width, void *stream);

int foc_fixed_tail_forward(const void *h, const void *c, const float *nears, const float *fars, const float *noise,
                           const float *bg_ray, float bg_scalar, uint32_t N, uint32_t T, float density_scale, float thresh,
                           float *sigma, float *trans, float *weights, float *weights_sum, float *depth, float *image,
                           uint32_t c_width, float *ray_sumsq, void *stream);
int foc_fixed_tail_backward(const float *grad_image, const float *grad_ws, const float *grad_depth, const void *c,
                            const float *sigma, const float *trans, const float *weights, const float *nears,
                            const float *fars, const float *noise, const float *bg_ray, float bg_scalar, uint32_t N,
                            uint32_t T, float density_scale, float thresh, void *grad_c, void *grad_h0, uint32_t c_width,
                            const float *grad_sumsq, void *stream);

int foc_occ_tail_forward(const void *h, const void *c, uint32_t c_width, const float *deltas, const int32_t *rays,
                         uint32_t M, uint32_t N, float T_thresh, float density_scale, const float *bg_ray, float bg_scalar,
                         const float *nears, const float *fars, float *weights_sum, float *image_raw, float *image,
                         float *depth, void *stream);
int foc_occ_tail_backward(const float *grad_image, const float *grad_ws, const void *h, const void *c, uint32_t c_width,
                          const float *deltas, const int32_t *rays, const int32_t *counter, const float *weights_sum,
                          const float *image_raw, uint32_t M, uint32_t N, float T_thresh, float density_scale,
                          const float *bg_ray, float bg_scalar, void *grad_c, void *grad_h0, void *stream);

typedef struct FocOccTrainNode {
    uint32_t struct_bytes;
    uint32_t n_rays, max_steps, cascade, grid_size, cap, pad_align;
    float bound, dt_gamma, min_near;
    const float *rays_o, *rays_d, *aabb, *jitter;
    const uint8_t *bitfield;
    float *nears, *fars, *enc_in, *deltas;
    void *sh_rows;
    int32_t *rays, *counter, *march_scratch;
    uint32_t levels, base_resolution, gridtype, interp;
    int32_t align_corners, table_dtype;
    float per_level_scale_log2;
    const void *embeddings;
    const int32_t *offsets, *offsets_host;
    void *planes, *grid_workspace;
    uint64_t grid_workspace_bytes;
    uint32_t sigma_input_dim, sigma_hidden, sigma_layers, sigma_activation, sigma_output_activation;
    uint32_t color_hidden, color_layers, color_activation, c_width;
    const void *w_sigma, *w_color;
    void *h, *c;
    float T_thresh, density_scale, bg_scalar;
    const float *bg_ray;
    float *weights_sum, *image_raw, *image, *depth;
    int32_t precounted;
    const float *grad_image, *grad_ws;
    void *grad_c, *grad_h0, *grad_h, *grad_planes, *grad_w_color, *grad_w_sigma, *grad_embeddings, *mlp_workspace;
    uint64_t mlp_workspace_bytes;
} FocOccTrainNode;
int foc_occ_train_forward(const FocOccTrainNode *node, void *stream);
int foc_occ_train_backward(const FocOccTrainNode *node, void *stream);
int foc_occ_train_forward_pad31(const FocOccTrainNode *node, float input_pad, void *stream);
int foc_occ_train_backward_pad31(const FocOccTrainNode *node, float input_pad, void *stream);

int foc_view_tile_order(const float *rays_d, uint32_t N, uint32_t tile_h, uint32_t tile_w, int64_t *perm, void *state16,
                        void *stream);

int foc_fixed_composite_forward(const void *c, const float *weights, const float *bg_ray, float bg_scalar,
                                uint32_t N, uint32_t T, float thresh, float *image, void *stream);
int foc_fixed_composite_backward(const float *grad_image, const void *c, const float *weights,
                                 const float *bg_ray, float bg_scalar, uint32_t N, uint32_t T, float thresh,
                                 void *grad_c, float *grad_w, void *stream);

int foc_fixed_render_inference(const float *sigma, const float *rgb, const float *nears, const float *fars,
                               const float *noise, const float *bg_ray, float bg_scalar, uint32_t N, uint32_t T,
                               float density_scale, float thresh, float *image, float *depth, float *weights_sum,
                               float *rgb_masked, uint32_t ray_block, float *sigma_raymajor, void *stream);

int foc_fixed_field_pack(const float *sigma, const float *rgb, const float *nears, const float *fars,
                         const float *noise, const float *bg_ray, float bg_scalar, uint32_t N, uint32_t T,
                         float density_scale, float thresh, float *image, float *depth, float *weights_sum,
                         float *field4, uint32_t ray_block, void *stream);


int foc_sample_head_forward(const void *h, const float *dirs, uint64_t M, float *sigma, void *cin,
                            const void *obj_feat, uint32_t cin_width, void *stream);
int foc_sample_head_backward(const void *h, const float *grad_sigma, const void *grad_cin, uint64_t M,
                             void *grad_h, uint32_t cin_width, void *stream);
int foc_sh_encode(const float *dirs, uint64_t M, float *out, void *stream);
int foc_rgb_head_forward(const void *c, uint64_t M, float *rgb, void *stream);
int foc_rgb_head_backward(const void *c, const float *grad_rgb, uint64_t M, void *grad_c, void *stream);


int foc_mark_untrained_grid(const float *poses, uint32_t B, float fx, float fy, float cx, float cy, float bound,
                            uint32_t cascade, uint32_t H, float *density_grid, int32_t *count, void *stream);
int foc_grid_cells_xyz(uint32_t cascade, uint32_t H, float bound, const float *jitter, float *xyzs, void *stream);
uint64_t foc_grid_update_sample_workspace_bytes(uint32_t cascade, uint32_t H);
int foc_grid_update_sample(const float *density_grid, uint32_t cascade, uint32_t H, float bound, uint32_t N,
                           const int32_t *rand_coords, const float *rand_pick, const float *jitter,
// ... 20 lines not shown
```

Baseline: 1.371 billion.

## Emit compact density logits, add wave-per-ray sampler and wide grid scan

The fused field forward kernel now also writes the first column of h (the density logit) into a compact fp16 buffer. A new tail-forward entry point reads that compact buffer instead of striding through the full 16-wide h rows. Separately, a wave-per-ray fixed-step sampling kernel that stages positions in shared memory is added, along with a wide grid-backward scan; both are behind new options that default on. This cuts strided reads in the tail, in exchange for an extra small write and more kernel variants to maintain.

```diff
diff --git a/focnerf_amd/_lib.py b/focnerf_amd/_lib.py
--- a/focnerf_amd/_lib.py
+++ b/focnerf_amd/_lib.py
@@ -129,6 +129,7 @@
     "foc_composite_fixed_steps": (i32, [c_vp, c_vp, c_vp, c_vp, u32, u32, f32, c_vp, c_vp, c_vp]),
     "foc_fixed_sample": (i32, [c_vp, c_vp, c_vp, c_vp, c_vp, c_vp, u32, u32, f32, c_vp, c_vp, c_vp, u32, c_vp]),
     "foc_fixed_tail_forward": (i32, [c_vp, c_vp, c_vp, c_vp, c_vp, c_vp, f32, u32, u32, f32, f32, c_vp, c_vp, c_vp, c_vp, c_vp, c_vp, u32, c_vp, c_vp]),
+    "foc_fixed_tail_forward_h0": (i32, [c_vp, c_vp, c_vp, c_vp, c_vp, c_vp, f32, u32, u32, f32, f32, c_vp, c_vp, c_vp, c_vp, c_vp, c_vp, u32, c_vp, c_vp]),
     "foc_fixed_tail_backward": (i32, [c_vp, c_vp, c_vp, c_vp, c_vp, c_vp, c_vp, c_vp, c_vp, c_vp, c_vp, f32, u32, u32, f32, f32, c_vp, c_vp, u32, c_vp, c_vp]),
     "foc_fixed_head_forward": (i32, [c_vp, c_vp, c_vp, c_vp, c_vp, u32, u32, f32, c_vp, c_vp, c_vp, c_vp, c_vp, c_vp, c_vp, u32, c_vp]),
     "foc_fixed_head_backward": (i32, [c_vp, c_vp, c_vp, c_vp, c_vp, c_vp, c_vp, c_vp, c_vp, c_vp, u32, u32, f32, c_vp, u32, c_vp]),
@@ -141,6 +142,9 @@
     "foc_color_head_forward_pad31": (i32, [c_vp, c_vp, u32, c_vp, u32, u32, u32, u32, c_vp, u32, c_vp, f32, c_vp]),
     "foc_color_head_backward_pad31": (i32, [c_vp, c_vp, c_vp, u32, c_vp, c_vp, u32, u32, u32, u32, c_vp, c_vp, c_vp, u64, u32, c_vp, c_vp, f32, c_vp]),
     "foc_field_forward_train_pad31": (i32, [c_vp, c_vp, u32, c_vp, u32, c_vp, u32, u32, u32, u32, c_vp, c_vp, u32, c_vp, f32, c_vp]),
+    "foc_field_forward_train_h0": (i32, [c_vp, c_vp, u32, c_vp, u32, c_vp, u32, u32, u32, u32, c_vp, c_vp, u32, c_vp, c_vp, c_vp]),
+    "foc_field_forward_train_pad_h0": (i32, [c_vp, c_vp, u32, c_vp, u32, c_vp, u32, u32, u32, u32, c_vp, c_vp, u32, c_vp, f32, c_vp, c_vp]),
+    "foc_field_forward_train_pad31_h0": (i32, [c_vp, c_vp, u32, c_vp, u32, c_vp, u32, u32, u32, u32, c_vp, c_vp, u32, c_vp, f32, c_vp, c_vp]),
     "foc_fixed_composite_forward": (i32, [c_vp, c_vp, c_vp, f32, u32, u32, f32, c_vp, c_vp]),
     "foc_fixed_composite_backward": (i32, [c_vp, c_vp, c_vp, c_vp, f32, u32, u32, f32, c_vp, c_vp, c_vp]),
     "foc_sample_head_forward": (i32, [c_vp, c_vp, u64, c_vp, c_vp, c_vp, u32, c_vp]),
diff --git a/focnerf_amd/csrc/combine.hip b/focnerf_amd/csrc/combine.hip
--- a/focnerf_amd/csrc/combine.hip
+++ b/focnerf_amd/csrc/combine.hip
@@ -191,7 +191,7 @@
 static FocOptionRow foc_option_table[FOC_OPT_COUNT] = {
     {"FOC_MLP_BWD_FUSED", 1}, {"FOC_FIELD_FWD_FUSED", 1}, {"FOC_GB_MERGE_MAX_RES", 480}, {"FOC_GB_FACTORED", 1}, {"FOC_GB_TAIL_SPLIT", 16}, {"FOC_GRID_FUSE_SMALL", 1},
     {"FOC_GRID_PAIRS", 1}, {"FOC_GRID_FAST", 1}, {"FOC_MARCH_SERIAL", -1}, {"FOC_MARCH_RAYS_ROW_MAX", 131072}, {"FOC_OCC_MARCH_FORM", -1},
-    {"FOC_OCC_SAMPLE_MAJOR", 1}, {"FOC_OCC_FIELD_PIECE", 1 << 23},
+    {"FOC_OCC_SAMPLE_MAJOR", 1}, {"FOC_OCC_FIELD_PIECE", 1 << 23}, {"FOC_FS_SAMPLE_WAVE", 1}, {"FOC_GB_SCAN_WIDE", 1},
 };
 static int foc_option_parse(int which, const char *text) {
     if (which == FOC_OPT_OCC_MARCH_FORM) {
diff --git a/focnerf_amd/csrc/common.h b/focnerf_amd/csrc/common.h
--- a/focnerf_amd/csrc/common.h
+++ b/focnerf_amd/csrc/common.h
@@ -24,6 +24,8 @@
     FOC_OPT_OCC_MARCH_FORM,
     FOC_OPT_OCC_SAMPLE_MAJOR,
     FOC_OPT_OCC_FIELD_PIECE,
+    FOC_OPT_FS_SAMPLE_WAVE,
+    FOC_OPT_GB_SCAN_WIDE,
     FOC_OPT_COUNT
 };
 int foc_opt(FocOpt which);
diff --git a/focnerf_amd/csrc/field_fwd.hip b/focnerf_amd/csrc/field_fwd.hip
--- a/focnerf_amd/csrc/field_fwd.hip
+++ b/focnerf_amd/csrc/field_fwd.hip
@@ -14,7 +14,7 @@
 template <int NLS, int NLC, bool RELU>
 __global__ void __launch_bounds__(MLP_BLOCK, FF_MIN_WAVES) k_field_fwd_train(const _Float16 *__restrict__ planes, const _Float16 *__restrict__ w_sigma,
                                                                const _Float16 *__restrict__ w_color, _Float16 *__restrict__ h_out,
-                                                               _Float16 *__restrict__ c_out, uint32_t B, MlpHead hd) {
+                                                               _Float16 *__restrict__ c_out, uint32_t B, MlpHead hd, _Float16 *__restrict__ h0_out) {
     constexpr int HIDDEN = 64, MT = 2, KC = 4, KS0 = 2;
     constexpr int FS = MT * KS0 + (NLS - 1) * MT * KC + KC;
     constexpr int FC = MT * KS0 + (NLC - 1) * MT * KC + KC;
@@ -92,6 +92,7 @@
 #endif
             *reinterpret_cast<ff_u2 *>(h_out + row_raw * 16 + 4 * h) = ff_u2{P0, P1};
             *reinterpret_cast<ff_u2 *>(h_out + row_raw * 16 + 8 + 4 * h) = ff_u2{P2, P3};
+            if (h0_out && h == 0) h0_out[row_raw] = __builtin_bit_cast(_Float16, (uint16_t)P0);
         }
         const uint32_t nxt = h == 0 ? P2 : 0u;
         const ff_u2 s02 = __builtin_amdgcn_permlane32_swap(P0, P2, false, false);
@@ -147,7 +148,7 @@
 }
 
 template <int NLS, int NLC, bool RELU>
-static int ff_launch(const void *planes, const void *w_sigma, const void *w_color, void *h, void *c, uint32_t B, const MlpHead &hd, hipStream_t st) {
+static int ff_launch(const void *planes, const void *w_sigma, const void *w_color, void *h, void *c, uint32_t B, const MlpHead &hd, void *h0, hipStream_t st) {
     auto kern = k_field_fwd_train<NLS, NLC, RELU>;
     const size_t lds = (size_t)((4 + (NLS - 1) * 8 + 4) + (4 + (NLC - 1) * 8 + 4)) * 1024 + 256;
     if (lds > 64 * 1024) (void)hipFuncSetAttribute(reinterpret_cast<const void *>(kern), hipFuncAttributeMaxDynamicSharedMemorySize, (int)lds);
@@ -161,19 +162,19 @@
     const uint32_t cap = ff_num_cus() * (uint32_t)resident;
     if (grid > cap) grid = cap;
     hipLaunchKernelGGL(kern, dim3(grid), dim3(MLP_BLOCK), lds, st, (const _Float16 *)planes, (const _Float16 *)w_sigma, (const _Float16 *)w_color,
-                       (_Float16 *)h, (_Float16 *)c, B, hd);
+                       (_Float16 *)h, (_Float16 *)c, B, hd, (_Float16 *)h0);
     FOC_CHECK_LAUNCH("field_forward_train");
     return FOC_OK;
 }
 
 template <int NLS, int NLC>
-static int ff_launch_act(const void *planes, const void *w_sigma, const void *w_color, void *h, void *c, uint32_t B, int relu, const MlpHead &hd, hipStream_t st) {
-    return relu ? ff_launch<NLS, NLC, true>(planes, w_sigma, w_color, h, c, B, hd, st) : ff_launch<NLS, NLC, false>(planes, w_sigma, w_color, h, c, B, hd, st);
+static int ff_launch_act(const void *planes, const void *w_sigma, const void *w_color, void *h, void *c, uint32_t B, int relu, const MlpHead &hd, void *h0, hipStream_t st) {
+    return relu ? ff_launch<NLS, NLC, true>(planes, w_sigma, w_color, h, c, B, hd, h0, st) : ff_launch<NLS, NLC, false>(planes, w_sigma, w_color, h, c, B, hd, h0, st);
 }
 
 static int field_forward_train(const void *planes, const void *sigma_weights, uint32_t sigma_layers, const void *ray_sh, uint32_t samples_per_ray,
                                const void *color_weights, uint32_t color_layers, uint32_t hidden_dim, uint32_t activation, uint32_t B, void *h, void *c,
-                               uint32_t out_width, const void *obj_feat, float input_pad, bool pad31, void *stream) {
+                               uint32_t out_width, const void *obj_feat, float input_pad, bool pad31, void *h0, void *stream) {
     FocDeviceGuard foc_guard_(stream, planes);
     if (B == 0) return FOC_OK;
     FOC_REQUIRE(planes && sigma_weights && ray_sh && color_weights && h && c, FOC_E_INVALID, "field_forward_train: null pointer");
@@ -186,11 +187,11 @@
     const int relu = activation == FOC_ACT_RELU;
     hipStream_t st = (hipStream_t)stream;
     switch (sigma_layers * 10 + color_layers) {
-        case 12: return ff_launch_act<1, 2>(planes, sigma_weights, color_weights, h, c, B, relu, hd, st);
-        case 13: return ff_launch_act<1, 3>(planes, sigma_weights, color_weights, h, c, B, relu, hd, st);
-        case 22: return ff_launch_act<2, 2>(planes, sigma_weights, color_weights, h, c, B, relu, hd, st);
-        case 23: return ff_launch_act<2, 3>(planes, sigma_weights, color_weights, h, c, B, relu, hd, st);
-        case 33: return ff_launch_act<3, 3>(planes, sigma_weights, color_weights, h, c, B, relu, hd, st);
+        case 12: return ff_launch_act<1, 2>(planes, sigma_weights, color_weights, h, c, B, relu, hd, h0, st);
+        case 13: return ff_launch_act<1, 3>(planes, sigma_weights, color_weights, h, c, B, relu, hd, h0, st);
+        case 22: return ff_launch_act<2, 2>(planes, sigma_weights, color_weights, h, c, B, relu, hd, h0, st);
+        case 23: return ff_launch_act<2, 3>(planes, sigma_weights, color_weights, h, c, B, relu, hd, h0, st);
+        case 33: return ff_launch_act<3, 3>(planes, sigma_weights, color_weights, h, c, B, relu, hd, h0, st);
         default: foc_set_error("field_forward_train: layer counts (%u, %u) are not built (1/2, 1/3, 2/2, 2/3, 3/3)", sigma_layers, color_layers); return FOC_E_INVALID;
     }
 }
@@ -201,21 +202,45 @@
                             const void *color_weights, uint32_t color_layers, uint32_t hidden_dim, uint32_t activation, uint32_t B, void *h, void *c,
                             uint32_t out_width, const void *obj_feat, void *stream) {
     return field_forward_train(planes, sigma_weights, sigma_layers, ray_sh, samples_per_ray, color_weights, color_layers, hidden_dim, activation, B, h, c,
-                               out_width, obj_feat, 0.0f, false, stream);
+                               out_width, obj_feat, 0.0f, false, nullptr, stream);
 }
 
 int foc_field_forward_train_pad(const void *planes, const void *sigma_weights, uint32_t sigma_layers, const void *ray_sh, uint32_t samples_per_ray,
                                 const void *color_weights, uint32_t color_layers, uint32_t hidden_dim, uint32_t activation, uint32_t B, void *h, void *c,
                                 uint32_t out_width, const void *obj_feat, float input_pad, void *stream) {
     return field_forward_train(planes, sigma_weights, sigma_layers, ray_sh, samples_per_ray, color_weights, color_layers, hidden_dim, activation, B, h, c,
-                               out_width, obj_feat, input_pad, false, stream);
+                               out_width, obj_feat, input_pad, false, nullptr, stream);
 }
 
 int foc_field_forward_train_pad31(const void *planes, const void *sigma_weights, uint32_t sigma_layers, const void *ray_sh, uint32_t samples_per_ray,
                                   const void *color_weights, uint32_t color_layers, uint32_t hidden_dim, uint32_t activation, uint32_t B, void *h, void *c,
                                   uint32_t out_width, const void *obj_feat, float input_pad, void *stream) {
     return field_forward_train(planes, sigma_weights, sigma_layers, ray_sh, samples_per_ray, color_weights, color_layers, hidden_dim, activation, B, h, c,
-                               out_width, obj_feat, input_pad, true, stream);
-}
-
-}
+                               out_width, obj_feat, input_pad, true, nullptr, stream);
+}
+
+int foc_field_forward_train_h0(const void *planes, const void *sigma_weights, uint32_t sigma_layers, const void *ray_sh, uint32_t samples_per_ray,
+                               const void *color_weights, uint32_t color_layers, uint32_t hidden_dim, uint32_t activation, uint32_t B, void *h, void *c,
+                               uint32_t out_width, const void *obj_feat, void *h0, void *stream) {
+    FOC_REQUIRE(h0 || B == 0, FOC_E_INVALID, "field_forward_train_h0: null h0");
+    return field_forward_train(planes, sigma_weights, sigma_layers, ray_sh, samples_per_ray, color_weights, color_layers, hidden_dim, activation, B, h, c,
+                               out_width, obj_feat, 0.0f, false, h0, stream);
+}
+
+int foc_field_forward_train_pad_h0(const void *planes, const void *sigma_weights, uint32_t sigma_layers, const void *ray_sh, uint32_t samples_per_ray,
+                                   const void *color_weights, uint32_t color_layers, uint32_t hidden_dim, uint32_t activation, uint32_t B, void *h, void *c,
+                                   uint32_t out_width, const void *obj_feat, float input_pad, void *h0, void *stream) {
+    FOC_REQUIRE(h0 || B == 0, FOC_E_INVALID, "field_forward_train_pad_h0: null h0");
+    return field_forward_train(planes, sigma_weights, sigma_layers, ray_sh, samples_per_ray, color_weights, color_layers, hidden_dim, activation, B, h, c,
+                               out_width, obj_feat, input_pad, false, h0, stream);
+}
+
+int foc_field_forward_train_pad31_h0(const void *planes, const void *sigma_weights, uint32_t sigma_layers, const void *ray_sh, uint32_t samples_per_ray,
+                                     const void *color_weights, uint32_t color_layers, uint32_t hidden_dim, uint32_t activation, uint32_t B, void *h, void *c,
+                                     uint32_t out_width, const void *obj_feat, float input_pad, void *h0, void *stream) {
+    FOC_REQUIRE(h0 || B == 0, FOC_E_INVALID, "field_forward_train_pad31_h0: null h0");
+    return field_forward_train(planes, sigma_weights, sigma_layers, ray_sh, samples_per_ray, color_weights, color_layers, hidden_dim, activation, B, h, c,
+                               out_width, obj_feat, input_pad, true, h0, stream);
+}
+
+}
diff --git a/focnerf_amd/csrc/fixedstep.hip b/focnerf_amd/csrc/fixedstep.hip
--- a/focnerf_amd/csrc/fixedstep.hip
+++ b/focnerf_amd/csrc/fixedstep.hip
@@ -53,6 +53,23 @@
     o[15] = 0.59004358992664352f * x * (-x2 + 3.0f * y2);
 }
 
+__device__ __forceinline__ void fs_sample_point(const float *__restrict__ rays_o, const float *__restrict__ rays_d, const float *__restrict__ nears,
+                                                const float *__restrict__ fars, const float *__restrict__ noise, uint32_t n, uint32_t i, uint32_t T,
+                                                float a0, float a1, float a2, float a3, float a4, float a5, float &x, float &y, float &w) {
+    const FsGeom g = fs_geom(nears, fars, n, T);
+    const float z = fs_z(g, i, T, noise, (uint64_t)n * T + i);
+    x = rays_o[n * 3] + rays_d[n * 3] * z; y = rays_o[n * 3 + 1] + rays_d[n * 3 + 1] * z; w = rays_o[n * 3 + 2] + rays_d[n * 3 + 2] * z;
+    x = fminf(fmaxf(x, a0), a3); y = fminf(fmaxf(y, a1), a4); w = fminf(fmaxf(w, a2), a5);
+}
+__device__ __forceinline__ void fs_store_ray_sh(const float *__restrict__ rays_d, uint32_t n, _Float16 *__restrict__ ray_sh) {
+    float sh[16];
+    fs_sh16(rays_d[n * 3], rays_d[n * 3 + 1], rays_d[n * 3 + 2], sh);
+    h8 lo, hi;
+#pragma unroll
+    for (int k = 0; k < 8; k++) { lo[k] = foc_f2h(sh[k]); hi[k] = foc_f2h(sh[8 + k]); }
+    h8 *dst = reinterpret_cast<h8 *>(ray_sh + (uint64_t)n * 16);
+    dst[0] = lo; dst[1] = hi;
+}
 __global__ void __launch_bounds__(256) k_fs_sample(const float *__restrict__ rays_o, const float *__restrict__ rays_d, const float *__restrict__ nears,
                                                    const float *__restrict__ fars, const float *__restrict__ aabb, const float *__restrict__ noise,
                                                    uint32_t N, uint32_t T, float bound, float *__restrict__ xyzs, float *__restrict__ enc_in,
@@ -72,22 +89,44 @@
         } else {
             n = (uint32_t)(s / T); i = (uint32_t)(s - (uint64_t)n * T);
         }
-        const FsGeom g = fs_geom(nears, fars, n, T);
-        const float z = fs_z(g, i, T, noise, (uint64_t)n * T + i);
-        float x = rays_o[n * 3] + rays_d[n * 3] * z, y = rays_o[n * 3 + 1] + rays_d[n * 3 + 1] * z, w = rays_o[n * 3 + 2] + rays_d[n * 3 + 2] * z;
-        x = fminf(fmaxf(x, a0), a3); y = fminf(fmaxf(y, a1), a4); w = fminf(fmaxf(w, a2), a5);
+        float x, y, w;
+        fs_sample_point(rays_o, rays_d, nears, fars, noise, n, i, T, a0, a1, a2, a3, a4, a5, x, y, w);
         if (xyzs) { xyzs[s * 3] = x; xyzs[s * 3 + 1] = y; xyzs[s * 3 + 2] = w; }
         if (enc_in) { enc_in[s * 3] = (x + bound) / two_b; enc_in[s * 3 + 1] = (y + bound) / two_b; enc_in[s * 3 + 2] = (w + bound) / two_b; }
-        if (ray_sh && i == 0 && own) {
-            float sh[16];
-            fs_sh16(rays_d[n * 3], rays_d[n * 3 + 1], rays_d[n * 3 + 2], sh);
-            h8 lo, hi;
-#pragma unroll
-            for (int k = 0; k < 8; k++) { lo[k] = foc_f2h(sh[k]); hi[k] = foc_f2h(sh[8 + k]); }
-            h8 *dst = reinterpret_cast<h8 *>(ray_sh + (uint64_t)n * 16);
-            dst[0] = lo; dst[1] = hi;
-        }
-    }
+        if (ray_sh && i == 0 && own) fs_store_ray_sh(rays_d, n, ray_sh);
+    }
+}
+
+__global__ void __launch_bounds__(256) k_fs_sample_wave(const float *__restrict__ rays_o, const float *__restrict__ rays_d, const float *__restrict__ nears,
+                                                        const float *__restrict__ fars, const float *__restrict__ aabb, const float *__restrict__ noise,
+                                                        uint32_t N, uint32_t T, float bound, float *__restrict__ xyzs, float *__restrict__ enc_in,
+                                                        _Float16 *__restrict__ ray_sh) {
+    __shared__ float s_pos[2][4][192];
+    const uint32_t lane = threadIdx.x & 63, wave = threadIdx.x >> 6;
+    const uint32_t per_ray = T / 64u;
+    const uint32_t wv = (uint32_t)__builtin_amdgcn_readfirstlane((int)(blockIdx.x * 4u + wave));
+    if (wv >= N * per_ray) return;
+    const uint32_t n = wv / per_ray, i = (wv - n * per_ray) * 64u + lane;
+    const float a0 = aabb[0], a1 = aabb[1], a2 = aabb[2], a3 = aabb[3], a4 = aabb[4], a5 = aabb[5];
+    const float two_b = 2 * bound;
+    float x, y, w;
+    fs_sample_point(rays_o, rays_d, nears, fars, noise, n, i, T, a0, a1, a2, a3, a4, a5, x, y, w);
+    const uint64_t out0 = (uint64_t)wv * 192u;
+    float *sx = s_pos[0][wave], *se = s_pos[1][wave];
+    if (xyzs) { sx[lane * 3u] = x; sx[lane * 3u + 1u] = y; sx[lane * 3u + 2u] = w; }
+    if (enc_in) { se[lane * 3u] = (x + bound) / two_b; se[lane * 3u + 1u] = (y + bound) / two_b; se[lane * 3u + 2u] = (w + bound) / two_b; }
+    __builtin_amdgcn_fence(__ATOMIC_RELEASE, "wavefront");
+    __builtin_amdgcn_wave_barrier();
+    __builtin_amdgcn_fence(__ATOMIC_ACQUIRE, "wavefront");
+    if (xyzs) {
+#pragma unroll
+        for (uint32_t j = 0; j < 3u; j++) xyzs[out0 + j * 64u + lane] = sx[j * 64u + lane];
+    }
+    if (enc_in) {
+#pragma unroll
+        for (uint32_t j = 0; j < 3u; j++) enc_in[out0 + j * 64u + lane] = se[j * 64u + lane];
+    }
+    if (ray_sh && i == 0) fs_store_ray_sh(rays_d, n, ray_sh);
 }
 
 __global__ void __launch_bounds__(256) k_fs_head_fwd(const _Float16 *__restrict__ h, const float *__restrict__ rays_d, const float *__restrict__ nears,
@@ -276,7 +315,7 @@
                                                      float bg_scalar, uint32_t N, uint32_t T, float density_scale, float thresh,
                                                      float *__restrict__ sigma_out, float *__restrict__ trans_out, float *__restrict__ weights_out,
                                                      float *__restrict__ weights_sum, float *__restrict__ depth, float *__restrict__ image, uint32_t c_ld,
-                                                     float *__restrict__ ray_sumsq) {
+                                                     float *__restrict__ ray_sumsq, uint32_t h_ld) {
     const uint32_t lane = threadIdx.x & 63;
     const uint32_t n = blockIdx.x * 4 + (threadIdx.x >> 6);
     if (n >= N) return;
@@ -287,7 +326,7 @@
         const bool valid = i < T;
         const uint32_t ic = valid ? i : T - 1;
         const uint64_t s = (uint64_t)n * T + ic;
-        const _Float16 h0 = h[s * 16];
+        const _Float16 h0 = h[s * h_ld];
         const uint2 raw = *reinterpret_cast<const uint2 *>(c + s * c_ld);
         float u0 = 0.0f, u1 = 0.0f;
         if (NOISE) { u0 = noise[s]; u1 = noise[(uint64_t)n * T + min(ic + 1u, T - 1u)]; }
@@ -544,6 +583,12 @@
     FOC_REQUIRE(T >= 2, FOC_E_INVALID, "fixed_sample: T must be >= 2");
     FOC_REQUIRE(ray_block == 0 || ray_block == FS_RAY_BLOCK, FOC_E_INVALID, "fixed_sample: ray_block must be 0 (ray-major) or %u (got %u)", FS_RAY_BLOCK, ray_block);
     const uint64_t rows = ray_block ? (uint64_t)foc_div_up(N, FS_RAY_BLOCK) * FS_RAY_BLOCK * T : (uint64_t)N * T;
+    if (!ray_block && T % 64u == 0u && rows / 64u < (1ull << 31) && foc_opt(FOC_OPT_FS_SAMPLE_WAVE)) {
+        hipLaunchKernelGGL(k_fs_sample_wave, dim3((uint32_t)((rows / 64u + 3u) / 4u)), dim3(256), 0, (hipStream_t)stream, rays_o, rays_d, nears, fars, aabb,
+                           noise, N, T, bound, xyzs, enc_in, (_Float16 *)ray_sh);
+        FOC_CHECK_LAUNCH("fixed_sample");
+        return FOC_OK;
+    }
     hipLaunchKernelGGL(k_fs_sample, dim3(foc_grid_1d(rows, 256, 256 * 16)), dim3(256), 0, (hipStream_t)stream, rays_o, rays_d, nears, fars, aabb,
                        noise, N, T, bound, xyzs, enc_in, (_Float16 *)ray_sh, ray_block);
     FOC_CHECK_LAUNCH("fixed_sample");
@@ -601,19 +646,33 @@
     return FOC_OK;
 }
 
+static int fixed_tail_forward(const char *who, const void *h, uint32_t h_ld, const void *c, const float *nears, const float *fars, const float *noise,
+                              const float *bg_ray, float bg_scalar, uint32_t N, uint32_t T, float density_scale, float thresh, float *sigma, float *trans,
+                              float *weights, float *weights_sum, float *depth, float *image, uint32_t c_width, float *ray_sumsq, void *stream) {
+    FocDeviceGuard foc_guard_(stream, h);
+    if (N == 0) return FOC_OK;
+    FOC_REQUIRE(c_width == 16 || c_width == 4, FOC_E_INVALID, "%s: c_width must be 16 or 4 (got %u)", who, c_width);
+    FOC_REQUIRE(h && c && nears && fars && sigma && trans && weights && weights_sum && depth && image, FOC_E_INVALID, "%s: null pointer", who);
+    FOC_REQUIRE(T >= 2, FOC_E_INVALID, "%s: T must be >= 2", who);
+    auto kern = noise ? k_fs_tail_fwd<true> : k_fs_tail_fwd<false>;
+    hipLaunchKernelGGL(kern, dim3(foc_div_up(N, 4)), dim3(256), 0, (hipStream_t)stream, (const _Float16 *)h, (const _Float16 *)c, nears, fars, noise,
+                       bg_ray, bg_scalar, N, T, density_scale, thresh, sigma, trans, weights, weights_sum, depth, image, c_width, ray_sumsq, h_ld);
+    FOC_CHECK_LAUNCH(who);
+    return FOC_OK;
+}
+
 int foc_fixed_tail_forward(const void *h, const void *c, const float *nears, const float *fars, const float *noise, const float *bg_ray, float bg_scalar,
                            uint32_t N, uint32_t T, float density_scale, float thresh, float *sigma, float *trans, float *weights, float *weights_sum,
                            float *depth, float *image, uint32_t c_width, float *ray_sumsq, void *stream) {
-    FocDeviceGuard foc_guard_(stream, h);
-    if (N == 0) return FOC_OK;
-    FOC_REQUIRE(c_width == 16 || c_width == 4, FOC_E_INVALID, "fixed_tail_forward: c_width must be 16 or 4 (got %u)", c_width);
-    FOC_REQUIRE(h && c && nears && fars && sigma && trans && weights && weights_sum && depth && image, FOC_E_INVALID, "fixed_tail_forward: null pointer");
-    FOC_REQUIRE(T >= 2, FOC_E_INVALID, "fixed_tail_forward: T must be >= 2");
-    auto kern = noise ? k_fs_tail_fwd<true> : k_fs_tail_fwd<false>;
-    hipLaunchKernelGGL(kern, dim3(foc_div_up(N, 4)), dim3(256), 0, (hipStream_t)stream, (const _Float16 *)h, (const _Float16 *)c, nears, fars, noise,
-                       bg_ray, bg_scalar, N, T, density_scale, thresh, sigma, trans, weights, weights_sum, depth, image, c_width, ray_sumsq);
-    FOC_CHECK_LAUNCH("fixed_tail_forward");
-    return FOC_OK;
+    return fixed_tail_forward("fixed_tail_forward", h, 16, c, nears, fars, noise, bg_ray, bg_scalar, N, T, density_scale, thresh, sigma, trans, weights,
+                              weights_sum, depth, image, c_width, ray_sumsq, stream);
+}
+
+int foc_fixed_tail_forward_h0(const void *h0, const void *c, const float *nears, const float *fars, const float *noise, const float *bg_ray, float bg_scalar,
+                              uint32_t N, uint32_t T, float density_scale, float thresh, float *sigma, float *trans, float *weights, float *weights_sum,
+                              float *depth, float *image, uint32_t c_width, float *ray_sumsq, void *stream) {
+    return fixed_tail_forward("fixed_tail_forward_h0", h0, 1, c, nears, fars, noise, bg_ray, bg_scalar, N, T, density_scale, thresh, sigma, trans, weights,
+                              weights_sum, depth, image, c_width, ray_sumsq, stream);
 }
 
 int foc_fixed_tail_backward(const float *grad_image, const float *grad_ws, const float *grad_depth, const void *c, const float *sigma, const float *trans,
diff --git a/focnerf_amd/csrc/gridencoder.hip b/focnerf_amd/csrc/gridencoder.hip
--- a/focnerf_amd/csrc/gridencoder.hip
+++ b/focnerf_amd/csrc/gridencoder.hip
@@ -572,7 +572,7 @@
 #define GB_PM_TILE 1024u
 #define GB_PMS_WG 1024u
 
-__global__ void __launch_bounds__(256) k_gbin_scans(GbHeader *__restrict__ hdr, uint32_t *__restrict__ wg_hist, uint32_t n_wg, uint32_t L) {
+__global__ void __launch_bounds__(256) k_gbin_scans(GbHeader *__restrict__ hdr, uint32_t *__restrict__ wg_hist, uint32_t n_wg, uint32_t L, uint32_t wide) {
     __shared__ uint32_t s_wave[2][4];
     const uint32_t lane = threadIdx.x & 63, wave = threadIdx.x >> 6;
     const uint32_t n = L * GB_MAX_SEGS;
@@ -596,6 +596,30 @@
     }
     const uint32_t slot = blockIdx.x;
     uint32_t *col = wg_hist + (uint64_t)slot * n_wg;
+    if (wide && (n_wg & 3u) == 0u && (reinterpret_cast<uintptr_t>(col) & 15u) == 0u) {
+        uint4 *col4 = reinterpret_cast<uint4 *>(col);
+        const uint32_t n4 = n_wg >> 2, per4 = (n4 + 255u) / 256u;
+        const uint32_t lo = min(n4, threadIdx.x * per4), hi = min(n4, lo + per4);
+        const uint4 zero4 = make_uint4(0u, 0u, 0u, 0u);
+        const uint4 v0 = lo < hi ? col4[lo] : zero4, v1 = lo + 1u < hi ? col4[lo + 1u] : zero4;
+        uint32_t local = (v0.x + v0.y + v0.z + v0.w) + (v1.x + v1.y + v1.z + v1.w);
+        for (uint32_t i = lo + 2u; i < hi; i++) { const uint4 v = col4[i]; local += v.x + v.y + v.z + v.w; }
+        const uint32_t incl = (uint32_t)wave_incl_sum_i((int)local, (int)lane);
+        if (lane == 63) s_wave[0][wave] = incl;
+        __syncthreads();
+        uint32_t run = incl - local;
+        for (uint32_t k = 0; k < wave; k++) run += s_wave[0][k];
+        auto put = [&](uint32_t i, const uint4 &v) {
+            uint4 o;
+            o.x = run; o.y = o.x + v.x; o.z = o.y + v.y; o.w = o.z + v.z;
+            run = o.w + v.w;
+            col4[i] = o;
+        };
+        if (lo < hi) put(lo, v0);
+        if (lo + 1u < hi) put(lo + 1u, v1);
+        for (uint32_t i = lo + 2u; i < hi; i++) put(i, col4[i]);
+        return;
+    }
     const uint32_t per = (n_wg + 255) / 256;
     const uint32_t lo = min(n_wg, threadIdx.x * per), hi = min(n_wg, lo + per);
     uint32_t local = 0;
@@ -1342,7 +1366,7 @@
     uint32_t *wg_hist = reinterpret_cast<uint32_t *>(reinterpret_cast<char *>(recs) + gb_recs_bytes(B, L, dtype));
     hipLaunchKernelGGL(k_gbin_count_pt, dim3(n_wg), dim3(GB_PMS_WG), 0, st, inputs, offsets, hdr, wg_hist, B, L, lv, gridtype, ac, interp);
     FOC_CHECK_LAUNCH("grid_encode_backward(count)");
-    hipLaunchKernelGGL(k_gbin_scans, dim3(L * GB_MAX_SEGS + 1), dim3(256), 0, st, hdr, wg_hist, n_wg, L);
+    hipLaunchKernelGGL(k_gbin_scans, dim3(L * GB_MAX_SEGS + 1), dim3(256), 0, st, hdr, wg_hist, n_wg, L, foc_opt(FOC_OPT_GB_SCAN_WIDE) ? 1u : 0u);
     FOC_CHECK_LAUNCH("grid_encode_backward(scans)");
     return FOC_OK;
 }
@@ -1364,7 +1388,7 @@
     hipLaunchKernelGGL((k_grid_fwd_counted<T>), dim3(fwd_blocks + n_count), dim3(256), 0, st, inputs, (const T *)emb, offsets, (T *)outputs, B, L, lv, gridtype, ac,
                        interp, chunks, sizeof(T) == 2 ? ge_pairs_mode(emb, nullptr, sizeof(T), 3, 2, gridtype, ac, interp) : 0u, hdr, wg_hist, n_tiles, period, w0, lc, csplit);
     FOC_CHECK_LAUNCH("grid_encode_forward_counted");
-    hipLaunchKernelGGL(k_gbin_scans, dim3(L * GB_MAX_SEGS + 1), dim3(256), 0, st, hdr, wg_hist, n_tiles, L);
+    hipLaunchKernelGGL(k_gbin_scans, dim3(L * GB_MAX_SEGS + 1), dim3(256), 0, st, hdr, wg_hist, n_tiles, L, foc_opt(FOC_OPT_GB_SCAN_WIDE) ? 1u : 0u);
     FOC_CHECK_LAUNCH("grid_encode_forward_counted(scans)");
     return FOC_OK;
 }
diff --git a/focnerf_amd/field.py b/focnerf_amd/field.py
--- a/focnerf_amd/field.py
+++ b/focnerf_amd/field.py
@@ -53,11 +53,11 @@
     background: bool = False
 
 
-def pad_twin(name, pad, obj):
+def pad_twin(name, pad, obj, suffix=""):
     from ._lib import lib
     if pad == 0:
-        return getattr(lib, name), ()
-    return getattr(lib, name + ("_pad" if obj else "_pad31")), (float(pad),)
+        return getattr(lib, name + suffix), ()
+    return getattr(lib, name + ("_pad" if obj else "_pad31") + suffix), (float(pad),)
 
 
 def _on(switch):
@@ -204,7 +204,7 @@
         if ticket is None:
             _gridencoder.grid_encode_forward(x, emb, offsets, enc, B, 3, 2, L, S, H, None, gridtype, align_corners, interp)
         h = torch.empty(B, 16, device=x.device, dtype=torch.half)
-        c = None
+        c = h0 = None
         if colour is not None:
             from ._lib import ptr, stream_of, check
             cweights, cshape, ray_sh, T, c_width, obj_feat = colour[:6]
@@ -212,10 +212,11 @@
             wc = _half_of(cweights)
             obj16 = obj_feat.detach().reshape(-1).half().contiguous() if obj_feat is not None else None
             c = torch.empty(B, c_width, device=x.device, dtype=torch.half)
+            h0 = torch.empty(B, device=x.device, dtype=torch.half)
             args = (ptr(enc), ptr(w), sigma.num_layers, ptr(ray_sh), int(T), ptr(wc), int(cshape.num_layers), 64, int(sigma.activation), B, ptr(h),
                     ptr(c), int(c_width), ptr(obj16))
-            fn, extra = pad_twin("foc_field_forward_train", pad, obj16 is not None)
-            check(fn(*args, *extra, stream_of(enc)), "field_forward_train")
+            fn, extra = pad_twin("foc_field_forward_train", pad, obj16 is not None, "_h0")
+            check(fn(*args, *extra, ptr(h0), stream_of(enc)), "field_forward_train")
         else:
             _ffmlp.ffmlp_forward_planar(enc, w, B, sigma.input_dim, 16, sigma.hidden_dim, sigma.num_layers, sigma.activation, sigma.output_activation, h)
         if training:
@@ -224,13 +225,13 @@
             ctx.ticket = ticket
         if c is None:
             return h
-        ctx.mark_non_differentiable(c)
+        ctx.mark_non_differentiable(c, h0)
         ctx.set_materialize_grads(False)
-        return h, c
+        return h, c, h0
 
     @staticmethod
     @custom_bwd(device_type="cuda")
-    def backward(ctx, grad_h, _grad_c=None):
+    def backward(ctx, grad_h, _grad_c=None, _grad_h0=None):
         x, emb, w, offsets, enc = ctx.saved_tensors
         grid, sigma, B, L = ctx.cfg
         if grad_h is None:
@@ -279,6 +280,6 @@
     h = _hashgrid_mlp.apply(xn, encoder.embeddings, mlp.weights, encoder.offsets, encoder.spec(), MlpShape.of(mlp), mlp.training and torch.is_grad_enabled(),
                             colour)
     if colour is not None:
-        h, c = h
-        return h.view(prefix + [16]), c
+        h, c, h0 = h
+        return h.view(prefix + [16]), c, h0
     return h.view(prefix + [16])
diff --git a/focnerf_amd/fixedstep.py b/focnerf_amd/fixedstep.py
--- a/focnerf_amd/fixedstep.py
+++ b/focnerf_amd/fixedstep.py
@@ -126,7 +126,7 @@
 
     @staticmethod
     def forward(ctx, h, cweights, ray_sh, nears, fars, noise, bg_ray, bg_scalar, N, T, density_scale, thresh, num_layers, activation, obj_feat=None,
-                want_sumsq=False, c_pre=None, w16_pre=None, input_pad=0.0):
+                want_sumsq=False, c_pre=None, w16_pre=None, input_pad=0.0, h0_pre=None):
         from .field import _half_of, pad_twin
         h = h.contiguous()
         assert h.dtype == torch.float16 and h.shape == (N * T, 16)
@@ -153,8 +153,11 @@
         depth = torch.empty(N, dtype=torch.float32, device=dev)
         image = torch.empty(N, 3, dtype=torch.float32, device=dev)
         sumsq = torch.empty(N, dtype=torch.float32, device=dev) if want_sumsq else None
-        check(lib.foc_fixed_tail_forward(ptr(h), ptr(c), ptr(nears), ptr(fars), ptr(noise), ptr(bg_ray), float(bg_scalar), N, T, float(density_scale),
-                                         float(thresh), ptr(sigma), ptr(trans), ptr(weights), ptr(ws), ptr(depth), ptr(image), _C_WIDTH, ptr(sumsq), st),
+        if h0_pre is not None:
+            assert c_pre is not None and h0_pre.dtype == torch.float16 and h0_pre.shape == (M,) and h0_pre.is_contiguous()
+        tail_fwd, density_logits = (lib.foc_fixed_tail_forward_h0, h0_pre) if h0_pre is not None else (lib.foc_fixed_tail_forward, h)
+        check(tail_fwd(ptr(density_logits), ptr(c), ptr(nears), ptr(fars), ptr(noise), ptr(bg_ray), float(bg_scalar), N, T, float(density_scale),
+                       float(thresh), ptr(sigma), ptr(trans), ptr(weights), ptr(ws), ptr(depth), ptr(image), _C_WIDTH, ptr(sumsq), st),
               "fixed_tail_forward")
         empty = torch.empty(0, device=dev)
         ctx.bg_grad = bg_ray is not None and ctx.needs_input_grad[6]
@@ -200,7 +203,7 @@
         check(fn(*args, *extra, st), "color_head_backward")
         g_obj = g_obj32.to(obj_dtype).view(obj_shape) if g_obj32 is not None else None
         g_bg = g_image * (1 - ws).unsqueeze(-1) if ctx.bg_grad else None
-        return (grad_h, g_w, None, None, None, None, g_bg) + (None,) * 7 + (g_obj, None, None, None, None)
+        return (grad_h, g_w, None, None, None, None, g_bg) + (None,) * 7 + (g_obj, None, None, None, None, None)
 
 
 class _masked_norm(Function):
@@ -282,7 +285,7 @@
 
     enc = model.encoder
     from .field import hashgrid_mlp, fused_mlp
-    c_pre = obj_feat = None
+    c_pre = h0_pre = obj_feat = None
     cweights = fused_mlp(model, "color_net").weights if want_tail else None
     with torch.autocast("cuda", dtype=torch.float16):
         if plan.uses_object_feature:
@@ -295,7 +298,7 @@
                 colour = (wc16, plan.colour, ray_sh, T, _C_WIDTH, obj_feat, plan.colour_input_pad)
             h = hashgrid_mlp(enc, fused_mlp(model, "sigma_net"), enc_in, None, colour)
             if colour is not None:
-                h, c_pre = h
+                h, c_pre, h0_pre = h
         else:
             feats = grid_encode(enc_in, enc.embeddings, enc.offsets, enc.per_level_scale, enc.base_resolution, False, enc.gridtype_id,
                                 enc.align_corners, enc.interp_id)
@@ -310,7 +313,7 @@
             bg_ray, bg_scalar = _background(bg_color, N, dev)
             outs = _render_tail.apply(h, cweights, ray_sh, nears, fars, noise, bg_ray, bg_scalar, N, T, model.density_scale, weight_thresh,
                                       cn.num_layers, cn.activation, obj_feat, want_crit and yolo_details[0].numel() == N, c_pre,
-                                      wc16 if c_pre is not None else None, plan.colour_input_pad)
+                                      wc16 if c_pre is not None else None, plan.colour_input_pad, h0_pre)
             image, weights_sum, depth, sigma, weights, c = outs[:6]
             if len(outs) == 7:
                 criterion_outside_mask = _masked_norm.apply(outs[6], (~yolo_details[0].reshape(N)).to(torch.float32))
diff --git a/include/focnerf.h b/include/focnerf.h
--- a/include/focnerf.h
+++ b/include/focnerf.h
@@ -237,6 +237,15 @@
 int foc_field_forward_train_pad31(const void *planes, const void *sigma_weights, uint32_t sigma_layers, const void *ray_sh, uint32_t samples_per_ray,
                                   const void *color_weights, uint32_t color_layers, uint32_t hidden_dim, uint32_t activation, uint32_t B,
                                   void *h, void *c, uint32_t out_width, const void *obj_feat, float input_pad, void *stream);
+int foc_field_forward_train_h0(const void *planes, const void *sigma_weights, uint32_t sigma_layers, const void *ray_sh, uint32_t samples_per_ray,
+                               const void *color_weights, uint32_t color_layers, uint32_t hidden_dim, uint32_t activation, uint32_t B,
+                               void *h, void *c, uint32_t out_width, const void *obj_feat, void *h0, void *stream);
+int foc_field_forward_train_pad_h0(const void *planes, const void *sigma_weights, uint32_t sigma_layers, const void *ray_sh, uint32_t samples_per_ray,
+                                   const void *color_weights, uint32_t color_layers, uint32_t hidden_dim, uint32_t activation, uint32_t B,
+                                   void *h, void *c, uint32_t out_width, const void *obj_feat, float input_pad, void *h0, void *stream);
+int foc_field_forward_train_pad31_h0(const void *planes, const void *sigma_weights, uint32_t sigma_layers, const void *ray_sh, uint32_t samples_per_ray,
+                                     const void *color_weights, uint32_t color_layers, uint32_t hidden_dim, uint32_t activation, uint32_t B,
+                                     void *h, void *c, uint32_t out_width, const void *obj_feat, float input_pad, void *h0, void *stream);
 
 int foc_allocate_splitk(uint64_t size);
 int foc_free_splitk(void);
@@ -280,6 +289,10 @@
                            const float *bg_ray, float bg_scalar, uint32_t N, uint32_t T, float density_scale, float thresh,
                            float *sigma, float *trans, float *weights, float *weights_sum, float *depth, float *image,
                            uint32_t c_width, float *ray_sumsq, void *stream);
+int foc_fixed_tail_forward_h0(const void *h0, const void *c, const float *nears, const float *fars, const float *noise,
+                              const float *bg_ray, float bg_scalar, uint32_t N, uint32_t T, float density_scale, float thresh,
+                              float *sigma, float *trans, float *weights, float *weights_sum, float *depth, float *image,
+                              uint32_t c_width, float *ray_sumsq, void *stream);
 int foc_fixed_tail_backward(const float *grad_image, const float *grad_ws, const float *grad_depth, const void *c,
                             const float *sigma, const float *trans, const float *weights, const float *nears,
                             const float *fars, const float *noise, const float *bg_ray, float bg_scalar, uint32_t N,
```

After: 1.381 billion (median of 6 runs). About the same (+0.7%).
